# Maboroshi0327/MHAda-Style-Transfer

Hardware: AMD Instinct MI355X
Metric: stylized frames/sec (whole job) at 512x512 batch 8 fp32 [configs[1]] (higher is better)
Workload: dtype f32; 1 GPU; stylize 512x512 content+style, batch 8; resolution=512, batch_per_gpu=8, global_batch=8, compute_dtype=f32, parallelism=replicas x1

## Files before the change

include/mhada_hip.h:

```cpp
#ifndef MHADA_HIP_H
#define MHADA_HIP_H

#ifdef __cplusplus
extern "C" {
#endif

typedef void* mhada_stream_t;

enum { MHADA_OK = 0, MHADA_ERR_ARG = 1, MHADA_ERR_LAUNCH = 2 };
enum { MHADA_F32 = 0, MHADA_BF16 = 1 };
enum { MHADA_ACT_SOFTMAX = 0, MHADA_ACT_COSINE = 1 };
enum { MHADA_PAD_REFLECT = 0, MHADA_PAD_ZERO = 1 };
enum {
  MHADA_A_ROWS = 0,
  MHADA_A_PATCH8 = 1,
  MHADA_A_CONV3X3 = 2,
  MHADA_A_CONV3X3_UP2 = 3,
  MHADA_A_CONV3X3_ZERO = 4,
  MHADA_A_SPLIT3 = 5
};
enum { MHADA_BF16X3 = 2 };

int mhada_abi_version(void);
const char* mhada_last_error(void);

int mhada_set_tuning(const char* name, int value);
int mhada_get_tuning(const char* name, int* value);

int mhada_clock_probe(unsigned long long* stamps, int nblk, int iters, mhada_stream_t stream);

typedef struct mhada_gemm_args {
  int M, N, K;
  int nb1, nb2;
  int compute;
  int a_mode;
  const void* a; int a_dtype; long long lda, sa1, sa2;
  const float* a_mu; long long smu1, smu2;
  int img_c, img_h, img_w;
  const void* w; long long ldw, sw1, sw2;
  const float* bias; long long sb1, sb2;
  const void* r; int r_dtype; long long ldr, sr1, sr2;
  void* c; int c_dtype; long long ldc, sc1, sc2;
  int relu;
  int pad;
  void* c2; long long ldc2, sc21, sc22;
  void* vt; long long ldt, svt1, svt2;
  int c2_planes;
} mhada_gemm_args;

int mhada_gemm(const mhada_gemm_args* args, mhada_stream_t stream);

int mhada_layernorm(const float* x, void* y, int y_dtype, const float* gamma, const float* beta,
                    int rows, int cols, float eps, mhada_stream_t stream);

int mhada_vit_batch_attn(const void* qkv, void* out, int dtype, int L, int ntok, int heads,
                         int head_dim, mhada_stream_t stream);
int mhada_vit_batch_attn_split3(const float* qkv, void* planes, long long pstride, int L, int ntok, int heads,
                                int head_dim, mhada_stream_t stream);

int mhada_pos_embed(const float* pos, float* out, int C, int bh, int bw, int oh, int ow,
                    mhada_stream_t stream);

int mhada_instnorm_stats(const float* x, float* mu, float* rstd, double* work, int B, int N,
                         int C, int splits, float eps, mhada_stream_t stream);

int mhada_fold_block(const float* wf, const float* wg, const float* wh, const float* bg,
                     const float* bh, const float* rstd_c, const float* mu_s,
                     const float* rstd_s, void* wq, void* wkv, float* bkv, float* v_mu,
                     float kscale, int dtype, int B, int H, mhada_stream_t stream);

int mhada_transpose_v(const void* kv, void* vt, int dtype, int B, int H, int Ns, mhada_stream_t stream);

int mhada_cosine_prep(void* q, void* kv, int dtype, int B, int H, int Nc, int Ns,
                      mhada_stream_t stream);

int mhada_attn(const void* q, const void* kv, const void* vt, const float* fcs,
               const float* fcs_mu, const float* fcs_rstd, const float* v_mu, void* out,
               int dtype, int B, int H, int Nc, int Ns, int activation, mhada_stream_t stream);

int mhada_fold_block_hd(const float* wf, const float* wg, const float* wh, const float* bg,
                        const float* bh, const float* rstd_c, const float* mu_s,
                        const float* rstd_s, void* wq, void* wkv, float* bkv, float* v_mu,
                        float kscale, int dtype, int B, int H, int D, mhada_stream_t stream);

int mhada_cosine_prep_hd(void* q, void* kv, int dtype, int B, int H, int D, int Nc, int Ns,
                         mhada_stream_t stream);

int mhada_attn_hd(const void* q, const void* kv, const float* fcs, const float* fcs_mu,
                  const float* fcs_rstd, const float* v_mu, void* out, int dtype, int B, int H,
                  int D, int Nc, int Ns, int activation, mhada_stream_t stream);

int mhada_split3_kv(const float* kv, const float* vt, void* img, int B, int H, int Ns, mhada_stream_t stream);
int mhada_split3_rows(const float* x, void* planes, long long n, mhada_stream_t stream);
int mhada_split3_weight(const float* w, void* out, int N, int K0, int transposed, mhada_stream_t stream);

int mhada_layernorm_half2(const float* x, void* y, const float* gamma, const float* beta, int rows, int cols,
                          float eps, float scale, mhada_stream_t stream);
int mhada_half2_weight(const float* w, void* out, float* t, int N, int K0, mhada_stream_t stream);
int mhada_gemm_half2(const mhada_gemm_args* args, const float* col_scale, mhada_stream_t stream);
int mhada_kv_proj_split3(const float* fs, const float* mu_s, const float* wkv, const float* bkv, void* img,
                         int B, int H, int Ns, mhada_stream_t stream);
int mhada_attn_split3(const float* q, const void* img, const float* fcs, const float* fcs_mu,
                      const float* fcs_rstd, const float* v_mu, float* out, int B, int H, int Nc, int Ns,
                      mhada_stream_t stream);
int mhada_attn_split3_planes(const float* q, const void* img, const float* fcs, const float* fcs_mu,
                             const float* fcs_rstd, const float* v_mu, void* planes, int B, int H, int Nc, int Ns,
                             mhada_stream_t stream);

int mhada_cosine_moments(const void* kv, const void* vt, int dtype, int B, int H, int Ns, float* mom,
                         float* work, int splits, mhada_stream_t stream);
int mhada_cosine_attn(const void* q, const float* mom, const float* fcs, const float* fcs_mu,
                      const float* fcs_rstd, const float* v_mu, void* out, int dtype, int B, int H,
                      int Nc, mhada_stream_t stream);

int mhada_attn_train_fwd(const float* q, const float* k, const float* v, const float* x, float* out,
                         float* mo, float* lse, int BH, int Nc, int Ns, mhada_stream_t stream);
int mhada_attn_train_fwd_vt(const float* q, const float* k, const float* v, float* vt, const float* x,
                            float* out, float* mo, float* lse, int BH, int Nc, int Ns, mhada_stream_t stream);
int mhada_attn_train_fwd_split3(const float* q, const float* k, const float* v, void* img, const float* x,
                                float* out, float* mo, float* lse, int BH, int Nc, int Ns, mhada_stream_t stream);
int mhada_transpose64(const float* src, float* dst, int BH, int N, int ldt, mhada_stream_t stream);
int mhada_gemm_n64_split3(const float* a, const void* w_planes, float* c, int nz, int M, int K, int lda,
                          long long sa, int ldw, long long sw, long long wps, int ldc, long long sc,
                          mhada_stream_t stream);
int mhada_transpose64_split3(const float* k, void* planes, int BH, int N, int ldt, mhada_stream_t stream);
int mhada_attn_train_bwd(const float* q, const float* k, const float* v, const float* lse,
                         const float* dmo, const float* dd, float* dq, float* dk, float* dv,
                         int BH, int Nc, int Ns, mhada_stream_t stream);
int mhada_attn_train_dkv(const float* q, const float* k, const float* v, const float* lse, const float* dmo,
                         const float* dd, float* dk, float* dv, float* ds, int BH, int Nc, int Ns,
                         mhada_stream_t stream);

int mhada_attn_train_fwd_hd(const float* q, const float* k, const float* v, const float* x, float* out,
                            float* mo, float* lse, int BH, int D, int Nc, int Ns, mhada_stream_t stream);
int mhada_attn_train_bwd_hd(const float* q, const float* k, const float* v, const float* lse,
                            const float* dmo, const float* dd, float* dq, float* dk, float* dv,
                            int BH, int D, int Nc, int Ns, mhada_stream_t stream);

int mhada_attn_train_dq(const float* q, const float* k, const float* v, const float* lse, const float* dmo,
                        const float* dd, float* dq, int BH, int Nc, int Ns, mhada_stream_t stream);
int mhada_attn_train_dq_hd(const float* q, const float* k, const float* v, const float* lse, const float* dmo,
                           const float* dd, float* dq, int BH, int D, int Nc, int Ns, mhada_stream_t stream);

long long mhada_attn_train_bf16_workspace(int BH, int Nc, int Ns, int backward);
int mhada_attn_train_fwd_bf16(const float* q, const float* k, const float* v, const float* x, float* out,
                              float* mo, float* lse, void* ws, long long ws_size, int BH, int Nc, int Ns,
                              mhada_stream_t stream);
int mhada_attn_train_bwd_bf16(const float* q, const float* k, const float* v, const float* lse,
                              const float* dmo, const float* mo, float* dq, float* dk, float* dv,
                              void* ws, long long ws_size, int BH, int Nc, int Ns, int phases,
                              mhada_stream_t stream);

int mhada_conv3x3_out3(const void* x, int dtype, const float* w, const float* b, float* y,
                       int B, int H, int W, int Cin, int clamp255, mhada_stream_t stream);

int mhada_upsample2x(const void* x, void* y, int dtype, int B, int H, int W, int C,
                     mhada_stream_t stream);


int mhada_warp(const float* x, const float* flow, float* y, int B, int C, int H, int W,
               int padding, mhada_stream_t stream);

int mhada_warp_bwd(const float* gy, const float* flow, float* gx, int B, int C, int H, int W,
                   int padding, mhada_stream_t stream);

int mhada_flow_warp_mask(const float* flo01, const float* flo10, float* mask, int H, int W,
                         float threshold, int padding, mhada_stream_t stream);

int mhada_warp_l1(const float* cs1, const float* cs2, const float* flow, const float* mask,
                  double* work, float* out, int B, int C, int H, int W, mhada_stream_t stream);


typedef struct mhada_gemm_tn_args {
  int M, N, K;
  const float* a; long long lda;
  const float* b; long long ldb;
  int b_mode;
  int img_c, img_h, img_w, pad;
  float* c; long long ldc;
  float* colsum;
  int nb;
  long long sza, szb;
} mhada_gemm_tn_args;
int mhada_gemm_tn_splits(int M, int N, int K);
int mhada_gemm_tn(const mhada_gemm_tn_args* args, float* work, long long work_floats, mhada_stream_t stream);

int mhada_vit_batch_attn_bwd(const float* qkv, const float* dout, float* dqkv, int L, int ntok, int heads,
                             int head_dim, mhada_stream_t stream);
int mhada_vit_batch_attn_bwd_split3(const float* qkv, const float* dout, float* dqkv, void* planes,
                                    long long pstride, int L, int ntok, int heads, int head_dim,
                                    mhada_stream_t stream);

int mhada_colsum(const float* x, float* out, long long rows, int C, float* work, long long work_floats,
                 mhada_stream_t stream);

int mhada_layernorm_fwd(const float* x, float* y, float* stats, const float* gamma, const float* beta,
                        int rows, int cols, float eps, mhada_stream_t stream);
int mhada_layernorm_fwd_split3(const float* x, float* y, void* planes, float* stats, const float* gamma,
                               const float* beta, int rows, int cols, float eps, mhada_stream_t stream);

int mhada_layernorm_bwd(const float* x, const float* dy, const float* stats, const float* gamma, float* dx,
                        float* dgamma, float* dbeta, float* work, long long work_floats, int rows, int cols,
                        mhada_stream_t stream);

int mhada_instnorm_bwd(const float* dy, const float* y, const float* rstd, float* dx, double* work,
                       int B, int N, int C, int splits, mhada_stream_t stream);

int mhada_attn_train_bwd_prep(const float* dout, const float* x, const float* mo, float* dx, float* dmo,
                              float* dd, long long rows, mhada_stream_t stream);
int mhada_attn_train_bwd_prep_hd(const float* dout, const float* x, const float* mo, float* dx, float* dmo,
                                 float* dd, long long rows, int D, mhada_stream_t stream);

int mhada_pos_embed_bwd(const float* g, float* gpos, int C, int bh, int bw, int oh, int ow,
                        mhada_stream_t stream);
long long mhada_feat_stats_work(int B, long long P, int C);
int mhada_feat_stats(const float* x, const float* t, float* mu, float* sd, float* mse, double* work,
                     long long work_doubles, int B, long long P, int C, mhada_stream_t stream);
int mhada_feat_loss_bwd(const float* x, const float* t, const float* mu, const float* alpha, const float* beta,
                        const float* kp, float ks, float* g, int B, long long P, int C, int relu, mhada_stream_t stream);
int mhada_relu_bwd(const float* dy, const float* y, float* dx, long long n, mhada_stream_t stream);
int mhada_reflect_fold(const float* dxp, float* dx, int B, int H, int W, int C, const float* relu_mask,
                       mhada_stream_t stream);
int mhada_maxpool2(const float* x, float* y, int B, int H, int W, int C, mhada_stream_t stream);
int mhada_maxpool2_bwd(const float* x, const float* dy, float* dx, int B, int H, int W, int C, int relu_mask,
                       mhada_stream_t stream);
int mhada_upsample2x_bwd(const float* dy, const float* relu_x, float* dx, int B, int H, int W, int C,
                         mhada_stream_t stream);
int mhada_vgg_input(const float* img, float* out, int B, int H, int W, int Cp, mhada_stream_t stream);
int mhada_vgg_input_bwd(const float* dout, float* dimg, int B, int H, int W, int Cp, mhada_stream_t stream);

int mhada_loss_attn(const float* q, const float* k, const float* v, const float* x, const float* x_mu,
                    const float* x_rs, float* out, int B, int Nq, int Ns, int Dqk, int Dv, int activation,
                    mhada_stream_t stream);
int mhada_rows_normalize(const float* x, const float* mu, const float* rs, float* out, int unit,
                         int B, int N, int C, mhada_stream_t stream);

int mhada_frame_ingest(const void* frames, int B, int H, int W, long long row_bytes, int bgr, float* out,
                       int Ho, int Wo, mhada_stream_t stream);

int mhada_wino_weights(const float* w, float* u, int Cout, int Cin, mhada_stream_t stream);
int mhada_conv3x3_wgrad_wino_splits(int B, int H, int W, int Cin, int Cout);
int mhada_conv3x3_wgrad_wino(const float* x, const float* g, float* dw, float* db, float* work, long long work_floats,
                             int B, int H, int W, int Cin, int Cout, long long ldg, int pad_mode,
                             mhada_stream_t stream);
int mhada_conv3x3_wino(const float* x, const float* u, const float* bias, float* y, int B, int H, int W,
                       int Cin, int Cout, long long ldc, int pad_mode, int pad, int relu,
                       const float* relu_mask, mhada_stream_t stream);
int mhada_wino_weights_split3(const float* w, void* up, int Cout, int Cin, mhada_stream_t stream);
int mhada_conv3x3_wino_split3(const float* x, const float* u, const void* up, const float* bias, float* y, int B,
                              int H, int W, int Cin, int Cout, long long ldc, int pad_mode, int pad, int relu,
                              const float* relu_mask, mhada_stream_t stream);

// ... 16 lines not shown
```

mhada-style-transfer_amd/csrc/common.h:

```cpp
#pragma once
#include <hip/hip_runtime.h>
#include <stdint.h>
#include <string>

#include "../../include/mhada_hip.h"

typedef __bf16 bf16;
typedef __bf16 bf16x8 __attribute__((ext_vector_type(8)));
typedef __bf16 bf16x4 __attribute__((ext_vector_type(4)));
typedef float f32x16 __attribute__((ext_vector_type(16)));
typedef float f32x4 __attribute__((ext_vector_type(4)));
typedef float f32x2 __attribute__((ext_vector_type(2)));

#define MHADA_DEV __device__ __forceinline__

namespace mhada {

void set_error(const std::string& msg);
int fail(const std::string& msg);
int check_launch(const char* what);

struct Tuning {
  int attn_fixed_shift = 1;
  int attn_waves = 0;
  int attn_tk = 128;
  int attn_prio = 1;
  int vit_attn_vec = 1;
  int out3_mfma = 1;
  int out3_tile = 1;
  int gemm_pp = 1;
  int gemm_persist = 1;
  int gemm_pp128 = 1;
  int gemm_ldsepi = 1;
  int gemm_n64 = 128;
  int conv_c64 = 1;
  int conv_dir = 1;
  int gemm_rinit = 1;
  int tn_skinny_lds = 1;
  int wino4 = 1;
  int wino_split3 = 1;
  int gemm_s3_order = 1;
  int train_dkv_dma = 1;
  int upsample_quad = 1;
  int xknob = 0;
};
const Tuning& tuning();

int conv3x3_c64(const void* x, const void* w, const float* bias, void* y, int B, int H, int W, bool up, int relu,
                hipStream_t s);
int conv3x3_dir(const void* x, const void* w, const float* bias, void* y, int B, int H, int W, int cin, int cout,
                int relu, hipStream_t s);

int vit_batch_attn_hd(const void* qkv, void* out, int dtype, int L, int ntok, int heads, int head_dim, hipStream_t s);

template <typename T> MHADA_DEV float to_f32(T x);
template <> MHADA_DEV float to_f32<float>(float x) { return x; }
template <> MHADA_DEV float to_f32<bf16>(bf16 x) { return (float)x; }

template <typename T> MHADA_DEV T from_f32(float x);
template <> MHADA_DEV float from_f32<float>(float x) { return x; }
template <> MHADA_DEV bf16 from_f32<bf16>(float x) { return (bf16)x; }

template <typename T> struct Vec16;
template <> struct Vec16<float> { typedef f32x4 type; static constexpr int N = 4; };
template <> struct Vec16<bf16> { typedef bf16x8 type; static constexpr int N = 8; };

MHADA_DEV float bilerp(float ly0, float ly1, float lx0, float lx1, float x00, float x01, float x10, float x11) {
  return fmaf(ly1, fmaf(lx0, x10, lx1 * x11), ly0 * fmaf(lx0, x00, lx1 * x01));
}

MHADA_DEV float wave_sum(float v) {
#pragma unroll
  for (int o = 32; o > 0; o >>= 1) v += __shfl_xor(v, o, 64);
  return v;
}
MHADA_DEV float wave_max(float v) {
#pragma unroll
  for (int o = 32; o > 0; o >>= 1) v = fmaxf(v, __shfl_xor(v, o, 64));
  return v;
}

MHADA_DEV int xcd_remap(int bid, int nblk) {
  const int q = nblk / 8, r = nblk % 8;
  const int xcd = bid % 8, k = bid / 8;
  return (xcd < r ? xcd * (q + 1) : r * (q + 1) + (xcd - r) * q) + k;
}

}
```

mhada-style-transfer_amd/csrc/gemm_half2.hip:

```cpp
#include "gemm_impl.h"

using namespace mhada;

extern "C" int mhada_gemm_half2(const mhada_gemm_args* a, const float* col_scale, mhada_stream_t stream_) {
  if (!a) return fail("mhada_gemm_half2: null args");
  hipStream_t stream = (hipStream_t)stream_;
  if (a->M < 0 || a->N <= 0 || a->K <= 0) return fail("mhada_gemm_half2: bad sizes");
  if (a->nb1 != 1 || a->nb2 != 1) return fail("mhada_gemm_half2: one problem only (nb1 = nb2 = 1)");
  if (a->K % 64) return fail("mhada_gemm_half2: K0 must be a multiple of 64");
  if (a->a_mode != MHADA_A_ROWS || a->a_mu || a->vt) return fail("mhada_gemm_half2: ROWS mode, no centring / vt");
  if (a->c_dtype != MHADA_F32 && a->c_dtype != MHADA_BF16) return fail("mhada_gemm_half2: bad c_dtype");
  if (a->r && a->r_dtype != a->c_dtype) return fail("mhada_gemm_half2: residual dtype must equal output dtype");
  if (a->relu < 0 || a->relu > 1) return fail("mhada_gemm_half2: relu must be 0 or 1");
  if (!a->a || !a->w || !col_scale || (!a->c && !a->c2_planes)) return fail("mhada_gemm_half2: null operand");
  if (a->M == 0) return MHADA_OK;
  if (!aligned16(a->a) || a->lda % 8 || a->lda < a->K)
    return fail("mhada_gemm_half2: A must be 16-byte aligned with lda a multiple of 8 and >= K0");
  if (!aligned16(a->w) || a->ldw % 8 || a->ldw < 2 * (long long)a->K)
    return fail("mhada_gemm_half2: W must be 16-byte aligned with ldw a multiple of 8 and >= 2 K0");
  if (!aligned16(col_scale)) return fail("mhada_gemm_half2: col_scale must be 16-byte aligned");
  if (((uintptr_t)a->c & 7) || a->ldc % 4) return fail("mhada_gemm_half2: C must be 8-byte aligned with ldc % 4 == 0");
  if (a->r && (((uintptr_t)a->r & 7) || a->ldr % 4))
    return fail("mhada_gemm_half2: R must be 8-byte aligned with ldr % 4 == 0");
  if (a->bias && !aligned16(a->bias)) return fail("mhada_gemm_half2: bias must be 16-byte aligned");
  if (a->c2 && (a->c_dtype != MHADA_F32 || ((uintptr_t)a->c2 & 7) || a->ldc2 % 4))
    return fail("mhada_gemm_half2: c2 needs fp32 C, 8-byte alignment and ldc2 % 4 == 0");
  if (a->c2_planes && (!a->c2 || a->N % 4 || !tuning().gemm_ldsepi))
    return fail("mhada_gemm_half2: c2_planes needs a c2 buffer, N % 4 == 0 and the LDS epilogue");
  if ((((long long)a->M + 255) / 256) * (((long long)a->N + 255) / 256) >= (1LL << 31))
    return fail("mhada_gemm_half2: more than 2^31 tiles");
  if ((long long)(a->M - 1) * a->lda + a->K >= (1LL << 31) || (long long)(a->N - 1) * a->ldw + 2LL * a->K >= (1LL << 31))
    return fail("mhada_gemm_half2: operand spans need 32-bit element offsets");
  GemmP p{};
  p.M = a->M; p.N = a->N; p.K = a->K; p.nb2 = 1;
  p.a = a->a; p.lda = a->lda;
  p.spl = (long long)a->M * a->lda;
  p.w = a->w; p.ldw = a->ldw;
  p.bias = a->bias;
  p.r = a->r; p.ldr = a->ldr;
  p.c = a->c; p.ldc = a->ldc;
  p.relu = a->relu;
  p.c2 = a->c2; p.ldc2 = a->ldc2;
  p.c2planes = a->c2_planes ? 1 : 0;
  if (a->c_dtype == MHADA_F32) return launch_gemm_h2<float>(p, col_scale, stream);
  return launch_gemm_h2<bf16>(p, col_scale, stream);
}
```

mhada-style-transfer_amd/csrc/gemm_impl.h:

```cpp
#pragma once
#include "common.h"

#include <algorithm>
#include <mutex>
#include <stdlib.h>

namespace mhada {

struct GemmP {
  int M, N, K, nb2;
  const void* a; long long lda, sa1, sa2;
  const float* a_mu; long long smu1, smu2;
  int img_c, img_h, img_w, out_h, out_w;
  int pad;
  const void* w; long long ldw, sw1, sw2;
  const float* bias; long long sb1, sb2;
  const void* r; long long ldr, sr1, sr2;
  void* c; long long ldc, sc1, sc2;
  int relu, tiles_n, ntiles;
  int lds_epi;
  int rinit;
  void* c2; long long ldc2, sc21, sc22;
  void* vt; long long ldt, svt1, svt2;
  long long spl;
// ... 87 lines not shown
  bool valid;
};

template <typename TA, typename TC, int AMODE, int A_CH>
MHADA_DEV void issue_a(AStage<TA, TC, AMODE, A_CH>& st, const GemmP& p, const TA* abase,
                       const RowInfo (&ri)[A_CH], int k0, int kc) {
  constexpr int E = Cfg<TC>::E;
  const int k = k0 + kc * E;
  const bool kvalid = k < p.K;
  if constexpr (AMODE == MHADA_A_ROWS || AMODE == kRowsCentred) {
#pragma unroll
    for (int i = 0; i < A_CH; ++i) {
      const long long m = (long long)ri[i].b;
      st.raw[i][0] = (ri[i].valid && kvalid) ? load_raw<TA, TC>(abase + m * p.lda + k) : zero_raw<TA, TC>();
      st.wt[i][0] = 1.f;
    }
    if constexpr (AMODE == kRowsCentred) {
#pragma unroll
      for (int e = 0; e < E; ++e) st.mu[e] = kvalid ? p.a_mu[k + e] : 0.f;
    }
  } else if constexpr (AMODE == MHADA_A_PATCH8) {
    const int cch = k >> 6, py = (k >> 3) & 7, px = k & 7;
    const long long plane = (long long)p.img_h * p.img_w;
#pragma unroll
    for (int i = 0; i < A_CH; ++i) {
      const TA* src = abase + cch * plane + (long long)(ri[i].y * 8 + py) * p.img_w + ri[i].x * 8 + px;
      st.raw[i][0] = (ri[i].valid && kvalid) ? load_raw<TA, TC>(src) : zero_raw<TA, TC>();
      st.wt[i][0] = 1.f;
    }
  } else {
    const int cin_n = p.img_c;
    const int tap = k / cin_n, cin = k - tap * cin_n;
    const int dy = tap / 3 - 1, dx = tap % 3 - 1;
#pragma unroll
    for (int i = 0; i < A_CH; ++i) {
      int Y, X;
      const bool inside = conv_src<AMODE>(p, ri[i].y, ri[i].x, dy, dx, Y, X);
      const bool ok = ri[i].valid && kvalid && inside;
      if constexpr (AMODE == MHADA_A_CONV3X3 || AMODE == MHADA_A_CONV3X3_ZERO) {
        const TA* src = abase + (((long long)ri[i].b * p.img_h + Y) * p.img_w + X) * cin_n + cin;
        st.raw[i][0] = ok ? load_raw<TA, TC>(src) : zero_raw<TA, TC>();
        st.wt[i][0] = 1.f;
      } else {
        const float sy = fmaxf(((float)Y + 0.5f) * 0.5f - 0.5f, 0.f);
        const float sx = fmaxf(((float)X + 0.5f) * 0.5f - 0.5f, 0.f);
        const int y0 = (int)sy, x0 = (int)sx;
        const int y1 = y0 + (y0 < p.img_h - 1 ? 1 : 0), x1 = x0 + (x0 < p.img_w - 1 ? 1 : 0);
        const float ly1 = sy - (float)y0, lx1 = sx - (float)x0;
        const float ly0 = 1.f - ly1, lx0 = 1.f - lx1;
        const long long rb = (long long)ri[i].b * p.img_h;
        const TA* s00 = abase + ((rb + y0) * p.img_w + x0) * cin_n + cin;
        const TA* s01 = abase + ((rb + y0) * p.img_w + x1) * cin_n + cin;
        const TA* s10 = abase + ((rb + y1) * p.img_w + x0) * cin_n + cin;
        const TA* s11 = abase + ((rb + y1) * p.img_w + x1) * cin_n + cin;
        st.raw[i][0] = ok ? load_raw<TA, TC>(s00) : zero_raw<TA, TC>();
        st.raw[i][1] = ok ? load_raw<TA, TC>(s01) : zero_raw<TA, TC>();
        st.raw[i][2] = ok ? load_raw<TA, TC>(s10) : zero_raw<TA, TC>();
        st.raw[i][3] = ok ? load_raw<TA, TC>(s11) : zero_raw<TA, TC>();
        st.wt[i][0] = ly0; st.wt[i][1] = ly1; st.wt[i][2] = lx0; st.wt[i][3] = lx1;
      }
    }
  }
}

template <int RS, typename TA, typename TC, int AMODE, int A_CH>
MHADA_DEV void commit_a(const AStage<TA, TC, AMODE, A_CH>& st, TC* sA, int tid) {
  constexpr int E = Cfg<TC>::E, LS = Cfg<TC>::LS;
  const int kc = tid & 7;
#pragma unroll
  for (int i = 0; i < A_CH; ++i) {
    const int row = (tid >> 3) + RS * i;
    float f[E];
    if constexpr (AMODE == MHADA_A_CONV3X3_UP2) {
      const float ly0 = st.wt[i][0], ly1 = st.wt[i][1], lx0 = st.wt[i][2], lx1 = st.wt[i][3];
#pragma unroll
      for (int e = 0; e < E; ++e)
        f[e] = bilerp(ly0, ly1, lx0, lx1, raw_get(st.raw[i][0], e), raw_get(st.raw[i][1], e),
                      raw_get(st.raw[i][2], e), raw_get(st.raw[i][3], e));
    } else if constexpr (AMODE == kRowsCentred || sizeof(TA) != sizeof(TC)) {
#pragma unroll
      for (int e = 0; e < E; ++e) f[e] = raw_get(st.raw[i][0], e) - (AMODE == kRowsCentred ? st.mu[e] : 0.f);
    } else {
      *reinterpret_cast<typename Vec16<TC>::type*>(sA + row * LS + kc * E) = st.raw[i][0].v;
      continue;
    }
    store_chunk<TC>(sA + row * LS + kc * E, f);
  }
}

template <typename TO, int TM, int TN>
MHADA_DEV void store_tile(const GemmP& p, const f32x16 (&acc)[TM][TN], int z1, int z2, int mrow, int ncol, int h) {
  TO* cbase = reinterpret_cast<TO*>(p.c) + z1 * p.sc1 + z2 * p.sc2;
  const TO* rbase = p.r ? reinterpret_cast<const TO*>(p.r) + z1 * p.sr1 + z2 * p.sr2 : nullptr;
  const float* bbase = p.bias ? p.bias + z1 * p.sb1 + z2 * p.sb2 : nullptr;
#pragma unroll
  for (int mi = 0; mi < TM; ++mi) {
    const int m = mrow + mi * 32;
    if (m >= p.M) continue;
    TO* crow = cbase + (long long)m * p.ldc;
    const TO* rrow = rbase ? rbase + (long long)m * p.ldr : nullptr;
#pragma unroll
    for (int ni = 0; ni < TN; ++ni) {
#pragma unroll
      for (int g = 0; g < 4; ++g) {
        const int n = ncol + ni * 32 + 8 * g + 4 * h;
        float v[4];
#pragma unroll
        for (int e = 0; e < 4; ++e) v[e] = acc[mi][ni][4 * g + e];
        if (n + 3 < p.N) {
          if (bbase) {
            const f32x4 bb = *reinterpret_cast<const f32x4*>(bbase + n);
#pragma unroll
            for (int e = 0; e < 4; ++e) v[e] += bb[e];
          }
          if (p.relu == 1) {
#pragma unroll
            for (int e = 0; e < 4; ++e) v[e] = fmaxf(v[e], 0.f);
          }
          if constexpr (sizeof(TO) == 4) {
            if (rrow) {
              const f32x4 rr = *reinterpret_cast<const f32x4*>(rrow + n);
#pragma unroll
              for (int e = 0; e < 4; ++e) v[e] = p.relu == 2 ? (rr[e] > 0.f ? v[e] : 0.f) : v[e] + rr[e];
            }
            *reinterpret_cast<f32x4*>(crow + n) = f32x4{v[0], v[1], v[2], v[3]};
            if (p.c2)
              *reinterpret_cast<bf16x4*>(reinterpret_cast<bf16*>(p.c2) + z1 * p.sc21 + z2 * p.sc22 +
                                         (long long)m * p.ldc2 + n) = bf16x4{(bf16)v[0], (bf16)v[1], (bf16)v[2], (bf16)v[3]};
          } else {
            if (rrow) {
              const bf16x4 rr = *reinterpret_cast<const bf16x4*>(rrow + n);
#pragma unroll
              for (int e = 0; e < 4; ++e) v[e] += (float)rr[e];
            }
            *reinterpret_cast<bf16x4*>(crow + n) = bf16x4{(bf16)v[0], (bf16)v[1], (bf16)v[2], (bf16)v[3]};
          }
        } else {
#pragma unroll
          for (int e = 0; e < 4; ++e) {
            if (n + e < p.N) {
              float x = v[e] + (bbase ? bbase[n + e] : 0.f);
              if (p.relu == 1) x = fmaxf(x, 0.f);
              if (rrow) x = p.relu == 2 ? (to_f32<TO>(rrow[n + e]) > 0.f ? x : 0.f) : x + to_f32<TO>(rrow[n + e]);
              crow[n + e] = from_f32<TO>(x);
            }
          }
        }
      }
    }
  }
}


template <typename TO, int TM, int TN, bool PLANES = false>
MHADA_DEV void store_tile_lds(const GemmP& p, const f32x16 (&acc)[TM][TN], int z1, int z2, int mrow0, int ncol0,
                              int lane, float* scr) {
  TO* cbase = reinterpret_cast<TO*>(p.c) + z1 * p.sc1 + z2 * p.sc2;
  const TO* rbase = p.r ? reinterpret_cast<const TO*>(p.r) + z1 * p.sr1 + z2 * p.sr2 : nullptr;
  const float* bbase = p.bias ? p.bias + z1 * p.sb1 + z2 * p.sb2 : nullptr;
  const int h = lane >> 5, r32 = lane & 31;
  const int rr = lane >> 3, cq = lane & 7;
#pragma unroll
  for (int ni = 0; ni < TN; ++ni) {
    const int n = ncol0 + ni * 32 + 4 * cq;
    f32x4 bb = {0.f, 0.f, 0.f, 0.f};
    if (bbase) {
      if (n + 3 < p.N) {
        bb = *reinterpret_cast<const f32x4*>(bbase + n);
      } else {
#pragma unroll
        for (int e = 0; e < 4; ++e) bb[e] = n + e < p.N ? bbase[n + e] : 0.f;
      }
    }
#pragma unroll
    for (int mi = 0; mi < TM; ++mi) {
#pragma unroll
      for (int g = 0; g < 4; ++g) {
        const int c = 2 * g + h;
        *reinterpret_cast<f32x4*>(scr + r32 * 32 + 4 * (c ^ (r32 & 7))) =
            f32x4{acc[mi][ni][4 * g], acc[mi][ni][4 * g + 1], acc[mi][ni][4 * g + 2], acc[mi][ni][4 * g + 3]};
      }
      asm volatile("s_waitcnt lgkmcnt(0)" ::: "memory");
      f32x4 v[4];
#pragma unroll
      for (int i = 0; i < 4; ++i) {
        const int r = 8 * i + rr;
        v[i] = *reinterpret_cast<const f32x4*>(scr + r * 32 + 4 * (cq ^ (r & 7)));
      }
      asm volatile("s_waitcnt lgkmcnt(0)" ::: "memory");
#pragma unroll
      for (int i = 0; i < 4; ++i) {
        const int m = mrow0 + mi * 32 + 8 * i + rr;
        if (m >= p.M) continue;
        float x[4];
#pragma unroll
        for (int e = 0; e < 4; ++e) {
          x[e] = v[i][e] + bb[e];
          if (p.relu == 1) x[e] = fmaxf(x[e], 0.f);
        }
        TO* crow = cbase + (long long)m * p.ldc;
        const TO* rrow = rbase ? rbase + (long long)m * p.ldr : nullptr;
        if (n + 3 < p.N) {
          if constexpr (sizeof(TO) == 4) {
            if (rrow) {
              const f32x4 q = *reinterpret_cast<const f32x4*>(rrow + n);
#pragma unroll
              for (int e = 0; e < 4; ++e) x[e] = p.relu == 2 ? (q[e] > 0.f ? x[e] : 0.f) : x[e] + q[e];
            }
            if (!PLANES || p.c) *reinterpret_cast<f32x4*>(crow + n) = f32x4{x[0], x[1], x[2], x[3]};
            if (p.c2) {
              bf16* c2row = reinterpret_cast<bf16*>(p.c2) + z1 * p.sc21 + z2 * p.sc22 + (long long)m * p.ldc2 + n;
              const bf16x4 h0 = {(bf16)x[0], (bf16)x[1], (bf16)x[2], (bf16)x[3]};
              *reinterpret_cast<bf16x4*>(c2row) = h0;
              if (PLANES && p.c2planes) {
                const long long pl = (long long)p.M * p.ldc2;
                float r1[4];
                bf16x4 h1, h2;
#pragma unroll
                for (int e = 0; e < 4; ++e) {
                  r1[e] = x[e] - (float)h0[e];
                  h1[e] = (bf16)r1[e];
                  h2[e] = (bf16)(r1[e] - (float)h1[e]);
                }
                *reinterpret_cast<bf16x4*>(c2row + pl) = h1;
                *reinterpret_cast<bf16x4*>(c2row + 2 * pl) = h2;
              }
            }
          } else {
            if (rrow) {
              const bf16x4 q = *reinterpret_cast<const bf16x4*>(rrow + n);
#pragma unroll
              for (int e = 0; e < 4; ++e) x[e] += (float)q[e];
            }
            *reinterpret_cast<bf16x4*>(crow + n) = bf16x4{(bf16)x[0], (bf16)x[1], (bf16)x[2], (bf16)x[3]};
          }
        } else {
#pragma unroll
          for (int e = 0; e < 4; ++e) {
            if (n + e < p.N) {
              float y = x[e];
              if (rrow) y = p.relu == 2 ? (to_f32<TO>(rrow[n + e]) > 0.f ? y : 0.f) : y + to_f32<TO>(rrow[n + e]);
              crow[n + e] = from_f32<TO>(y);
            }
          }
        }
      }
    }
  }
}

template <typename TO, int TM>
MHADA_DEV void store_vt_tile(const GemmP& p, const f32x16 (&acc)[TM][2], int z1, int z2, int mrow0, int ncol0,
                             int lane, float* scr) {
  TO* vbase = reinterpret_cast<TO*>(p.vt) + z1 * p.svt1 + z2 * p.svt2;
  const float* bbase = p.bias ? p.bias + z1 * p.sb1 + z2 * p.sb2 : nullptr;
  const int h = lane >> 5, r32 = lane & 31;
#pragma unroll
  for (int mi = 0; mi < TM; ++mi) {
    const int m0 = mrow0 + 32 * mi;
    if (m0 >= p.ldt) break;
    const bool mv = m0 + r32 < p.M;
#pragma unroll
    for (int ni = 0; ni < 2; ++ni) {
      if constexpr (sizeof(TO) == 2) {
        bf16* sb = reinterpret_cast<bf16*>(scr);
        const int pos = (r32 & ~12) | ((r32 & 4) << 1) | ((r32 & 8) >> 1);
#pragma unroll
        for (int g = 0; g < 4; ++g)
#pragma unroll
          for (int e = 0; e < 4; ++e) {
            const int ol = 8 * g + 4 * h + e;
            float x = acc[mi][ni][4 * g + e] + (bbase ? bbase[ncol0 + 32 * ni + ol] : 0.f);
            sb[ol * 32 + pos] = mv ? (bf16)x : (bf16)0.0f;
          }
        asm volatile("s_waitcnt lgkmcnt(0)" ::: "memory");
        bf16x8 v[2];
#pragma unroll
        for (int j = 0; j < 2; ++j) {
          const int c = lane + 64 * j;
          v[j] = *reinterpret_cast<const bf16x8*>(sb + (c >> 2) * 32 + 8 * (c & 3));
        }
        asm volatile("s_waitcnt lgkmcnt(0)" ::: "memory");
#pragma unroll
        for (int j = 0; j < 2; ++j) {
          const int c = lane + 64 * j, ol = c >> 2, part = c & 3;
          TO* dst = vbase + (long long)(32 * ni + ol) * p.ldt + m0 + 8 * part;
          *reinterpret_cast<bf16x8*>(dst) = v[j];
          bf16x8 sq;
#pragma unroll
          for (int e = 0; e < 8; ++e) {
            const float f = (float)v[j][e];
            sq[e] = (bf16)(f * f);
          }
          *reinterpret_cast<bf16x8*>(dst + 64 * p.ldt) = sq;
        }
      } else {
#pragma unroll
        for (int g = 0; g < 4; ++g)
#pragma unroll
          for (int e = 0; e < 4; ++e) {
            const int ol = 8 * g + 4 * h + e;
            const float x = acc[mi][ni][4 * g + e] + (bbase ? bbase[ncol0 + 32 * ni + ol] : 0.f);
            scr[ol * 32 + r32] = mv ? x : 0.f;
          }
        asm volatile("s_waitcnt lgkmcnt(0)" ::: "memory");
        f32x4 v[4];
#pragma unroll
        for (int j = 0; j < 4; ++j) {
          const int c = lane + 64 * j;
          v[j] = *reinterpret_cast<const f32x4*>(scr + (c >> 3) * 32 + 4 * (c & 7));
        }
        asm volatile("s_waitcnt lgkmcnt(0)" ::: "memory");
#pragma unroll
        for (int j = 0; j < 4; ++j) {
          const int c = lane + 64 * j, ol = c >> 3, part = c & 7;
          float* dst = reinterpret_cast<float*>(vbase) + (long long)(32 * ni + ol) * p.ldt + m0 + 4 * part;
          *reinterpret_cast<f32x4*>(dst) = v[j];
          *reinterpret_cast<f32x4*>(dst + 64 * p.ldt) = v[j] * v[j];
        }
      }
    }
  }
}

template <int TM>
MHADA_DEV void store_tile_lds_bf16(const GemmP& p, const f32x16 (&acc)[TM][2], int z1, int z2, int mrow0, int ncol0,
                                   int lane, float* scr_f) {
  bf16* cbase = reinterpret_cast<bf16*>(p.c) + z1 * p.sc1 + z2 * p.sc2;
  const float* bbase = p.bias ? p.bias + z1 * p.sb1 + z2 * p.sb2 : nullptr;
  char* scr = reinterpret_cast<char*>(scr_f);
  const int h = lane >> 5, r32 = lane & 31;
  const int rr = lane >> 3, cq = lane & 7;
  f32x4 bb[2][4];
#pragma unroll
  for (int ni = 0; ni < 2; ++ni)
#pragma unroll
    for (int g = 0; g < 4; ++g) {
      const int n = ncol0 + ni * 32 + 8 * g + 4 * h;
      bb[ni][g] = f32x4{0.f, 0.f, 0.f, 0.f};
      if (bbase) {
        if (n + 3 < p.N) {
          bb[ni][g] = *reinterpret_cast<const f32x4*>(bbase + n);
        } else {
#pragma unroll
          for (int e = 0; e < 4; ++e) bb[ni][g][e] = n + e < p.N ? bbase[n + e] : 0.f;
        }
      }
    }
  const int n = ncol0 + 8 * cq;
#pragma unroll
  for (int mi = 0; mi < TM; ++mi) {
#pragma unroll
    for (int ni = 0; ni < 2; ++ni)
#pragma unroll
      for (int g = 0; g < 4; ++g) {
        bf16x4 o;
#pragma unroll
        for (int e = 0; e < 4; ++e) {
          float x = acc[mi][ni][4 * g + e] + bb[ni][g][e];
          if (p.relu == 1) x = fmaxf(x, 0.f);
          o[e] = (bf16)x;
        }
        const int c = 4 * ni + g;
// ... 642 lines not shown
#pragma unroll
      for (int i = 0; i < 2; ++i) glds16(src + s.aoff[hh][i], dst + hh * HALF + PE * i);
  };
  auto stage_w = [&](const St& s, int hh, int blk, int kk, int slot) {
    const bf16* src = wb + (6 * kk + blk) * BK;
    bf16* dst = smW + slot * SLOT + hh * HALF + wave * 2 * PE;
#pragma unroll
    for (int i = 0; i < 2; ++i) glds16(src + s.woff[hh][i], dst + PE * i);
  };

  const int swz = (r32 >> 1) & 7;
  int koff[4];
#pragma unroll
  for (int ks = 0; ks < 4; ++ks) koff[ks] = 8 * ((2 * ks + h) ^ swz);
  const bf16* sA = smA + grp * HALF + r32 * BK;
  const bf16* sW = smW + (wc >> 1) * HALF + ((wc & 1) * 64 + r32) * BK;
  bf16x8 af[4][2], wf[2][2];
  auto read_a = [&](int kp, int slot) {
#pragma unroll
    for (int mt = 0; mt < 4; ++mt)
#pragma unroll
      for (int s2 = 0; s2 < 2; ++s2)
        af[mt][s2] = *reinterpret_cast<const bf16x8*>(sA + slot * SLOT + mt * 32 * BK + koff[2 * kp + s2]);
  };
  auto read_w = [&](int nt, int kp, int slot) {
#pragma unroll
    for (int s2 = 0; s2 < 2; ++s2)
      wf[nt][s2] = *reinterpret_cast<const bf16x8*>(sW + slot * SLOT + nt * 32 * BK + koff[2 * kp + s2]);
  };
  f32x16 acc[4][2];
  auto zero_acc = [&](const St& s) {
    if constexpr (sizeof(TO) == 4) {
      if (p.rinit) {
        const float* rb = reinterpret_cast<const float*>(p.r);
        const float* bb = p.bias;
#pragma unroll
        for (int nt = 0; nt < 2; ++nt)
#pragma unroll
          for (int g = 0; g < 4; ++g) {
            const int n = s.n0 + wc * 64 + nt * 32 + 8 * g + 4 * h;
            const bool nok = n + 3 < p.N;
            const f32x4 b4 = (bb && nok) ? *reinterpret_cast<const f32x4*>(bb + n) : f32x4{0.f, 0.f, 0.f, 0.f};
#pragma unroll
            for (int mt = 0; mt < 4; ++mt) {
              const int m = s.m0 + grp * 128 + mt * 32 + r32;
              f32x4 r4 = {0.f, 0.f, 0.f, 0.f};
              if (nok && m < p.M) r4 = *reinterpret_cast<const f32x4*>(rb + (long long)m * p.ldr + n);
#pragma unroll
              for (int e = 0; e < 4; ++e) acc[mt][nt][4 * g + e] = r4[e] + b4[e];
            }
          }
        return;
      }
    }
#pragma unroll
    for (int a = 0; a < 4; ++a)
#pragma unroll
      for (int b = 0; b < 2; ++b)
#pragma unroll
        for (int e = 0; e < 16; ++e) acc[a][b][e] = 0.f;
  };
  GemmP pe = p;
  if (p.rinit) {
    pe.r = nullptr;
    pe.bias = nullptr;
  }
  auto compute = [&](int nt) {
    __builtin_amdgcn_s_setprio(1);
#pragma unroll
    for (int s2 = 0; s2 < 2; ++s2)
#pragma unroll
      for (int mt = 0; mt < 4; ++mt)
        acc[mt][nt] = __builtin_amdgcn_mfma_f32_32x32x16_bf16(wf[nt][s2], af[mt][s2], acc[mt][nt], 0, 0, 0);
    __builtin_amdgcn_s_setprio(0);
  };
  constexpr int EPI_MIN = sizeof(TO) == 4 ? 32 : 16;
  auto wait_vm = [&](int keep) __attribute__((always_inline)) {
    if (keep == 0) asm volatile("s_waitcnt vmcnt(0)" ::: "memory");
    else if (keep == 4) asm volatile("s_waitcnt vmcnt(4)" ::: "memory");
    else if (keep == 8) asm volatile("s_waitcnt vmcnt(8)" ::: "memory");
    else asm volatile("s_waitcnt vmcnt(%0)" :: "n"(8 + EPI_MIN) : "memory");
  };
  auto ktile = [&](int as, int ws, bool sw, const St& wt, int wblk, int wkk, int wsl, bool sa, const St& at, int apl,
                   int akk, int asl, int keep) __attribute__((always_inline)) {
    read_a(0, as); read_w(0, 0, ws);
    if (sw) stage_w(wt, 0, wblk, wkk, wsl);
    PP_LGKM0(); PP_BARRIER(); compute(0); PP_BARRIER();
    read_w(1, 0, ws);
    if (sw) stage_w(wt, 1, wblk, wkk, wsl);
    PP_LGKM0(); PP_BARRIER(); compute(1); PP_BARRIER();
    read_a(1, as); read_w(0, 1, ws);
    PP_LGKM0(); PP_BARRIER(); compute(0); PP_BARRIER();
    read_w(1, 1, ws);
    if (sa) stage_a(at, apl, akk, asl);
    wait_vm(keep);
    PP_LGKM0(); PP_BARRIER(); compute(1); PP_BARRIER();
  };
  int ap = 0;
  auto chunk = [&](const St& sc, int kk, const St& sn, int kn, bool nx, bool wx) __attribute__((always_inline)) {
    const int a0 = ap, a1 = ap ^ 1;
    ktile(a0, 0, true, sc, 0, kk, 1, true, sc, 0, kk, a0, wx ? 8 + EPI_MIN : 8);
    ktile(a1, 0, false, sc, 0, 0, 0, false, sc, 0, 0, 0, 4);
    ktile(a1, 1, true, sc, 2, kk, 0, nx, sn, 2, kn, a1, nx ? 8 : 4);
    ktile(a0, 1, false, sc, 0, 0, 0, false, sc, 0, 0, 0, nx ? 4 : 0);
    ktile(a0, 0, true, sc, 1, kk, 1, false, sc, 0, 0, 0, 0);
    ktile(a0, 1, nx, sn, 1, kn, 0, nx, sn, 1, kn, a0, nx ? 4 : 0);
    ap ^= 1;
  };

  const int KC = p.K / (6 * BK);
  int w = blockIdx.x;
  St cur, nxt;
  setup(w, cur);
  bool has_nxt = w + G < total;
  if (has_nxt) setup(w + G, nxt);
  zero_acc(cur);
  stage_a(cur, 2, 0, 0);
  stage_w(cur, 0, 1, 0, 0); stage_w(cur, 1, 1, 0, 0);
  stage_a(cur, 1, 0, 1);
  asm volatile("s_waitcnt vmcnt(4)" ::: "memory");
  PP_BARRIER();
  if (grp == 1) PP_BARRIER();

  bool lazy = false;
  while (true) {
    for (int kk = 0; kk + 1 < KC; ++kk) chunk(cur, kk, cur, kk + 1, true, kk == 0 && lazy);
    chunk(cur, KC - 1, nxt, 0, has_nxt, KC == 1 && lazy);
    if (grp == 0) PP_BARRIER();
    lazy = has_nxt && !p.rinit && cur.m0 + 256 <= p.M && cur.n0 + 256 <= p.N;
    __builtin_amdgcn_sched_barrier(0);
    if (p.lds_epi) {
      float* scr = reinterpret_cast<float*>(smem + 4 * SLOT) + wave * 1024;
      bool wide = false;
      if constexpr (sizeof(TO) == 2) {
        wide = !pe.r;
        if (wide) store_tile_lds_bf16<4>(pe, acc, 0, 0, cur.m0 + grp * 128, cur.n0 + wc * 64, lane, scr);
      }
      if (!wide) store_tile_lds<TO, 4, 2, true>(pe, acc, 0, 0, cur.m0 + grp * 128, cur.n0 + wc * 64, lane, scr);
    } else {
      store_tile<TO, 4, 2>(pe, acc, 0, 0, cur.m0 + grp * 128 + r32, cur.n0 + wc * 64, h);
    }
    if (!has_nxt) break;
    if (grp == 1) PP_BARRIER();
    zero_acc(nxt);
    cur = nxt;
    w += G;
    has_nxt = w + G < total;
    if (has_nxt) setup(w + G, nxt);
  }
}

typedef _Float16 f16x8 __attribute__((ext_vector_type(8)));

template <typename TO>
__global__ void __launch_bounds__(512) gemm_h2_kernel(const GemmP p, int total, const float* __restrict__ cs) {
  constexpr int BK = 64, PE = 512, HALF = 128 * BK, SLOT = 2 * HALF;
  constexpr int SCR = 8 * 4096 / 2;
  __shared__ __attribute__((aligned(16))) _Float16 smem[4 * SLOT + SCR];
  _Float16* const smA = smem;
  _Float16* const smW = smem + 2 * SLOT;
  const int tid = threadIdx.x, lane = tid & 63;
  const int wave = __builtin_amdgcn_readfirstlane(tid >> 6);
  const int grp = wave >> 2, wc = wave & 3;
  const int h = lane >> 5, r32 = lane & 31;
  const int G = gridDim.x;

  int cofs[2];
#pragma unroll
  for (int i = 0; i < 2; ++i) cofs[i] = 8 * ((lane & 7) ^ (4 * i + (lane >> 4)));
  struct St {
    unsigned aoff[2][2], woff[2][2];
    int m0, n0;
  };
  const _Float16* const ab = reinterpret_cast<const _Float16*>(p.a);
  const _Float16* const wb = reinterpret_cast<const _Float16*>(p.w);
  auto setup = [&](int w, St& s) {
    const int t = xcd_remap(w, total);
    const int tm = t / p.tiles_n, tn = t - tm * p.tiles_n;
    s.m0 = tm * 256;
    s.n0 = tn * 256;
#pragma unroll
    for (int hh = 0; hh < 2; ++hh)
#pragma unroll
      for (int i = 0; i < 2; ++i) {
        const int rr = 16 * wave + 8 * i + (lane >> 3);
        const int m = min(s.m0 + 128 * hh + rr, p.M - 1);
        const int n = min(s.n0 + 128 * hh + rr, p.N - 1);
        s.woff[hh][i] = (unsigned)((long long)n * p.ldw + cofs[i]);
        s.aoff[hh][i] = (unsigned)((long long)m * p.lda + cofs[i]);
      }
  };
  auto stage_a = [&](const St& s, int pl, int kk, int slot) {
    const _Float16* src = ab + pl * p.spl + kk * BK;
    _Float16* dst = smA + slot * SLOT + wave * 2 * PE;
#pragma unroll
    for (int hh = 0; hh < 2; ++hh)
#pragma unroll
      for (int i = 0; i < 2; ++i) glds16(src + s.aoff[hh][i], dst + hh * HALF + PE * i);
  };
  auto stage_w = [&](const St& s, int hh, int blk, int kk, int slot) {
    const _Float16* src = wb + (2 * kk + blk) * BK;
    _Float16* dst = smW + slot * SLOT + hh * HALF + wave * 2 * PE;
#pragma unroll
    for (int i = 0; i < 2; ++i) glds16(src + s.woff[hh][i], dst + PE * i);
  };

  const int swz = (r32 >> 1) & 7;
  int koff[4];
#pragma unroll
  for (int ks = 0; ks < 4; ++ks) koff[ks] = 8 * ((2 * ks + h) ^ swz);
  const _Float16* sA = smA + grp * HALF + r32 * BK;
  const _Float16* sW = smW + (wc >> 1) * HALF + ((wc & 1) * 64 + r32) * BK;
  f16x8 af[4][2], wf[2][2];
  auto read_a = [&](int kp, int slot) {
#pragma unroll
    for (int mt = 0; mt < 4; ++mt)
#pragma unroll
      for (int s2 = 0; s2 < 2; ++s2)
        af[mt][s2] = *reinterpret_cast<const f16x8*>(sA + slot * SLOT + mt * 32 * BK + koff[2 * kp + s2]);
  };
  auto read_w = [&](int nt, int kp, int slot) {
#pragma unroll
    for (int s2 = 0; s2 < 2; ++s2)
      wf[nt][s2] = *reinterpret_cast<const f16x8*>(sW + slot * SLOT + nt * 32 * BK + koff[2 * kp + s2]);
  };
  f32x16 acc[4][2];
  auto zero_acc = [&]() {
#pragma unroll
    for (int a = 0; a < 4; ++a)
#pragma unroll
      for (int b = 0; b < 2; ++b)
#pragma unroll
        for (int e = 0; e < 16; ++e) acc[a][b][e] = 0.f;
  };
  auto scale_acc = [&](const St& s) {
#pragma unroll
    for (int nt = 0; nt < 2; ++nt)
#pragma unroll
      for (int g = 0; g < 4; ++g) {
        const int n = s.n0 + wc * 64 + nt * 32 + 8 * g + 4 * h;
        f32x4 c4 = {0.f, 0.f, 0.f, 0.f};
        if (n + 3 < p.N) {
          c4 = *reinterpret_cast<const f32x4*>(cs + n);
        } else {
#pragma unroll
          for (int e = 0; e < 4; ++e)
            if (n + e < p.N) c4[e] = cs[n + e];
        }
#pragma unroll
        for (int mt = 0; mt < 4; ++mt)
#pragma unroll
          for (int e = 0; e < 4; ++e) acc[mt][nt][4 * g + e] *= c4[e];
      }
  };
  auto compute = [&](int nt) {
    __builtin_amdgcn_s_setprio(1);
#pragma unroll
    for (int s2 = 0; s2 < 2; ++s2)
#pragma unroll
      for (int mt = 0; mt < 4; ++mt)
        acc[mt][nt] = __builtin_amdgcn_mfma_f32_32x32x16_f16(wf[nt][s2], af[mt][s2], acc[mt][nt], 0, 0, 0);
    __builtin_amdgcn_s_setprio(0);
  };
  constexpr int EPI_MIN = sizeof(TO) == 4 ? 32 : 16;
  auto wait_vm = [&](int keep) __attribute__((always_inline)) {
    if (keep == 0) asm volatile("s_waitcnt vmcnt(0)" ::: "memory");
    else if (keep == 4) asm volatile("s_waitcnt vmcnt(4)" ::: "memory");
    else if (keep == 8) asm volatile("s_waitcnt vmcnt(8)" ::: "memory");
    else asm volatile("s_waitcnt vmcnt(%0)" :: "n"(8 + EPI_MIN) : "memory");
  };
  auto ktile = [&](int as, int ws, bool sw, const St& wt, int wblk, int wkk, int wsl, bool sa, const St& at, int apl,
                   int akk, int asl, int keep) __attribute__((always_inline)) {
    read_a(0, as); read_w(0, 0, ws);
    if (sw) stage_w(wt, 0, wblk, wkk, wsl);
    PP_LGKM0(); PP_BARRIER(); compute(0); PP_BARRIER();
    read_w(1, 0, ws);
    if (sw) stage_w(wt, 1, wblk, wkk, wsl);
    PP_LGKM0(); PP_BARRIER(); compute(1); PP_BARRIER();
    read_a(1, as); read_w(0, 1, ws);
    PP_LGKM0(); PP_BARRIER(); compute(0); PP_BARRIER();
    read_w(1, 1, ws);
    if (sa) stage_a(at, apl, akk, asl);
    wait_vm(keep);
    PP_LGKM0(); PP_BARRIER(); compute(1); PP_BARRIER();
  };
  auto chunk = [&](const St& sc, int kk, const St& sn, int kn, bool nx, bool wx) __attribute__((always_inline)) {
    ktile(0, 0, true, sc, 1, kk, 1, nx, sn, 1, kn, 0, nx ? (wx ? 8 + EPI_MIN : 8) : 4);
    ktile(1, 0, false, sc, 0, 0, 0, false, sc, 0, 0, 0, nx ? 4 : 0);
    ktile(1, 1, nx, sn, 0, kn, 0, nx, sn, 0, kn, 1, nx ? 4 : 0);
  };

  const int KC = p.K / BK;
  int w = blockIdx.x;
  St cur, nxt;
  setup(w, cur);
  bool has_nxt = w + G < total;
  if (has_nxt) setup(w + G, nxt);
  zero_acc();
  stage_a(cur, 1, 0, 0);
  stage_w(cur, 0, 0, 0, 0); stage_w(cur, 1, 0, 0, 0);
  stage_a(cur, 0, 0, 1);
  asm volatile("s_waitcnt vmcnt(4)" ::: "memory");
  PP_BARRIER();
  if (grp == 1) PP_BARRIER();

  bool lazy = false;
  while (true) {
    for (int kk = 0; kk + 1 < KC; ++kk) chunk(cur, kk, cur, kk + 1, true, kk == 0 && lazy);
    chunk(cur, KC - 1, nxt, 0, has_nxt, KC == 1 && lazy);
    if (grp == 0) PP_BARRIER();
    lazy = has_nxt && cur.m0 + 256 <= p.M && cur.n0 + 256 <= p.N;
    __builtin_amdgcn_sched_barrier(0);
    scale_acc(cur);
    if (p.lds_epi) {
      float* scr = reinterpret_cast<float*>(smem + 4 * SLOT) + wave * 1024;
      bool wide = false;
      if constexpr (sizeof(TO) == 2) {
        wide = !p.r;
        if (wide) store_tile_lds_bf16<4>(p, acc, 0, 0, cur.m0 + grp * 128, cur.n0 + wc * 64, lane, scr);
      }
      if (!wide) store_tile_lds<TO, 4, 2, true>(p, acc, 0, 0, cur.m0 + grp * 128, cur.n0 + wc * 64, lane, scr);
    } else {
      store_tile<TO, 4, 2>(p, acc, 0, 0, cur.m0 + grp * 128 + r32, cur.n0 + wc * 64, h);
    }
    if (!has_nxt) break;
    if (grp == 1) PP_BARRIER();
    zero_acc();
    cur = nxt;
    w += G;
    has_nxt = w + G < total;
    if (has_nxt) setup(w + G, nxt);
  }
}

template <int BM, int NS, int BK>
__global__ void __launch_bounds__(BM * 2) gemm_n64_kernel(const GemmP p) {
  constexpr int NWV = BM / 32, CH = BK / 4, RPI = 64 / CH;
  constexpr int AH = BM * BK, WH = 64 * BK, STAGE = AH + WH;
  constexpr int API = 32 / RPI, WPI = 64 / RPI / NWV;
  static_assert(WPI >= 1 && (CH == 8 || CH == 16), "tile config");
  __shared__ __attribute__((aligned(16))) float smem[NS * STAGE];
  const int tid = threadIdx.x, lane = tid & 63;
  const int wave = __builtin_amdgcn_readfirstlane(tid >> 6);
  int z, tile;
  if (p.lds_epi == 4) {
    const int L = blockIdx.y * gridDim.x + blockIdx.x, nt = gridDim.x;
    z = L % 8 + 8 * (L / (8 * nt));
    tile = (L / 8) % nt;
  } else {
    z = blockIdx.y;
    tile = xcd_remap(blockIdx.x, p.ntiles);
  }
  const int z1 = z / p.nb2, z2 = z - z1 * p.nb2;
  const int m0 = tile * BM;
  const float* ab = reinterpret_cast<const float*>(p.a) + z1 * p.sa1 + z2 * p.sa2;
  const float* wb = reinterpret_cast<const float*>(p.w) + z1 * p.sw1 + z2 * p.sw2;
  auto sw = [](int r) { return CH == 8 ? (r >> 1) & 7 : r & 15; };
  const float* asrc[API];
  const float* wsrc[WPI];
#pragma unroll
  for (int i = 0; i < API; ++i) {
    const int r = 32 * wave + RPI * i + lane / CH;
    const int m = min(m0 + r, p.M - 1);
    asrc[i] = ab + (long long)m * p.lda + 4 * ((lane % CH) ^ sw(r));
  }
#pragma unroll
  for (int i = 0; i < WPI; ++i) {
    const int r = RPI * (WPI * wave + i) + lane / CH;
    const int n = min(r, p.N - 1);
    wsrc[i] = wb + (long long)n * p.ldw + 4 * ((lane % CH) ^ sw(r));
  }
  auto stage = [&](int kt, int slot) {
    float* dst = smem + slot * STAGE;
    const int k0 = kt * BK;
#pragma unroll
    for (int i = 0; i < API; ++i) glds16(asrc[i] + k0, dst + (32 * wave + RPI * i) * BK);
#pragma unroll
    for (int i = 0; i < WPI; ++i) glds16(wsrc[i] + k0, dst + AH + RPI * (WPI * wave + i) * BK);
  };
  const int h = lane >> 5, r32 = lane & 31;
  int koff[CH / 2];
#pragma unroll
  for (int q = 0; q < CH / 2; ++q) koff[q] = 4 * (((CH / 2) * h + q) ^ sw(r32));
  f32x16 acc[1][2];
#pragma unroll
  for (int n = 0; n < 2; ++n)
#pragma unroll
    for (int e = 0; e < 16; ++e) acc[0][n][e] = 0.f;
  const int KT = p.K / BK;
#pragma unroll
  for (int i = 0; i < NS - 1; ++i)
    if (i < KT) stage(i, i);
  for (int kt = 0; kt < KT; ++kt) {
    const int ahead = min(KT - 1 - kt, NS - 2);
    if (ahead >= 2) asm volatile("s_waitcnt vmcnt(%0)" :: "n"(2 * (API + WPI)) : "memory");
    else if (ahead == 1) asm volatile("s_waitcnt vmcnt(%0)" :: "n"(API + WPI) : "memory");
    else asm volatile("s_waitcnt vmcnt(0)" ::: "memory");
    PP_BARRIER();
    if (kt + NS - 1 < KT) stage(kt + NS - 1, (kt + NS - 1) % NS);
    const float* sa = smem + (kt % NS) * STAGE + (32 * wave + r32) * BK;
    const float* swp = smem + (kt % NS) * STAGE + AH + r32 * BK;
    f32x4 af[CH / 2], wf[2][CH / 2];
#pragma unroll
    for (int q = 0; q < CH / 2; ++q) af[q] = *reinterpret_cast<const f32x4*>(sa + koff[q]);
#pragma unroll
    for (int n = 0; n < 2; ++n)
#pragma unroll
      for (int q = 0; q < CH / 2; ++q) wf[n][q] = *reinterpret_cast<const f32x4*>(swp + n * 32 * BK + koff[q]);
#pragma unroll
    for (int s = 0; s < BK / 2; ++s)
#pragma unroll
      for (int n = 0; n < 2; ++n)
        acc[0][n] = __builtin_amdgcn_mfma_f32_32x32x2f32(wf[n][s >> 2][s & 3], af[s >> 2][s & 3], acc[0][n], 0, 0, 0);
  }
  store_tile<float, 1, 2>(p, acc, z1, z2, m0 + 32 * wave + r32, 0, h);
}

static bool aligned16(const void* ptr) { return ((uintptr_t)ptr & 15) == 0; }

static int num_cus() {
  static int n = 0;
  if (!n) {
    int dev = 0;
    (void)hipGetDevice(&dev);
    if (hipDeviceGetAttribute(&n, hipDeviceAttributeMultiprocessorCount, dev) != hipSuccess || n <= 0) n = 256;
  }
  return n;
}

static bool persist_enabled() { return tuning().gemm_persist != 0; }

template <typename TC, typename TO, int AMODE, int BN = 256>
static int launch_gemm_pp(const GemmP& p0, int nz, hipStream_t stream) {
  GemmP p = p0;
  p.tiles_n = (p.N + BN - 1) / BN;
  p.ntiles = ((p.M + 255) / 256) * p.tiles_n;
  p.lds_epi = tuning().gemm_ldsepi ? 1 : 0;
  p.rinit = (sizeof(TO) == 4 && p.r && !p.relu && tuning().gemm_rinit && ((uintptr_t)p.r & 15) == 0 &&
             p.ldr % 4 == 0 && p.sr1 % 4 == 0 && p.sr2 % 4 == 0 && p.N % 4 == 0) ? 1 : 0;
  const long long total = (long long)p.ntiles * nz;
  if constexpr (AMODE == kRowsSplit3 && sizeof(TC) == 2 && BN == 256) {
    if (tuning().gemm_s3_order && nz == 1 && total < (1LL << 31)) {
      const int grid = (int)std::min<long long>(total, num_cus());
      hipLaunchKernelGGL((gemm_s3_kernel<TO>), dim3(grid), dim3(512), 0, stream, p, (int)total);
      return check_launch("mhada_gemm");
    }
  }
  if (sizeof(TC) == 4 || BN != 256 || AMODE == kRowsSplit3 || (p.K >= 128 && persist_enabled() && total < (1LL << 31))) {
    const int grid = (int)std::min<long long>(total, num_cus());
    hipLaunchKernelGGL((gemm_ppp_kernel<TC, TO, AMODE, BN>), dim3(grid), dim3(512), 0, stream, p, (int)total);
    return check_launch("mhada_gemm");
  }
  if constexpr (sizeof(TC) == 2 && BN == 256 && AMODE != kRowsSplit3) {
    hipLaunchKernelGGL((gemm_pp_kernel<TO, AMODE>), dim3(p.ntiles, nz), dim3(512), 0, stream, p);
    return check_launch("mhada_gemm");
  }
  return fail("mhada_gemm: no ping-pong form");
}

template <typename TO>
static int launch_gemm_h2(const GemmP& p0, const float* cs, hipStream_t stream) {
  GemmP p = p0;
  p.tiles_n = (int)(((long long)p.N + 255) / 256);
  const long long total = (((long long)p.M + 255) / 256) * p.tiles_n;
  if (total >= (1LL << 31)) return fail("mhada_gemm_half2: more than 2^31 tiles");
  p.ntiles = (int)total;
  p.lds_epi = tuning().gemm_ldsepi ? 1 : 0;
  p.rinit = 0;
  const int grid = (int)std::min<long long>(total, num_cus());
  hipLaunchKernelGGL((gemm_h2_kernel<TO>), dim3(grid), dim3(512), 0, stream, p, (int)total, cs);
  return check_launch("mhada_gemm_half2");
}

static bool pp_enabled() { return tuning().gemm_pp != 0; }

template <typename TC, typename TA, typename TO, int AMODE, int BM, int BN, int WM, int WN>
static int launch_gemm(const GemmP& p0, int nz, hipStream_t stream) {
  GemmP p = p0;
  p.tiles_n = (p.N + BN - 1) / BN;
  p.lds_epi = (tuning().gemm_ldsepi &&
               (size_t)2 * (BM + BN) * Cfg<TC>::LS * sizeof(TC) >= (size_t)WM * WN * 4096) ? 1 : 0;
  const int tiles_m = (p.M + BM - 1) / BM;
  p.ntiles = tiles_m * p.tiles_n;
  const size_t lds2 = (size_t)2 * (BM + BN) * Cfg<TC>::LS * sizeof(TC);
  const size_t lds = p.K > Cfg<TC>::BK ? lds2
                                       : std::max(lds2 / 2, (size_t)(p.lds_epi || p.vt ? WM * WN * 4096 : 0));
  static std::once_flag attr_once;
  std::call_once(attr_once, [&] {
    (void)hipFuncSetAttribute((const void*)gemm_kernel<TC, TA, TO, AMODE, BM, BN, WM, WN>,
                              hipFuncAttributeMaxDynamicSharedMemorySize, (int)lds2);
  });
  hipLaunchKernelGGL((gemm_kernel<TC, TA, TO, AMODE, BM, BN, WM, WN>), dim3(p.ntiles, nz), dim3(64 * WM * WN),
                     lds, stream, p);
  return check_launch("mhada_gemm");
}

static bool pp_offsets_fit(const GemmP& p, int amode) {
  const long long lim = 1LL << 31;
  const long long wspan = (long long)(p.N - 1) * p.ldw + p.K;
  long long aspan;
  if (amode == MHADA_A_ROWS) aspan = (long long)(p.M - 1) * p.lda + p.K;
  else aspan = (long long)p.M / ((long long)p.out_h * p.out_w) * p.img_h * p.img_w * p.img_c;
  return wspan < lim && aspan < lim;
}

template <typename TC, typename TA, typename TO, int AMODE>
static int dispatch_tile(const GemmP& p, int nz, hipStream_t s) {
  if constexpr (AMODE == MHADA_A_ROWS || AMODE == kRowsCentred) {
    if (p.vt) {
      if constexpr (sizeof(TC) == 2) return launch_gemm<TC, TA, TO, AMODE, 256, 128, 4, 2>(p, nz, s);
      else return launch_gemm<TC, TA, TO, AMODE, 128, 128, 2, 2>(p, nz, s);
    }
  }
  if (p.N <= 64) {
    if constexpr (sizeof(TC) == 4 && sizeof(TA) == 4 && sizeof(TO) == 4 && AMODE == MHADA_A_ROWS) {
      if (p.K % 32 == 0 && p.lda % 4 == 0 && p.ldw % 4 == 0 && p.sa1 % 4 == 0 && p.sa2 % 4 == 0 &&
          p.sw1 % 4 == 0 && p.sw2 % 4 == 0 && aligned16(p.a) && aligned16(p.w)) {
        GemmP q = p;
        q.tiles_n = 1;
        q.lds_epi = nz % 8 == 0 ? 4 : 0;
        if (p.K >= 1024 && p.K % 64 == 0) {
          q.ntiles = (p.M + 255) / 256;
          hipLaunchKernelGGL((gemm_n64_kernel<256, 2, 64>), dim3(q.ntiles, nz), dim3(512), 0, s, q);
        } else {
          q.ntiles = (p.M + 127) / 128;
          hipLaunchKernelGGL((gemm_n64_kernel<128, 2, 32>), dim3(q.ntiles, nz), dim3(256), 0, s, q);
        }
        return check_launch("mhada_gemm");
      }
    }
    if (tuning().gemm_n64 == 256) return launch_gemm<TC, TA, TO, AMODE, 256, 64, 8, 1>(p, nz, s);
    return launch_gemm<TC, TA, TO, AMODE, 128, 64, 4, 1>(p, nz, s);
  }
  if constexpr (sizeof(TC) == 4) {
    if constexpr (sizeof(TA) == 4 && (AMODE == MHADA_A_ROWS || AMODE == MHADA_A_CONV3X3 || AMODE == MHADA_A_CONV3X3_ZERO)) {
      const long long t256 = (long long)((p.M + 255) / 256) * ((p.N + 255) / 256) * nz;
      if (p.N > 128 && p.K % 32 == 0 && p.K >= 64 && 8 * t256 >= 7LL * num_cus() && pp_enabled() && persist_enabled() &&
          pp_offsets_fit(p, AMODE)) {
        return launch_gemm_pp<float, TO, AMODE>(p, nz, s);
      }
    }
    return launch_gemm<TC, TA, TO, AMODE, 128, 128, 2, 2>(p, nz, s);
  } else {
    if constexpr (AMODE == MHADA_A_CONV3X3_UP2) {
      return launch_gemm<TC, TA, TO, AMODE, 128, 128, 2, 2>(p, nz, s);
    } else {
      if constexpr (sizeof(TA) == 2 && (AMODE == MHADA_A_ROWS || AMODE == MHADA_A_CONV3X3)) {
        if (p.N > 128 && p.K % 64 == 0 && pp_enabled() && pp_offsets_fit(p, AMODE))
          return launch_gemm_pp<bf16, TO, AMODE>(p, nz, s);
        if (p.N > 64 && p.N <= 128 && p.K % 64 == 0 && p.K >= 128 && tuning().gemm_pp128 && pp_enabled() &&
            pp_offsets_fit(p, AMODE))
          return launch_gemm_pp<bf16, TO, AMODE, 128>(p, nz, s);
      }
      if (p.N <= 128) return launch_gemm<TC, TA, TO, AMODE, 256, 128, 4, 2>(p, nz, s);
      return launch_gemm<TC, TA, TO, AMODE, 256, 256, 2, 4>(p, nz, s);
    }
  }
}

template <typename TC, typename TA, typename TO>
static int dispatch_mode(int mode, const GemmP& p, int nz, hipStream_t s) {
  switch (mode) {
    case MHADA_A_ROWS:
      if (p.a_mu) return dispatch_tile<TC, TA, TO, kRowsCentred>(p, nz, s);
      return dispatch_tile<TC, TA, TO, MHADA_A_ROWS>(p, nz, s);
    case MHADA_A_CONV3X3: return dispatch_tile<TC, TA, TO, MHADA_A_CONV3X3>(p, nz, s);
    case MHADA_A_CONV3X3_UP2: return dispatch_tile<TC, TA, TO, MHADA_A_CONV3X3_UP2>(p, nz, s);
    case MHADA_A_CONV3X3_ZERO: return dispatch_tile<TC, TA, TO, MHADA_A_CONV3X3_ZERO>(p, nz, s);
    case MHADA_A_PATCH8:
      if constexpr (sizeof(TA) == 4) return dispatch_tile<TC, TA, TO, MHADA_A_PATCH8>(p, nz, s);
      return fail("mhada_gemm: PATCH8 needs an fp32 image");
    case MHADA_A_SPLIT3:
      if constexpr (sizeof(TC) == 2 && sizeof(TA) == 2) {
        if (nz != 1 || p.N <= 128 || p.K % (6 * 64) || p.K < 6 * 64 || !pp_offsets_fit(p, MHADA_A_ROWS))
          return fail("mhada_gemm: SPLIT3 needs one problem, N > 128, K0 = K / 6 a multiple of 64 and 32-bit offsets");
        return launch_gemm_pp<bf16, TO, kRowsSplit3>(p, nz, s);
      }
      return fail("mhada_gemm: SPLIT3 needs bf16 planes and bf16 compute");
  }
  return fail("mhada_gemm: bad a_mode");
}



int gemm_dispatch_f32(int mode, const GemmP& p, int nz, hipStream_t s);
int gemm_dispatch_bf16_a32_o32(int mode, const GemmP& p, int nz, hipStream_t s);
int gemm_dispatch_bf16_a32_o16(int mode, const GemmP& p, int nz, hipStream_t s);
int gemm_dispatch_bf16_a16_o32(int mode, const GemmP& p, int nz, hipStream_t s);
int gemm_dispatch_bf16_a16_o16(int mode, const GemmP& p, int nz, hipStream_t s);

}
```

mhada-style-transfer_amd/csrc/small_ops.hip:

```cpp
#include "common.h"

#include <stdlib.h>

namespace mhada {

typedef _Float16 f16;
MHADA_DEV f16 half2_plane(float v) {
  const f16 q = (f16)v;
  return fabsf((float)q) < 6.103515625e-05f ? (f16)0.0f : q;
}

template <typename TO, int VPL, int FORM = 0>
__global__ void __launch_bounds__(256) layernorm_kernel(const float* __restrict__ x, TO* __restrict__ y,
                                                        const float* __restrict__ g,
                                                        const float* __restrict__ b, int rows, float eps,
                                                        float scale) {
  constexpr int COLS = VPL * 64;
  const int lane = threadIdx.x & 63;
  const int row = blockIdx.x * 4 + (threadIdx.x >> 6);
  if (row >= rows) return;
  const float* xr = x + (long long)row * COLS;
  float v[VPL];
#pragma unroll
  for (int i = 0; i < VPL / 4; ++i) {
    const f32x4 t = *reinterpret_cast<const f32x4*>(xr + (i * 64 + lane) * 4);
    v[4 * i] = t[0]; v[4 * i + 1] = t[1]; v[4 * i + 2] = t[2]; v[4 * i + 3] = t[3];
  }
  if constexpr (FORM == 2) {
#pragma clang fp contract(off)
    float s = 0.f;
#pragma unroll
    for (int i = 0; i < VPL; ++i) s += v[i];
    const float mean = wave_sum(s) * (1.0f / COLS);
    float ss = 0.f;
#pragma unroll
    for (int i = 0; i < VPL; ++i) {
      v[i] = v[i] - mean;
      ss += v[i] * v[i];
    }
    const float rstd = rsqrtf(fmaf(wave_sum(ss), 1.0f / COLS, eps));
    TO* yr = y + (long long)row * COLS;
    const long long plane = (long long)rows * COLS;
#pragma unroll
    for (int i = 0; i < VPL / 4; ++i) {
#pragma unroll
      for (int e = 0; e < 4; ++e) {
        const int c = (i * 64 + lane) * 4 + e;
        const float sv = fmaf(v[4 * i + e] * rstd, g[c], b[c]) * scale;
        const f16 hi = half2_plane(sv);
        yr[c] = hi;
        yr[plane + c] = half2_plane(sv - (float)hi);
      }
    }
    return;
  }
  float s = 0.f;
#pragma unroll
  for (int i = 0; i < VPL; ++i) s += v[i];
  const float mean = wave_sum(s) * (1.0f / COLS);
  float ss = 0.f;
#pragma unroll
  for (int i = 0; i < VPL; ++i) {
    const float d = v[i] - mean;
    ss += d * d;
  }
  const float rstd = rsqrtf(wave_sum(ss) * (1.0f / COLS) + eps);
  TO* yr = y + (long long)row * COLS;
  const long long plane = (long long)rows * COLS;
#pragma unroll
  for (int i = 0; i < VPL / 4; ++i) {
#pragma unroll
    for (int e = 0; e < 4; ++e) {
      const int c = (i * 64 + lane) * 4 + e;
      const float val = (v[4 * i + e] - mean) * rstd * g[c] + b[c];
      if constexpr (FORM == 1) {
        const bf16 p0 = (bf16)val;
        const float r1 = val - (float)p0;
        const bf16 p1 = (bf16)r1;
        yr[c] = p0;
        yr[plane + c] = p1;
        yr[2 * plane + c] = (bf16)(r1 - (float)p1);
      } else {
        yr[c] = from_f32<TO>(val);
      }
    }
  }
}

template <typename T>
__global__ void __launch_bounds__(256) vit_batch_attn_kernel(const T* __restrict__ qkv, T* __restrict__ out,
                                                             int L, int ntok, int heads) {
  constexpr int D = 64;
  const int lane = threadIdx.x & 63, wv = threadIdx.x >> 6;
  const long long pair = (long long)blockIdx.x * 4 + wv;
  const int C = heads * D;
  if (pair >= (long long)ntok * heads) return;
  const int n = (int)(pair / heads), hh = (int)(pair - (long long)n * heads);
  const float scale = 0.125f;
  const long long row_stride = (long long)ntok * 3 * C;
  const T* base = qkv + (long long)n * 3 * C + hh * D + lane;
  for (int i = 0; i < L; ++i) {
    const float qi = to_f32<T>(base[i * row_stride]) * scale;
    float m = -INFINITY, l = 0.f, o = 0.f;
    for (int j = 0; j < L; ++j) {
      const float sj = wave_sum(qi * to_f32<T>(base[j * row_stride + C]));
      const float mn = fmaxf(m, sj);
      const float a = __expf(m - mn), p = __expf(sj - mn);
      l = l * a + p;
      o = o * a + p * to_f32<T>(base[j * row_stride + 2 * C]);
      m = mn;
    }
    out[((long long)i * ntok + n) * C + hh * D + lane] = from_f32<T>(o / l);
  }
}

template <typename T, int LMAX>
__global__ void __launch_bounds__(256) vit_batch_attn_vec_kernel(const T* __restrict__ qkv, T* __restrict__ out,
                                                                 int L, int ntok, int heads) {
  constexpr int D = 64, E = 8;
  const int g8 = threadIdx.x & 7;
  const long long pair = (long long)blockIdx.x * 32 + (threadIdx.x >> 3);
  const bool valid = pair < (long long)ntok * heads;
  const long long pp = valid ? pair : 0;
  const int C = heads * D;
  const int n = (int)(pp / heads), hh = (int)(pp - (long long)n * heads);
  const long long row_stride = (long long)ntok * 3 * C;
  const T* base = qkv + (long long)n * 3 * C + hh * D + g8 * E;
  auto load8 = [&](const T* p, float (&f)[E]) {
    if constexpr (sizeof(T) == 2) {
      const bf16x8 v = *reinterpret_cast<const bf16x8*>(p);
#pragma unroll
      for (int e = 0; e < E; ++e) f[e] = (float)v[e];
    } else {
      const f32x4 a = *reinterpret_cast<const f32x4*>(p), b = *reinterpret_cast<const f32x4*>(p + 4);
#pragma unroll
      for (int e = 0; e < 4; ++e) {
        f[e] = a[e];
        f[4 + e] = b[e];
      }
    }
  };
  float q[LMAX][E], k[LMAX][E], v[LMAX][E];
#pragma unroll
  for (int i = 0; i < LMAX; ++i) {
    if (i < L) {
      load8(base + i * row_stride, q[i]);
      load8(base + i * row_stride + C, k[i]);
      load8(base + i * row_stride + 2 * C, v[i]);
    }
  }
#pragma unroll
  for (int i = 0; i < LMAX; ++i) {
    if (i >= L) break;
    float sc[LMAX];
    float m = -INFINITY;
#pragma unroll
    for (int j = 0; j < LMAX; ++j) {
      if (j < L) {
        float d = 0.f;
#pragma unroll
        for (int e = 0; e < E; ++e) d = fmaf(q[i][e], k[j][e], d);
#pragma unroll
        for (int o = 1; o < 8; o <<= 1) d += __shfl_xor(d, o, 64);
        sc[j] = d * 0.125f;
        m = fmaxf(m, sc[j]);
      }
    }
    float l = 0.f, o8[E];
#pragma unroll
    for (int e = 0; e < E; ++e) o8[e] = 0.f;
#pragma unroll
    for (int j = 0; j < LMAX; ++j) {
      if (j < L) {
        const float p = __expf(sc[j] - m);
        l += p;
#pragma unroll
        for (int e = 0; e < E; ++e) o8[e] = fmaf(p, v[j][e], o8[e]);
      }
    }
    const float inv = 1.f / l;
    if (valid) {
      T* dst = out + ((long long)i * ntok + n) * C + hh * D + g8 * E;
      if constexpr (sizeof(T) == 2) {
        bf16x8 r;
#pragma unroll
        for (int e = 0; e < E; ++e) r[e] = (bf16)(o8[e] * inv);
        *reinterpret_cast<bf16x8*>(dst) = r;
      } else {
        *reinterpret_cast<f32x4*>(dst) = f32x4{o8[0] * inv, o8[1] * inv, o8[2] * inv, o8[3] * inv};
        *reinterpret_cast<f32x4*>(dst + 4) = f32x4{o8[4] * inv, o8[5] * inv, o8[6] * inv, o8[7] * inv};
      }
    }
  }
}

__global__ void __launch_bounds__(256) vit_batch_copy_v_kernel(const uint4* __restrict__ qkv, uint4* __restrict__ out,
                                                               int ntok, int row16) {
  const long long idx = (long long)blockIdx.x * 256 + threadIdx.x;
  if (idx >= (long long)ntok * row16) return;
  const long long n = idx / row16;
  const int c = (int)(idx - n * row16);
  out[n * row16 + c] = qkv[n * 3 * row16 + 2 * row16 + c];
}

template <typename T, bool PLANES>
MHADA_DEV void vit_batch_attn_small_body(const T* __restrict__ qkv, void* __restrict__ out_, long long pstride,
                                         int L, int ntok, int heads) {
  constexpr int D = 64;
  __shared__ float sq[4][8][D + 1];
  __shared__ float sk[4][8][D + 1];
  __shared__ float sp[4][8][8];
  const int lane = threadIdx.x & 63, wv = threadIdx.x >> 6;
  const long long pair = (long long)blockIdx.x * 4 + wv;
  const bool valid = pair < (long long)ntok * heads;
  const int C = heads * D;
  const long long pp = valid ? pair : 0;
  const int n = (int)(pp / heads), hh = (int)(pp - (long long)n * heads);
  const long long row_stride = (long long)ntok * 3 * C;
  const T* base = qkv + (long long)n * 3 * C + hh * D + lane;
  float vr[8];
#pragma unroll
  for (int i = 0; i < 8; ++i) {
    if (i < L) {
      sq[wv][i][lane] = to_f32<T>(base[i * row_stride]) * 0.125f;
      sk[wv][i][lane] = to_f32<T>(base[i * row_stride + C]);
      vr[i] = to_f32<T>(base[i * row_stride + 2 * C]);
    } else {
      vr[i] = 0.f;
    }
  }
  __syncthreads();
  const int i = lane >> 3, j = lane & 7;
  float s = -INFINITY;
  if (i < L && j < L) {
    s = 0.f;
#pragma unroll 16
    for (int d = 0; d < D; ++d) s = fmaf(sq[wv][i][d], sk[wv][j][d], s);
  }
  float m = s;
#pragma unroll
  for (int o = 1; o < 8; o <<= 1) m = fmaxf(m, __shfl_xor(m, o, 64));
  const float e = (i < L && j < L) ? __expf(s - m) : 0.f;
  float sum = e;
#pragma unroll
  for (int o = 1; o < 8; o <<= 1) sum += __shfl_xor(sum, o, 64);
  sp[wv][i][j] = e / sum;
  __syncthreads();
  if (!valid) return;
  for (int r = 0; r < L; ++r) {
    float o = 0.f;
#pragma unroll
    for (int c = 0; c < 8; ++c) o = fmaf(sp[wv][r][c], vr[c], o);
    const long long at = ((long long)r * ntok + n) * C + hh * D + lane;
    if constexpr (PLANES) {
      bf16* pl = reinterpret_cast<bf16*>(out_) + at;
      const bf16 a = (bf16)o;
      const float r1 = o - (float)a;
      const bf16 b = (bf16)r1;
      pl[0] = a;
      pl[pstride] = b;
      pl[2 * pstride] = (bf16)(r1 - (float)b);
    } else {
      reinterpret_cast<T*>(out_)[at] = from_f32<T>(o);
    }
  }
}

template <typename T>
__global__ void __launch_bounds__(256) vit_batch_attn_small_kernel(const T* __restrict__ qkv, T* __restrict__ out,
                                                                   int L, int ntok, int heads) {
  vit_batch_attn_small_body<T, false>(qkv, out, 0, L, ntok, heads);
}

__global__ void __launch_bounds__(256) vit_batch_attn_small_s3_kernel(const float* __restrict__ qkv,
                                                                      bf16* __restrict__ planes, long long pstride,
                                                                      int L, int ntok, int heads) {
  vit_batch_attn_small_body<float, true>(qkv, planes, pstride, L, ntok, heads);
}

__global__ void __launch_bounds__(256) vit_batch_copy_v_s3_kernel(const float* __restrict__ qkv,
                                                                  bf16* __restrict__ planes, long long pstride,
                                                                  int ntok, int row4) {
  const long long idx = (long long)blockIdx.x * 256 + threadIdx.x;
  if (idx >= (long long)ntok * row4) return;
  const long long n = idx / row4;
  const int c = (int)(idx - n * row4);
  const f32x4 v = *reinterpret_cast<const f32x4*>(qkv + 4 * (n * 3 * row4 + 2 * row4 + c));
  bf16x4 a, b, d;
#pragma unroll
  for (int e = 0; e < 4; ++e) {
    a[e] = (bf16)v[e];
    const float r = v[e] - (float)a[e];
    b[e] = (bf16)r;
    d[e] = (bf16)(r - (float)b[e]);
  }
  bf16* pl = planes + 4 * idx;
  *reinterpret_cast<bf16x4*>(pl) = a;
  *reinterpret_cast<bf16x4*>(pl + pstride) = b;
  *reinterpret_cast<bf16x4*>(pl + 2 * pstride) = d;
}

__global__ void pos_embed_kernel(const float* __restrict__ pos, float* __restrict__ out, int C, int bh,
                                 int bw, int oh, int ow) {
  const long long idx = (long long)blockIdx.x * blockDim.x + threadIdx.x;
  if (idx >= (long long)oh * ow * C) return;
  const int c = (int)(idx % C);
  const int tkn = (int)(idx / C);
  const int oy = tkn / ow, ox = tkn - (tkn / ow) * ow;
  const float* pc = pos + (long long)c * bh * bw;
  if (oh == bh && ow == bw) {
    out[idx] = pc[oy * bw + ox];
    return;
  }
  const float shy = (float)bh / (float)oh, shx = (float)bw / (float)ow;
  const float sy = fmaxf(shy * ((float)oy + 0.5f) - 0.5f, 0.f);
  const float sx = fmaxf(shx * ((float)ox + 0.5f) - 0.5f, 0.f);
  const int y0 = min((int)sy, bh - 1), x0 = min((int)sx, bw - 1);
  const int y1 = y0 + (y0 < bh - 1 ? 1 : 0), x1 = x0 + (x0 < bw - 1 ? 1 : 0);
  const float ly1 = sy - (float)y0, lx1 = sx - (float)x0;
  const float ly0 = 1.f - ly1, lx0 = 1.f - lx1;
  out[idx] = ly0 * (lx0 * pc[y0 * bw + x0] + lx1 * pc[y0 * bw + x1]) +
             ly1 * (lx0 * pc[y1 * bw + x0] + lx1 * pc[y1 * bw + x1]);
}

__global__ void __launch_bounds__(256) in_partial_kernel(const float* __restrict__ x, double* __restrict__ work,
                                                         int B, int N, int C, int splits) {
  __shared__ double red[2][16][65];
  const int quad = threadIdx.x & 15, ph = threadIdx.x >> 4;
  const int c0 = blockIdx.x * 64 + 4 * quad;
  const int b = blockIdx.y, s = blockIdx.z;
  const int per = (N + splits - 1) / splits;
  const int r0 = s * per, r1 = min(N, r0 + per);
  double s1[4] = {0.0, 0.0, 0.0, 0.0}, s2[4] = {0.0, 0.0, 0.0, 0.0};
  if (c0 < C) {
    const float* xb = x + (long long)b * N * C + c0;
#pragma unroll 4
    for (int r = r0 + ph; r < r1; r += 16) {
      const f32x4 v = *reinterpret_cast<const f32x4*>(xb + (long long)r * C);
#pragma unroll
      for (int e = 0; e < 4; ++e) {
        const double d = (double)v[e];
        s1[e] += d;
        s2[e] += d * d;
      }
    }
  }
#pragma unroll
  for (int e = 0; e < 4; ++e) {
    red[0][ph][4 * quad + e] = s1[e];
    red[1][ph][4 * quad + e] = s2[e];
  }
  __syncthreads();
  if (threadIdx.x < 128) {
    const int t = threadIdx.x & 63, which = threadIdx.x >> 6;
    const int c = blockIdx.x * 64 + t;
    double a = 0.0;
#pragma unroll
    for (int k = 0; k < 16; ++k) a += red[which][k][t];
    if (c < C) work[(((long long)s * B + b) * C + c) * 2 + which] = a;
  }
}

__global__ void __launch_bounds__(256) in_finalize_kernel(const double* __restrict__ work, float* __restrict__ mu,
                                                          float* __restrict__ rstd, int B, int N, int C, int splits,
                                                          float eps) {
  __shared__ double red[2][16][17];
  const int o = threadIdx.x & 15, ph = threadIdx.x >> 4;
  const int idx = blockIdx.x * 16 + o;
  double a = 0.0, q = 0.0;
  if (idx < B * C) {
    for (int s = ph; s < splits; s += 16) {
      a += work[((long long)s * B * C + idx) * 2];
      q += work[((long long)s * B * C + idx) * 2 + 1];
    }
  }
  red[0][ph][o] = a;
  red[1][ph][o] = q;
  __syncthreads();
  if (ph == 0 && idx < B * C) {
    double sa = 0.0, sq = 0.0;
#pragma unroll
    for (int k = 0; k < 16; ++k) {
      sa += red[0][k][o];
      sq += red[1][k][o];
    }
    const double mean = sa / N;
    double var = sq / N - mean * mean;
    if (var < 0.0) var = 0.0;
    mu[idx] = (float)mean;
    rstd[idx] = (float)(1.0 / sqrt(var + (double)eps));
  }
}

template <typename T>
__global__ void __launch_bounds__(256) fold_kernel(const float* __restrict__ wf, const float* __restrict__ wg,
                                                   const float* __restrict__ wh, const float* __restrict__ bg,
                                                   const float* __restrict__ bh, const float* __restrict__ rstd_c,
                                                   const float* __restrict__ mu_s, const float* __restrict__ rstd_s,
                                                   T* __restrict__ wq, T* __restrict__ wkv, float* __restrict__ bkv,
                                                   float* __restrict__ v_mu, float kscale, int H) {
  constexpr int D = 64;
  const int b = blockIdx.x / H, hh = blockIdx.x - (blockIdx.x / H) * H;
  const int C = H * D;
  const float* rc = rstd_c + (long long)b * C + hh * D;
  const float* rs = rstd_s + (long long)b * C + hh * D;
  const float* ms = mu_s + (long long)b * C + hh * D;
  const float* Wf = wf + (long long)hh * D * D;
  const float* Wg = wg + (long long)hh * D * D;
  const float* Wh = wh + (long long)hh * D * D;
  T* oq = wq + (long long)blockIdx.x * D * D;
  T* okv = wkv + (long long)blockIdx.x * 2 * D * D;
  for (int i = threadIdx.x; i < D * D; i += 256) {
    const int c = i & (D - 1);
    oq[i] = from_f32<T>(Wf[i] * rc[c]);
    okv[i] = from_f32<T>(Wg[i] * rs[c] * kscale);
    okv[D * D + i] = from_f32<T>(Wh[i]);
  }
  if (threadIdx.x < D) {
    const int o = threadIdx.x;
    float acc = bh[hh * D + o];
    for (int c = 0; c < D; ++c) acc += Wh[o * D + c] * ms[c];
    v_mu[(long long)b * C + hh * D + o] = acc;
    if (b == 0) {
      bkv[hh * 2 * D + o] = bg[hh * D + o] * kscale;
      bkv[hh * 2 * D + D + o] = 0.f;
    }
  }
}

template <typename T>
// ... 384 lines not shown
    (void)frexpf(m, &e);
    tn = ldexpf(1.f, min(15 - e, 127));
  }
  if (threadIdx.x == 0) t[n] = tn;
  f16* o = out + (long long)n * 2 * K0;
  for (int k = threadIdx.x; k < K0; k += 256) {
    const float v = wr[k] * tn;
    const f16 hi = half2_plane(v);
    o[128 * (k >> 6) + (k & 63)] = hi;
    o[128 * (k >> 6) + 64 + (k & 63)] = half2_plane(v - (float)hi);
  }
}

}

using namespace mhada;

extern "C" int mhada_half2_weight(const float* w, void* out, float* t, int N, int K0, mhada_stream_t s_) {
  if (!w || !out || !t || N <= 0 || K0 <= 0 || K0 % 64) return fail("mhada_half2_weight: bad args (K0 % 64 == 0)");
  hipLaunchKernelGGL(half2_weight_kernel, dim3((unsigned)N), dim3(256), 0, (hipStream_t)s_, w, (f16*)out, t, K0);
  return check_launch("mhada_half2_weight");
}

extern "C" int mhada_layernorm_half2(const float* x, void* y, const float* gamma, const float* beta, int rows,
                                     int cols, float eps, float scale, mhada_stream_t s_) {
  hipStream_t s = (hipStream_t)s_;
  if (!x || !y || !gamma || !beta || rows < 0 || !(scale > 0.f) || !(scale < INFINITY))
    return fail("mhada_layernorm_half2: bad args");
  if (rows == 0) return MHADA_OK;
  if (!aligned16(x)) return fail("mhada_layernorm_half2: x must be 16-byte aligned");
  const dim3 grid((rows + 3) / 4), blk(256);
#define LN_CASE(VPL)                                                                                       \
  case VPL * 64:                                                                                           \
    hipLaunchKernelGGL((layernorm_kernel<f16, VPL, 2>), grid, blk, 0, s, x, (f16*)y, gamma, beta, rows, eps, \
                       scale);                                                                             \
    break;
  switch (cols) {
    LN_CASE(4)
    LN_CASE(8)
    LN_CASE(16)
    LN_CASE(32)
    default:
      return fail("mhada_layernorm_half2: cols must be 256, 512, 1024 or 2048");
  }
#undef LN_CASE
  return check_launch("mhada_layernorm_half2");
}

extern "C" int mhada_split3_weight(const float* w, void* out, int N, int K0, int transposed, mhada_stream_t s_) {
  if (!w || !out || N <= 0 || K0 <= 0 || K0 % 64) return fail("mhada_split3_weight: bad args (K0 % 64 == 0)");
  const long long n = (long long)N * K0;
  hipLaunchKernelGGL(split3_weight_kernel, dim3((unsigned)((n + 255) / 256)), dim3(256), 0, (hipStream_t)s_, w,
                     (bf16*)out, N, K0, transposed);
  return check_launch("mhada_split3_weight");
}

extern "C" int mhada_layernorm(const float* x, void* y, int y_dtype, const float* gamma, const float* beta,
                               int rows, int cols, float eps, mhada_stream_t s_) {
  hipStream_t s = (hipStream_t)s_;
  if (!x || !y || !gamma || !beta || rows < 0 || y_dtype < MHADA_F32 || y_dtype > MHADA_BF16X3)
    return fail("mhada_layernorm: bad args");
  if (rows == 0) return MHADA_OK;
  if (!aligned16(x)) return fail("mhada_layernorm: x must be 16-byte aligned");
  const dim3 grid((rows + 3) / 4), blk(256);
#define LN_CASE(VPL)                                                                                   \
  case VPL * 64:                                                                                       \
    if (y_dtype == MHADA_F32)                                                                          \
      hipLaunchKernelGGL((layernorm_kernel<float, VPL>), grid, blk, 0, s, x, (float*)y, gamma, beta, rows, eps, 1.f); \
    else if (y_dtype == MHADA_BF16X3)                                                                  \
      hipLaunchKernelGGL((layernorm_kernel<bf16, VPL, 1>), grid, blk, 0, s, x, (bf16*)y, gamma, beta, rows, eps, 1.f); \
    else                                                                                               \
      hipLaunchKernelGGL((layernorm_kernel<bf16, VPL>), grid, blk, 0, s, x, (bf16*)y, gamma, beta, rows, eps, 1.f); \
    break;
  switch (cols) {
    LN_CASE(4)
    LN_CASE(8)
    LN_CASE(16)
    LN_CASE(32)
    default:
      return fail("mhada_layernorm: cols must be 256, 512, 1024 or 2048");
  }
#undef LN_CASE
  return check_launch("mhada_layernorm");
}

extern "C" int mhada_vit_batch_attn(const void* qkv, void* out, int dtype, int L, int ntok, int heads,
                                    int head_dim, mhada_stream_t s_) {
  hipStream_t s = (hipStream_t)s_;
  if (!qkv || !out || L <= 0 || ntok < 0 || heads <= 0) return fail("mhada_vit_batch_attn: bad args");
  if (head_dim != 64 && head_dim != 32 && head_dim != 128)
    return fail("mhada_vit_batch_attn: head_dim must be 32, 64 or 128");
  if (ntok == 0) return MHADA_OK;
  const long long pairs = (long long)ntok * heads;
  const size_t lds = 0;
  const dim3 grid((unsigned)((pairs + 3) / 4));
  if (L == 1 && aligned16(qkv) && aligned16(out)) {
    const int row16 = heads * head_dim * (dtype == MHADA_F32 ? 4 : 2) / 16;
    const long long n16 = (long long)ntok * row16;
    hipLaunchKernelGGL(vit_batch_copy_v_kernel, dim3((unsigned)((n16 + 255) / 256)), dim3(256), 0, s,
                       (const uint4*)qkv, (uint4*)out, ntok, row16);
    return check_launch("mhada_vit_batch_attn");
  }
  if (head_dim != 64) return vit_batch_attn_hd(qkv, out, dtype, L, ntok, heads, head_dim, s);
  if (L <= 8) {
    if (dtype != MHADA_F32 && tuning().vit_attn_vec && aligned16(qkv) && aligned16(out)) {
      const dim3 g32((unsigned)((pairs + 31) / 32));
      if (L <= 4)
        hipLaunchKernelGGL((vit_batch_attn_vec_kernel<bf16, 4>), g32, dim3(256), 0, s, (const bf16*)qkv, (bf16*)out, L,
                           ntok, heads);
      else
        hipLaunchKernelGGL((vit_batch_attn_vec_kernel<bf16, 8>), g32, dim3(256), 0, s, (const bf16*)qkv, (bf16*)out, L,
                           ntok, heads);
      return check_launch("mhada_vit_batch_attn");
    }
    if (dtype == MHADA_F32)
      hipLaunchKernelGGL((vit_batch_attn_small_kernel<float>), grid, dim3(256), 0, s, (const float*)qkv, (float*)out,
                         L, ntok, heads);
    else
      hipLaunchKernelGGL((vit_batch_attn_small_kernel<bf16>), grid, dim3(256), 0, s, (const bf16*)qkv, (bf16*)out,
                         L, ntok, heads);
  } else if (dtype == MHADA_F32) {
    hipLaunchKernelGGL((vit_batch_attn_kernel<float>), grid, dim3(256), lds, s, (const float*)qkv, (float*)out, L,
                       ntok, heads);
  } else {
    hipLaunchKernelGGL((vit_batch_attn_kernel<bf16>), grid, dim3(256), lds, s, (const bf16*)qkv, (bf16*)out, L,
                       ntok, heads);
  }
  return check_launch("mhada_vit_batch_attn");
}

extern "C" int mhada_vit_batch_attn_split3(const float* qkv, void* planes, long long pstride, int L, int ntok,
                                           int heads, int head_dim, mhada_stream_t s_) {
  hipStream_t s = (hipStream_t)s_;
  if (!qkv || !planes || L <= 0 || ntok < 0 || heads <= 0) return fail("mhada_vit_batch_attn_split3: bad args");
  if (head_dim != 64) return fail("mhada_vit_batch_attn_split3: head_dim must be 64");
  if (L > 8) return fail("mhada_vit_batch_attn_split3: L must be <= 8");
  if (pstride < (long long)L * ntok * heads * 64)
    return fail("mhada_vit_batch_attn_split3: plane stride smaller than this call's output");
  if (ntok == 0) return MHADA_OK;
  bf16* pl = reinterpret_cast<bf16*>(planes);
  if (L == 1 && aligned16(qkv) && aligned16(planes) && pstride % 4 == 0) {
    const int row4 = heads * 16;
    const long long n4 = (long long)ntok * row4;
    hipLaunchKernelGGL(vit_batch_copy_v_s3_kernel, dim3((unsigned)((n4 + 255) / 256)), dim3(256), 0, s, qkv, pl, pstride,
                       ntok, row4);
  } else {
    const long long pairs = (long long)ntok * heads;
    hipLaunchKernelGGL(vit_batch_attn_small_s3_kernel, dim3((unsigned)((pairs + 3) / 4)), dim3(256), 0, s, qkv, pl,
                       pstride, L, ntok, heads);
  }
  return check_launch("mhada_vit_batch_attn_split3");
}

extern "C" int mhada_pos_embed(const float* pos, float* out, int C, int bh, int bw, int oh, int ow,
                               mhada_stream_t s_) {
  if (!pos || !out || C <= 0 || bh <= 0 || bw <= 0 || oh <= 0 || ow <= 0) return fail("mhada_pos_embed: bad args");
  const long long n = (long long)oh * ow * C;
  hipLaunchKernelGGL(pos_embed_kernel, dim3((unsigned)((n + 255) / 256)), dim3(256), 0, (hipStream_t)s_, pos, out,
                     C, bh, bw, oh, ow);
  return check_launch("mhada_pos_embed");
}

extern "C" int mhada_instnorm_stats(const float* x, float* mu, float* rstd, double* work, int B, int N, int C,
                                    int splits, float eps, mhada_stream_t s_) {
  hipStream_t s = (hipStream_t)s_;
  if (!x || !mu || !rstd || !work || B <= 0 || N <= 0 || C <= 0 || splits <= 0)
    return fail("mhada_instnorm_stats: bad args");
  if (splits > 65535) return fail("mhada_instnorm_stats: too many splits");
  if (C % 4 || ((uintptr_t)x & 15)) return fail("mhada_instnorm_stats: needs C % 4 == 0 and a 16-byte aligned x");
  hipLaunchKernelGGL(in_partial_kernel, dim3((C + 63) / 64, B, splits), dim3(256), 0, s, x, work, B, N, C, splits);
  int rc = check_launch("mhada_instnorm_stats/partial");
  if (rc) return rc;
  hipLaunchKernelGGL(in_finalize_kernel, dim3((B * C + 15) / 16), dim3(256), 0, s, work, mu, rstd, B, N, C, splits,
                     eps);
  return check_launch("mhada_instnorm_stats/finalize");
}

extern "C" int mhada_fold_block(const float* wf, const float* wg, const float* wh, const float* bg, const float* bh,
                                const float* rstd_c, const float* mu_s, const float* rstd_s, void* wq, void* wkv,
                                float* bkv, float* v_mu, float kscale, int dtype, int B, int H, mhada_stream_t s_) {
  hipStream_t s = (hipStream_t)s_;
  if (!wf || !wg || !wh || !bg || !bh || !rstd_c || !mu_s || !rstd_s || !wq || !wkv || !bkv || !v_mu || B <= 0 ||
      H <= 0)
    return fail("mhada_fold_block: bad args");
  if (dtype == MHADA_F32)
    hipLaunchKernelGGL((fold_kernel<float>), dim3(B * H), dim3(256), 0, s, wf, wg, wh, bg, bh, rstd_c, mu_s, rstd_s,
                       (float*)wq, (float*)wkv, bkv, v_mu, kscale, H);
  else
    hipLaunchKernelGGL((fold_kernel<bf16>), dim3(B * H), dim3(256), 0, s, wf, wg, wh, bg, bh, rstd_c, mu_s, rstd_s,
                       (bf16*)wq, (bf16*)wkv, bkv, v_mu, kscale, H);
  return check_launch("mhada_fold_block");
}

extern "C" int mhada_transpose_v(const void* kv, void* vt, int dtype, int B, int H, int Ns, mhada_stream_t s_) {
  if (!kv || !vt || B <= 0 || H <= 0 || Ns <= 0) return fail("mhada_transpose_v: bad args");
  if (dtype != MHADA_F32 && dtype != MHADA_BF16) return fail("mhada_transpose_v: bad dtype");
  const int ldt = (Ns + 63) / 64 * 64;
  const dim3 grid(ldt / 64, B * H);
  if (dtype == MHADA_F32)
    hipLaunchKernelGGL((transpose_v_kernel<float>), grid, dim3(256), 0, (hipStream_t)s_, (const float*)kv, (float*)vt,
                       Ns, ldt);
  else
    hipLaunchKernelGGL((transpose_v_kernel<bf16>), grid, dim3(256), 0, (hipStream_t)s_, (const bf16*)kv, (bf16*)vt,
                       Ns, ldt);
  return check_launch("mhada_transpose_v");
}

extern "C" int mhada_cosine_prep(void* q, void* kv, int dtype, int B, int H, int Nc, int Ns, mhada_stream_t s_) {
  hipStream_t s = (hipStream_t)s_;
  if (B <= 0 || H <= 0 || Nc < 0 || Ns < 0 || (Nc == 0 && Ns == 0) || (Nc > 0 && !q) || (Ns > 0 && !kv))
    return fail("mhada_cosine_prep: bad args");
  if (dtype != MHADA_F32 && dtype != MHADA_BF16) return fail("mhada_cosine_prep: bad dtype");
  const long long rq = (long long)B * H * Nc, rk = (long long)B * H * Ns;
  if (rq > 0) {
    if (dtype == MHADA_F32)
      hipLaunchKernelGGL((rownorm_kernel<float>), dim3((unsigned)((rq + 3) / 4)), dim3(256), 0, s, (float*)q, rq, 64);
    else
      hipLaunchKernelGGL((rownorm_kernel<bf16>), dim3((unsigned)((rq + 3) / 4)), dim3(256), 0, s, (bf16*)q, rq, 64);
  }
  if (rk > 0) {
    if (dtype == MHADA_F32)
      hipLaunchKernelGGL((rownorm_kernel<float>), dim3((unsigned)((rk + 3) / 4)), dim3(256), 0, s, (float*)kv, rk, 128);
    else
      hipLaunchKernelGGL((rownorm_kernel<bf16>), dim3((unsigned)((rk + 3) / 4)), dim3(256), 0, s, (bf16*)kv, rk, 128);
  }
  return check_launch("mhada_cosine_prep");
}

extern "C" int mhada_conv3x3_out3(const void* x, int dtype, const float* w, const float* b, float* y, int B, int H,
                                  int W, int Cin, int clamp255, mhada_stream_t s_) {
  if (!x || !w || !b || !y || B <= 0 || H < 2 || W < 2) return fail("mhada_conv3x3_out3: bad args");
  if (!aligned16(x)) return fail("mhada_conv3x3_out3: x must be 16-byte aligned");
  const long long pix = (long long)B * H * W;
  const dim3 grid((unsigned)((pix + 255) / 256));
  hipStream_t s = (hipStream_t)s_;
  if (dtype == MHADA_BF16 && tuning().out3_mfma && (Cin == 32 || Cin == 64)) {
    const int tiles_x = (W + 63) / 64, strips_y = (H + 4 * kOut3RowsM - 1) / (4 * kOut3RowsM);
    const long long nb = (long long)B * strips_y * tiles_x;
    if (nb >= (1LL << 31)) return fail("mhada_conv3x3_out3: grid too large");
    const dim3 g((unsigned)nb);
    if (Cin == 64)
      hipLaunchKernelGGL((conv_out3_mfma_kernel<64, 32>), g, dim3(256), 0, s, (const bf16*)x, w, b, y, H, W, tiles_x, strips_y, clamp255);
    else
      hipLaunchKernelGGL((conv_out3_mfma_kernel<32, 32>), g, dim3(256), 0, s, (const bf16*)x, w, b, y, H, W, tiles_x, strips_y, clamp255);
    return check_launch("mhada_conv3x3_out3");
  }
  if (dtype == MHADA_F32 && tuning().out3_tile && (Cin == 32 || Cin == 64)) {
    const int tiles_x = (W + 63) / 64, strips_y = (H + 4 * kOut3Rows - 1) / (4 * kOut3Rows);
    const long long nb = (long long)B * strips_y * tiles_x;
    if (nb >= (1LL << 31)) return fail("mhada_conv3x3_out3: grid too large");
    const dim3 g((unsigned)nb);
    if (Cin == 64)
      hipLaunchKernelGGL((conv_out3_f32_kernel<64, 16>), g, dim3(256), 0, s, (const float*)x, w, b, y, H, W, tiles_x,
                         strips_y, clamp255);
    else
      hipLaunchKernelGGL((conv_out3_f32_kernel<32, 16>), g, dim3(256), 0, s, (const float*)x, w, b, y, H, W, tiles_x,
                         strips_y, clamp255);
    return check_launch("mhada_conv3x3_out3");
  }
#define OUT3_CASE(CI)                                                                                          \
  case CI:                                                                                                     \
    if (dtype == MHADA_F32)                                                                                    \
      hipLaunchKernelGGL((conv_out3_kernel<float, CI>), grid, dim3(256), 0, s, (const float*)x, w, b, y, B, H, W, \
                         clamp255);                                                                            \
    else                                                                                                       \
      hipLaunchKernelGGL((conv_out3_kernel<bf16, CI>), grid, dim3(256), 0, s, (const bf16*)x, w, b, y, B, H, W,   \
                         clamp255);                                                                            \
    break;
  switch (Cin) {
    OUT3_CASE(64)
    OUT3_CASE(32)
    OUT3_CASE(128)
    default:
      return fail("mhada_conv3x3_out3: Cin must be 32, 64 or 128");
  }
#undef OUT3_CASE
  return check_launch("mhada_conv3x3_out3");
}

template <typename T>
__global__ void __launch_bounds__(256) upsample2x_quad_kernel(const T* __restrict__ x, T* __restrict__ y, int B, int H,
                                                              int W, int C) {
  typedef typename Vec16<T>::type V;
  constexpr int N = Vec16<T>::N, NV = 8 / N;
  const int G = C / 8;
  const long long idx = (long long)blockIdx.x * 256 + threadIdx.x;
  const long long total = (long long)B * H * W * G;
  if (idx >= total) return;
  const int g = (int)(idx % G);
  long long pix = idx / G;
  const int j = (int)(pix % W);
  pix /= W;
  const int i = (int)(pix % H);
  const int b = (int)(pix / H);
  const T* base = x + (long long)b * H * W * C + g * 8;
  const int Wo = 2 * W, Ho = 2 * H;
  T* obase = y + (long long)b * Ho * Wo * C + g * 8;
  if (i >= 1 && i <= H - 2 && j >= 1 && j <= W - 2) {
#pragma unroll
    for (int v = 0; v < NV; ++v) {
      V w[3][3];
#pragma unroll
      for (int r = 0; r < 3; ++r)
#pragma unroll
        for (int c = 0; c < 3; ++c)
          w[r][c] = reinterpret_cast<const V*>(base + ((long long)(i - 1 + r) * W + (j - 1 + c)) * C)[v];
// ... 91 lines not shown
```

mhada-style-transfer_amd/mhada_hip/_lib.py:

```python
from __future__ import annotations

import ctypes
import os
import threading

LIB_PATH = os.path.join(os.path.dirname(os.path.abspath(__file__)), "libmhada_hip.so")

F32, BF16 = 0, 1
ACT_SOFTMAX, ACT_COSINE = 0, 1
A_ROWS, A_PATCH8, A_CONV3X3, A_CONV3X3_UP2, A_CONV3X3_ZERO, A_SPLIT3 = 0, 1, 2, 3, 4, 5
BF16X3 = 2
PAD_REFLECT, PAD_ZERO = 0, 1

_c_ll = ctypes.c_longlong
_vp = ctypes.c_void_p


class GemmArgs(ctypes.Structure):
    _fields_ = [
        ("M", ctypes.c_int), ("N", ctypes.c_int), ("K", ctypes.c_int),
        ("nb1", ctypes.c_int), ("nb2", ctypes.c_int),
        ("compute", ctypes.c_int), ("a_mode", ctypes.c_int),
        ("a", _vp), ("a_dtype", ctypes.c_int), ("lda", _c_ll), ("sa1", _c_ll), ("sa2", _c_ll),
        ("a_mu", _vp), ("smu1", _c_ll), ("smu2", _c_ll),
        ("img_c", ctypes.c_int), ("img_h", ctypes.c_int), ("img_w", ctypes.c_int),
        ("w", _vp), ("ldw", _c_ll), ("sw1", _c_ll), ("sw2", _c_ll),
        ("bias", _vp), ("sb1", _c_ll), ("sb2", _c_ll),
        ("r", _vp), ("r_dtype", ctypes.c_int), ("ldr", _c_ll), ("sr1", _c_ll), ("sr2", _c_ll),
        ("c", _vp), ("c_dtype", ctypes.c_int), ("ldc", _c_ll), ("sc1", _c_ll), ("sc2", _c_ll),
        ("relu", ctypes.c_int), ("pad", ctypes.c_int),
        ("c2", _vp), ("ldc2", _c_ll), ("sc21", _c_ll), ("sc22", _c_ll),
        ("vt", _vp), ("ldt", _c_ll), ("svt1", _c_ll), ("svt2", _c_ll),
        ("c2_planes", ctypes.c_int),
    ]


class GemmTnArgs(ctypes.Structure):
    _fields_ = [
        ("M", ctypes.c_int), ("N", ctypes.c_int), ("K", ctypes.c_int),
        ("a", _vp), ("lda", _c_ll), ("b", _vp), ("ldb", _c_ll), ("b_mode", ctypes.c_int),
        ("img_c", ctypes.c_int), ("img_h", ctypes.c_int), ("img_w", ctypes.c_int), ("pad", ctypes.c_int),
        ("c", _vp), ("ldc", _c_ll), ("colsum", _vp),
        ("nb", ctypes.c_int), ("sza", _c_ll), ("szb", _c_ll),
    ]


_I, _F = ctypes.c_int, ctypes.c_float
SIGNATURES = {
    "mhada_abi_version": (_I, []),
    "mhada_last_error": (ctypes.c_char_p, []),
    "mhada_set_tuning": (_I, [ctypes.c_char_p, _I]),
    "mhada_get_tuning": (_I, [ctypes.c_char_p, ctypes.POINTER(_I)]),
    "mhada_clock_probe": (_I, [_vp, _I, _I, _vp]),
    "mhada_gemm": (_I, [ctypes.POINTER(GemmArgs), _vp]),
    "mhada_layernorm": (_I, [_vp, _vp, _I, _vp, _vp, _I, _I, _F, _vp]),
    "mhada_vit_batch_attn": (_I, [_vp, _vp, _I, _I, _I, _I, _I, _vp]),
    "mhada_vit_batch_attn_split3": (_I, [_vp, _vp, _c_ll, _I, _I, _I, _I, _vp]),
    "mhada_pos_embed": (_I, [_vp, _vp, _I, _I, _I, _I, _I, _vp]),
    "mhada_instnorm_stats": (_I, [_vp, _vp, _vp, _vp, _I, _I, _I, _I, _F, _vp]),
    "mhada_fold_block": (_I, [_vp] * 12 + [_F, _I, _I, _I, _vp]),
    "mhada_transpose_v": (_I, [_vp, _vp, _I, _I, _I, _I, _vp]),
    "mhada_cosine_prep": (_I, [_vp, _vp, _I, _I, _I, _I, _I, _vp]),
    "mhada_cosine_moments": (_I, [_vp, _vp, _I, _I, _I, _I, _vp, _vp, _I, _vp]),
    "mhada_cosine_attn": (_I, [_vp, _vp, _vp, _vp, _vp, _vp, _vp, _I, _I, _I, _I, _vp]),
    "mhada_attn": (_I, [_vp] * 8 + [_I, _I, _I, _I, _I, _I, _vp]),
    "mhada_fold_block_hd": (_I, [_vp] * 12 + [_F, _I, _I, _I, _I, _vp]),
    "mhada_cosine_prep_hd": (_I, [_vp, _vp, _I, _I, _I, _I, _I, _I, _vp]),
    "mhada_attn_hd": (_I, [_vp] * 7 + [_I, _I, _I, _I, _I, _I, _I, _vp]),
    "mhada_split3_kv": (_I, [_vp, _vp, _vp, _I, _I, _I, _vp]),
    "mhada_kv_proj_split3": (_I, [_vp] * 5 + [_I, _I, _I, _vp]),
    "mhada_split3_rows": (_I, [_vp, _vp, _c_ll, _vp]),
    "mhada_split3_weight": (_I, [_vp, _vp, _I, _I, _I, _vp]),
    "mhada_layernorm_half2": (_I, [_vp, _vp, _vp, _vp, _I, _I, _F, _F, _vp]),
    "mhada_half2_weight": (_I, [_vp, _vp, _vp, _I, _I, _vp]),
    "mhada_gemm_half2": (_I, [ctypes.POINTER(GemmArgs), _vp, _vp]),
    "mhada_attn_split3": (_I, [_vp] * 7 + [_I, _I, _I, _I, _vp]),
    "mhada_attn_split3_planes": (_I, [_vp] * 7 + [_I, _I, _I, _I, _vp]),
    "mhada_attn_train_fwd": (_I, [_vp] * 7 + [_I, _I, _I, _vp]),
    "mhada_attn_train_fwd_vt": (_I, [_vp] * 8 + [_I, _I, _I, _vp]),
    "mhada_attn_train_fwd_split3": (_I, [_vp] * 8 + [_I, _I, _I, _vp]),
    "mhada_transpose64": (_I, [_vp, _vp, _I, _I, _I, _vp]),
    "mhada_gemm_n64_split3": (_I, [_vp, _vp, _vp, _I, _I, _I, _I, _c_ll, _I, _c_ll, _c_ll, _I, _c_ll, _vp]),
    "mhada_transpose64_split3": (_I, [_vp, _vp, _I, _I, _I, _vp]),
    "mhada_attn_train_bwd": (_I, [_vp] * 9 + [_I, _I, _I, _vp]),
    "mhada_attn_train_dkv": (_I, [_vp] * 9 + [_I, _I, _I, _vp]),
    "mhada_attn_train_fwd_hd": (_I, [_vp] * 7 + [_I, _I, _I, _I, _vp]),
    "mhada_attn_train_bwd_hd": (_I, [_vp] * 9 + [_I, _I, _I, _I, _vp]),
    "mhada_attn_train_dq": (_I, [_vp] * 7 + [_I, _I, _I, _vp]),
    "mhada_attn_train_dq_hd": (_I, [_vp] * 7 + [_I, _I, _I, _I, _vp]),
    "mhada_patch_embed_dgrad": (_I, [_vp, _vp, _vp, _I, _I, _I, _I, _I, _vp]),
    "mhada_attn_train_bf16_workspace": (_c_ll, [_I, _I, _I, _I]),
    "mhada_attn_train_fwd_bf16": (_I, [_vp] * 8 + [_c_ll, _I, _I, _I, _vp]),
    "mhada_attn_train_bwd_bf16": (_I, [_vp] * 10 + [_c_ll, _I, _I, _I, _I, _vp]),
    "mhada_conv3x3_out3": (_I, [_vp, _I, _vp, _vp, _vp, _I, _I, _I, _I, _I, _vp]),
    "mhada_upsample2x": (_I, [_vp, _vp, _I, _I, _I, _I, _I, _vp]),
    "mhada_warp": (_I, [_vp, _vp, _vp, _I, _I, _I, _I, _I, _vp]),
    "mhada_warp_bwd": (_I, [_vp, _vp, _vp, _I, _I, _I, _I, _I, _vp]),
    "mhada_flow_warp_mask": (_I, [_vp, _vp, _vp, _I, _I, _F, _I, _vp]),
    "mhada_warp_l1": (_I, [_vp, _vp, _vp, _vp, _vp, _vp, _I, _I, _I, _I, _vp]),
    "mhada_frame_ingest": (_I, [_vp, _I, _I, _I, _c_ll, _I, _vp, _I, _I, _vp]),
    "mhada_gemm_tn_splits": (_I, [_I, _I, _I]),
    "mhada_loss_attn": (_I, [_vp] * 7 + [_I, _I, _I, _I, _I, _I, _vp]),
    "mhada_rows_normalize": (_I, [_vp] * 4 + [_I, _I, _I, _I, _vp]),
    "mhada_gemm_tn": (_I, [ctypes.POINTER(GemmTnArgs), _vp, _c_ll, _vp]),
    "mhada_colsum": (_I, [_vp, _vp, _c_ll, _I, _vp, _c_ll, _vp]),
    "mhada_layernorm_fwd": (_I, [_vp, _vp, _vp, _vp, _vp, _I, _I, _F, _vp]),
    "mhada_layernorm_fwd_split3": (_I, [_vp, _vp, _vp, _vp, _vp, _vp, _I, _I, _F, _vp]),
    "mhada_layernorm_bwd": (_I, [_vp, _vp, _vp, _vp, _vp, _vp, _vp, _vp, _c_ll, _I, _I, _vp]),
    "mhada_pos_embed_bwd": (_I, [_vp, _vp, _I, _I, _I, _I, _I, _vp]),
    "mhada_instnorm_bwd": (_I, [_vp, _vp, _vp, _vp, _vp, _I, _I, _I, _I, _vp]),
    "mhada_attn_train_bwd_prep": (_I, [_vp, _vp, _vp, _vp, _vp, _vp, _c_ll, _vp]),
    "mhada_attn_train_bwd_prep_hd": (_I, [_vp, _vp, _vp, _vp, _vp, _vp, _c_ll, _I, _vp]),
    "mhada_vit_batch_attn_bwd": (_I, [_vp, _vp, _vp, _I, _I, _I, _I, _vp]),
    "mhada_vit_batch_attn_bwd_split3": (_I, [_vp, _vp, _vp, _vp, _c_ll, _I, _I, _I, _I, _vp]),
    "mhada_relu_bwd": (_I, [_vp, _vp, _vp, _c_ll, _vp]),
    "mhada_feat_stats_work": (_c_ll, [_I, _c_ll, _I]),
    "mhada_feat_stats": (_I, [_vp, _vp, _vp, _vp, _vp, _vp, _c_ll, _I, _c_ll, _I, _vp]),
    "mhada_feat_loss_bwd": (_I, [_vp, _vp, _vp, _vp, _vp, _vp, _F, _vp, _I, _c_ll, _I, _I, _vp]),
    "mhada_reflect_fold": (_I, [_vp, _vp, _I, _I, _I, _I, _vp, _vp]),
    "mhada_maxpool2": (_I, [_vp, _vp, _I, _I, _I, _I, _vp]),
    "mhada_maxpool2_bwd": (_I, [_vp, _vp, _vp, _I, _I, _I, _I, _I, _vp]),
    "mhada_upsample2x_bwd": (_I, [_vp, _vp, _vp, _I, _I, _I, _I, _vp]),
    "mhada_vgg_input": (_I, [_vp, _vp, _I, _I, _I, _I, _vp]),
    "mhada_vgg_input_bwd": (_I, [_vp, _vp, _I, _I, _I, _I, _vp]),
    "mhada_wino_weights": (_I, [_vp, _vp, _I, _I, _vp]),
    "mhada_conv3x3_wgrad_wino_splits": (_I, [_I, _I, _I, _I, _I]),
    "mhada_conv3x3_wgrad_wino": (_I, [_vp, _vp, _vp, _vp, _vp, _c_ll, _I, _I, _I, _I, _I, _c_ll, _I, _vp]),
    "mhada_conv3x3_wino": (_I, [_vp] * 4 + [_I] * 5 + [_c_ll, _I, _I, _I, _vp, _vp]),
    "mhada_conv3x3_wino_split3": (_I, [_vp] * 5 + [_I] * 5 + [_c_ll, _I, _I, _I, _vp, _vp]),
    "mhada_wino_weights_split3": (_I, [_vp, _vp, _I, _I, _vp]),
    "mhada_vgg_stem_dgrad": (_I, [_vp] * 4 + [_I] * 3 + [_vp]),
    "mhada_out3_dgrad": (_I, [_vp] * 5 + [_I] * 3 + [_vp]),
    "mhada_out3_wgrad_work": (_c_ll, [_I, _I, _I]),
    "mhada_out3_wgrad": (_I, [_vp] * 6 + [_c_ll, _I, _I, _I, _vp]),
}

_lib = None
_lock = threading.Lock()


def load(path: str | None = None) -> ctypes.CDLL:
    global _lib
    if _lib is not None and path is None:
        return _lib
    with _lock:
        if _lib is not None and path is None:
            return _lib
        p = path or LIB_PATH
        if not os.path.exists(p):
            raise RuntimeError(
                f"MHAda HIP library not found at {p}; build it with "
                "`python -c 'import __graft_entry__ as g; g.build()'` (make -C mhada-style-transfer_amd/csrc)")
        lib = ctypes.CDLL(p)
        for name, (res, args) in SIGNATURES.items():
            fn = getattr(lib, name)
            fn.restype = res
            fn.argtypes = args
        if path is None:
            _lib = lib
        return lib


ABI_VERSION = 18


def get_tuning(name: str) -> int:
    v = ctypes.c_int()
    check(load().mhada_get_tuning(name.encode(), ctypes.byref(v)), "mhada_get_tuning")
    return v.value


def set_tuning(name: str, value: int) -> None:
    check(load().mhada_set_tuning(name.encode(), int(value)), "mhada_set_tuning")


class tuning:

    def __init__(self, **knobs: int):
        self.knobs = knobs
        self.saved = {}

    def __enter__(self):
        for k, v in self.knobs.items():
            self.saved[k] = get_tuning(k)
            set_tuning(k, v)
        return self

    def __exit__(self, *exc):
        for k, v in self.saved.items():
            set_tuning(k, v)
        return False


def check(rc: int, what: str) -> None:
    if rc != 0:
        msg = load().mhada_last_error()
        msg = msg.decode() if msg else "unknown error"
        if rc == 1:
            raise ValueError(f"{what}: {msg}")
        raise RuntimeError(f"{what}: {msg}")
```

mhada-style-transfer_amd/mhada_hip/engine.py:

```python
from __future__ import annotations

from typing import Dict, List, Optional, Sequence, Tuple

import weakref

import torch

from . import ops
from ._lib import ACT_COSINE, ACT_SOFTMAX

HEAD_DIM = 64
DECODER_LAYERS: Tuple[Tuple[str, bool], ...] = (
    ("conv1.0", False), ("conv1.1", True), ("conv1.2", False), ("conv1.3", False),
    ("conv1.4", False), ("conv2.0", True), ("conv2.1", False), ("conv3.0", True),
)
LAST_LAYER = "conv3.1"
FUSE_UPSAMPLE = {torch.float32: False, torch.bfloat16: False}


def _fuse_upsample(dt: torch.dtype, w: torch.Tensor) -> bool:
    return FUSE_UPSAMPLE[dt] or (dt == torch.bfloat16 and w.shape[0] == 64 and w.shape[1] == 9 * 64)


_event_log = None


def record_kernel_events(log) -> None:
    global _event_log
    _event_log = log


class _timed:
    def __init__(self, name):
        self.name = name

    def __enter__(self):
        if _event_log is not None:
            self.s = torch.cuda.Event(enable_timing=True)
            self.s.record()
        return self

    def __exit__(self, *exc):
        if _event_log is not None:
            e = torch.cuda.Event(enable_timing=True)
            e.record()
            _event_log.setdefault(self.name, []).append((self.s, e))
        return False


def resolve_compute_dtype(module: torch.nn.Module) -> torch.dtype:
    explicit = getattr(module, "compute_dtype", None)
    if explicit is not None:
        if explicit not in (torch.float32, torch.bfloat16):
            raise ValueError(f"compute_dtype must be torch.float32 or torch.bfloat16, got {explicit}")
        return explicit
    if torch.is_autocast_enabled("cuda"):
        if torch.get_autocast_dtype("cuda") in (torch.bfloat16, torch.float16):
            return torch.bfloat16
    return torch.float32


def _signature(module: torch.nn.Module):
    return tuple((p.data_ptr(), p._version) for p in module.parameters())


def cached_prep(module: torch.nn.Module, dtype: torch.dtype, build):
    cache: Dict = module.__dict__.setdefault("_mhada_prep", {})
    key = (dtype, _signature(module))
    hit = cache.get(dtype)
    if hit is not None and hit[0] == key:
        return hit[1]
    with torch.no_grad():
        prep = build(dtype)
    cache[dtype] = (key, prep)
    return prep


def require_device(t: torch.Tensor, what: str) -> None:
    if not t.is_cuda:
        raise RuntimeError(f"{what}: the MI355X-native network runs on ROCm device tensors only; "
                           "move the module and inputs with .to('cuda')")


def to_tokens(x: torch.Tensor) -> torch.Tensor:
    t = x.permute(0, 2, 3, 1)
    if t.dtype != torch.float32:
        t = t.float()
    return t.contiguous()


def tokens_to_nchw(t: torch.Tensor, h: int, w: int) -> torch.Tensor:
    B, _, C = t.shape
    return t.view(B, h, w, C).permute(0, 3, 1, 2)


def vit_prep(vit, dtype):
    def build(dt):
        pe = vit.patch_embedding.conv_proj
        layers = []
        for blk in vit.encoder:
            att = blk.attention
            layers.append(dict(
                ln1_g=blk.ln1.weight.float().contiguous(), ln1_b=blk.ln1.bias.float().contiguous(),
                ln2_g=blk.ln2.weight.float().contiguous(), ln2_b=blk.ln2.bias.float().contiguous(),
                w_qkv=att.in_proj_weight.to(dt).contiguous(), b_qkv=att.in_proj_bias.float().contiguous(),
                w_o=att.out_proj.weight.to(dt).contiguous(), b_o=att.out_proj.bias.float().contiguous(),
                w1=blk.mlp[0].weight.to(dt).contiguous(), b1=blk.mlp[0].bias.float().contiguous(),
                w2=blk.mlp[2].weight.to(dt).contiguous(), b2=blk.mlp[2].bias.float().contiguous(),
                heads=att.num_heads, eps=blk.ln1.eps))
        return dict(patch_w=pe.weight.reshape(pe.weight.shape[0], -1).to(dt).contiguous(),
                    patch_b=pe.bias.float().contiguous(), layers=layers, pos={})
    return cached_prep(vit, dtype, build)


_NUM_CUS: Dict = {}


def _split3_fills(M: int, N: int, dev: torch.device) -> bool:
    if not ops.F32_SPLIT:
        return False
    idx = dev.index if dev.index is not None else torch.cuda.current_device()
    if idx not in _NUM_CUS:
        _NUM_CUS[idx] = torch.cuda.get_device_properties(idx).multi_processor_count
    return 8 * ((M + 255) // 256) * ((N + 255) // 256) >= 7 * _NUM_CUS[idx]


def _w6(L: dict, key: str) -> torch.Tensor:
    k6 = key + "_split3"
    if k6 not in L:
        with torch.no_grad():
            L[k6] = ops.split3_weight(L[key])
    return L[k6]


def _h2(L: dict, ln: str, key: str) -> Optional[dict]:
    if not ops.F32_HALF2:
        return None
    k2 = key + "_half2"
    if k2 not in L:
        with torch.no_grad():
            L[k2] = ops.half2_prepare(L[ln + "_g"], L[ln + "_b"], L[key])
    return L[k2]


def vit_forward(vit, x: torch.Tensor) -> List[torch.Tensor]:
    require_device(x, "VisionTransformer")
    dt = resolve_compute_dtype(vit)
    prep = vit_prep(vit, dt)
    if x.dim() != 4 or x.shape[1] != 3:
        raise ValueError(f"expected an image batch (B, 3, H, W), got {tuple(x.shape)}")
    img = x.float().contiguous()
    B, _, H, W = img.shape
    p = vit.patch_size
    h, w = H // p, W // p
    N = h * w
    C = prep["patch_w"].shape[0]
    pos = None
    if vit.pos_embedding is not None:
        pos = prep["pos"].get((h, w))
        if pos is None:
            pos = ops.pos_embed(vit.pos_embedding.pos_embed.detach().float().contiguous(), h, w)
            prep["pos"][(h, w)] = pos
    tok = ops.patch_embed(img, prep["patch_w"], prep["patch_b"], pos, p)
    xs = tok.view(B * N, C)
    outs = []
    for L in prep["layers"]:
        split = dt == torch.float32 and _split3_fills(B * N, 3 * C, xs.device)
        split_mlp = dt == torch.float32 and _split3_fills(B * N, C, xs.device)
        h2q = _h2(L, "ln1", "w_qkv") if split else None
        h2m = _h2(L, "ln2", "w1") if split_mlp else None
        if h2q is not None:
            qkv = ops.linear_half2(ops.layernorm_half2(xs, L["ln1_g"], L["ln1_b"], L["eps"], h2q["s_a"]),
                                   h2q["w2"], h2q["cs"], L["b_qkv"], dt)
        elif split:
            qkv = ops.linear_split3(ops.layernorm_split3(xs, L["ln1_g"], L["ln1_b"], L["eps"]), _w6(L, "w_qkv"),
                                    L["b_qkv"], dt)
        else:
            hb = ops.layernorm(xs, L["ln1_g"], L["ln1_b"], dt, L["eps"])
            qkv = ops.linear(hb, L["w_qkv"], L["b_qkv"], dt)
        if split_mlp and ops.F32_SPLIT_OUTPROJ and C == L["heads"] * HEAD_DIM and B <= ops.VIT_ATTN_SPLIT3_MAX_L:
            att3 = ops.vit_batch_attn_split3(qkv.view(B, N, 3 * C), B, N, L["heads"])
            xs = ops.linear_split3(att3, _w6(L, "w_o"), L["b_o"], torch.float32, residual=xs)
        else:
            att = ops.vit_batch_attn(qkv.view(B, N, 3 * C), B, N, L["heads"])
            xs = ops.linear(att.view(B * N, C), L["w_o"], L["b_o"], torch.float32, residual=xs)
        if split_mlp:
            if h2m is not None:
                m1 = ops.linear_half2(ops.layernorm_half2(xs, L["ln2_g"], L["ln2_b"], L["eps"], h2m["s_a"]),
                                      h2m["w2"], h2m["cs"], L["b1"], dt, relu=True, out_planes=True)
            else:
                m1 = ops.linear_split3(ops.layernorm_split3(xs, L["ln2_g"], L["ln2_b"], L["eps"]), _w6(L, "w1"),
                                       L["b1"], dt, relu=True, out_planes=True)
            xs = ops.linear_split3(m1, _w6(L, "w2"), L["b2"], torch.float32, residual=xs)
        else:
            h2 = ops.layernorm(xs, L["ln2_g"], L["ln2_b"], dt, L["eps"])
            m1 = ops.linear(h2, L["w1"], L["b1"], dt, relu=True)
            xs = ops.linear(m1, L["w2"], L["b2"], torch.float32, residual=xs)
        outs.append(tokens_to_nchw(xs.view(B, N, C), h, w))
    return outs


def block_prep(blk, dtype):
    def build(dt):
        H = blk.num_heads
        d = blk.head_dim

        def stack(lst):
            return torch.stack([m.weight.reshape(d, d) for m in lst]).float().contiguous()

        def stackb(lst):
            return torch.stack([m.bias for m in lst]).float().contiguous()
        C = H * d
        return dict(wf=stack(blk.f_list), wg=stack(blk.g_list), wh=stack(blk.h_list),
                    bf=stackb(blk.f_list), bg=stackb(blk.g_list), bh=stackb(blk.h_list),
                    w_out=blk.out_conv.weight.reshape(C, C).to(dt).contiguous(),
                    b_out=blk.out_conv.bias.float().contiguous())
    return cached_prep(blk, dtype, build)


class _Feat:

    def __init__(self, t: torch.Tensor, h: int, w: int):
        self.t, self.h, self.w = t, h, w
        self._stats = None
        self.t16 = None

    @classmethod
    def from_nchw(cls, x: torch.Tensor):
        _, _, h, w = x.shape
        t = to_tokens(x)
        return cls(t.view(t.shape[0], h * w, t.shape[3]), h, w)

    def stats(self):
        if self._stats is None:
            self._stats = ops.instnorm_stats(self.t)
        return self._stats


def block_forward(blk, fc: _Feat, fs: Optional[_Feat], fcs: _Feat, dt: torch.dtype,
                  side: Optional[dict] = None, want_bf16: bool = False) -> _Feat:
    if blk.head_dim in ops.HD_WIDTHS:
        return _block_forward_hd(blk, fc, fs, fcs, dt, side, want_bf16)
    if blk.head_dim != HEAD_DIM:
        raise ValueError("the HIP MHAda kernels implement head_dim (qkv_dim/num_heads) in {32, 64, 128}, "
                         f"got {blk.head_dim}")
    prep = block_prep(blk, dt)
    H = blk.num_heads
    C = H * HEAD_DIM
    B, Nc, Cc = fc.t.shape
    cached = bool(side)
    mom = img = kv = vt = None
    act = ACT_COSINE if blk.activation_name == "cosine" else ACT_SOFTMAX
    split_attn = act == ACT_SOFTMAX and dt == torch.float32 and ops.F32_SPLIT_ATTN
    if cached:
        mu_s, rstd_s, mom, Ns = side["mu_s"], side["rstd_s"], side.get("mom"), side["Ns"]
        kv, vt, img = side.get("kv"), side.get("vt"), side.get("img")
        if side["B"] != B:
            raise ValueError(f"cached style batch {side['B']} != content batch {B}")
    else:
        if fs.t.shape[2] != C:
            raise ValueError(f"channel mismatch: block expects {C}")
        mu_s, rstd_s = fs.stats()
    if Cc != C or fcs.t.shape[2] != C:
        raise ValueError(f"channel mismatch: block expects {C}")
    mu_c, rstd_c = fc.stats()
    mu_o, rstd_o = fcs.stats()
    wq, wkv, bkv, v_mu = ops.fold_block(prep["wf"], prep["wg"], prep["wh"], prep["bg"], prep["bh"],
                                        rstd_c, mu_s, rstd_s, dt, ops.LOG2E if act == ACT_SOFTMAX else 1.0)
    dev = fc.t.device
    q = torch.empty(B, H, Nc, HEAD_DIM, device=dev, dtype=dt)
    ops.gemm(a=fc.t, w=wq, c=q, M=Nc, N=HEAD_DIM, K=HEAD_DIM, compute=dt, lda=C, sa=(Nc * C, HEAD_DIM),
             nb=(B, H), a_mu=mu_c, smu=(C, HEAD_DIM), ldw=HEAD_DIM, sw=(H * HEAD_DIM * HEAD_DIM, HEAD_DIM * HEAD_DIM),
             bias=prep["bf"], sb=(0, HEAD_DIM), ldc=HEAD_DIM, sc=(H * Nc * HEAD_DIM, Nc * HEAD_DIM))
    if not cached and split_attn:
        Ns = fs.t.shape[1]
        img = ops.kv_proj_split3(fs.t, mu_s, wkv, bkv)
        if side is not None:
            side.update(mu_s=mu_s, rstd_s=rstd_s, img=img, Ns=Ns, B=B)
    elif not cached:
        Ns = fs.t.shape[1]
        kv = torch.empty(B, H, Ns, 2 * HEAD_DIM, device=dev, dtype=dt)
        ldt = (Ns + 63) // 64 * 64
        vt = torch.empty(B, H, 2 * HEAD_DIM, ldt, device=dev, dtype=dt)
        ops.gemm(a=fs.t, w=wkv, c=kv, M=Ns, N=2 * HEAD_DIM, K=HEAD_DIM, compute=dt, lda=C, sa=(Ns * C, HEAD_DIM),
                 nb=(B, H), a_mu=mu_s, smu=(C, HEAD_DIM), ldw=HEAD_DIM,
                 sw=(H * 2 * HEAD_DIM * HEAD_DIM, 2 * HEAD_DIM * HEAD_DIM), bias=bkv, sb=(0, 2 * HEAD_DIM),
                 ldc=2 * HEAD_DIM, sc=(H * Ns * 2 * HEAD_DIM, Ns * 2 * HEAD_DIM),
                 vt=vt, ldt=ldt, svt=(H * 2 * HEAD_DIM * ldt, 2 * HEAD_DIM * ldt))
        if act == ACT_COSINE:
            ops.cosine_prep(None, kv)
            mom = ops.cosine_moments(kv, vt)
        if side is not None:
            side.update(mu_s=mu_s, rstd_s=rstd_s, kv=kv, vt=vt, mom=mom, Ns=Ns, B=B)
    if act == ACT_COSINE:
        ops.cosine_prep(q, None)
        with _timed("mhada_attn"):
            att = ops.cosine_attn(q, mom, fcs.t, mu_o, rstd_o, v_mu)
    elif split_attn and ops.F32_SPLIT_OUTPROJ and _split3_fills(B * Nc, C, dev):
        with _timed("mhada_attn"):
            att3 = ops.attn_split3_planes(q, img, Ns, fcs.t, mu_o, rstd_o, v_mu)
        if "w_out_split3" not in prep:
            with torch.no_grad():
                prep["w_out_split3"] = ops.split3_weight(prep["w_out"])
        out = ops.linear_split3(att3, prep["w_out_split3"], prep["b_out"], torch.float32)
        return _Feat(out.view(B, Nc, C), fc.h, fc.w)
    elif split_attn:
        with _timed("mhada_attn"):
            att = ops.attn_split3(q, img, Ns, fcs.t, mu_o, rstd_o, v_mu)
    else:
        with _timed("mhada_attn"):
            att = ops.mhada_attn(q, kv, vt, fcs.t, mu_o, rstd_o, v_mu, act)
    out = torch.empty(B * Nc, C, device=dev, dtype=torch.float32)
    t16 = torch.empty(B * Nc, C, device=dev, dtype=torch.bfloat16) if want_bf16 else None
    ops.gemm(a=att.view(B * Nc, C), w=prep["w_out"], c=out, M=B * Nc, N=C, K=C, compute=dt, lda=C, ldw=C,
             bias=prep["b_out"], ldc=C, c2=t16, ldc2=C)
    f = _Feat(out.view(B, Nc, C), fc.h, fc.w)
    f.t16 = None if t16 is None else t16.view(B, Nc, C)
    return f


def _block_forward_hd(blk, fc: _Feat, fs: Optional[_Feat], fcs: _Feat, dt: torch.dtype,
                      side: Optional[dict], want_bf16: bool) -> _Feat:
    prep = block_prep(blk, dt)
    H, D = blk.num_heads, blk.head_dim
    C = H * D
    B, Nc, Cc = fc.t.shape
    cached = bool(side)
    kv = None
    act = ACT_COSINE if blk.activation_name == "cosine" else ACT_SOFTMAX
    if cached:
        mu_s, rstd_s, kv, Ns = side["mu_s"], side["rstd_s"], side["kv"], side["Ns"]
        if side["B"] != B:
            raise ValueError(f"cached style batch {side['B']} != content batch {B}")
    else:
        if fs.t.shape[2] != C:
            raise ValueError(f"channel mismatch: block expects {C}")
        mu_s, rstd_s = fs.stats()
    if Cc != C or fcs.t.shape[2] != C:
        raise ValueError(f"channel mismatch: block expects {C}")
    mu_c, rstd_c = fc.stats()
    mu_o, rstd_o = fcs.stats()
    wq, wkv, bkv, v_mu = ops.fold_block_hd(prep["wf"], prep["wg"], prep["wh"], prep["bg"], prep["bh"],
                                           rstd_c, mu_s, rstd_s, dt, ops.LOG2E if act == ACT_SOFTMAX else 1.0)
    dev = fc.t.device
    q = torch.empty(B, H, Nc, D, device=dev, dtype=dt)
    ops.gemm(a=fc.t, w=wq, c=q, M=Nc, N=D, K=D, compute=dt, lda=C, sa=(Nc * C, D), nb=(B, H), a_mu=mu_c,
# ... 84 lines not shown
```

mhada-style-transfer_amd/mhada_hip/ops.py:

```python
from __future__ import annotations

import contextlib
import ctypes
import math
from typing import Optional

import torch

from . import _lib
from ._lib import A_CONV3X3, A_CONV3X3_UP2, A_CONV3X3_ZERO, A_PATCH8, A_ROWS, A_SPLIT3, BF16, BF16X3, F32, GemmArgs, GemmTnArgs

_DT = {torch.float32: F32, torch.bfloat16: BF16}


def dt_code(dtype: torch.dtype) -> int:
    try:
        return _DT[dtype]
    except KeyError:
        raise ValueError(f"unsupported dtype {dtype}; the HIP path computes in float32 or bfloat16")


def _ptr(t: Optional[torch.Tensor]) -> Optional[int]:
    return None if t is None else t.data_ptr()


def _need_gpu(*ts: Optional[torch.Tensor]) -> None:
    dev = None
    for t in ts:
        if t is None:
            continue
        if not t.is_cuda:
            raise RuntimeError("mhada_hip ops need ROCm device tensors (the MI355X path has no CPU fallback)")
        if dev is None:
            dev = t.device
        elif t.device != dev:
            raise RuntimeError(f"mhada_hip ops need all operands on one device, got {dev} and {t.device}")


def _call(name: str, dev_tensor: torch.Tensor, *args) -> None:
    idx = dev_tensor.device.index
    guard = contextlib.nullcontext() if idx is None or idx == torch.cuda.current_device() \
        else torch.cuda.device(idx)
    with guard:
        rc = getattr(_lib.load(), name)(*args, torch.cuda.current_stream().cuda_stream)
    _lib.check(rc, name)


def gemm(*, a: torch.Tensor, w: torch.Tensor, c: torch.Tensor, M: int, N: int, K: int,
         compute: torch.dtype, a_mode: int = A_ROWS, lda: int = 0, sa=(0, 0), nb=(1, 1),
         a_mu: Optional[torch.Tensor] = None, smu=(0, 0), img=(0, 0, 0),
         ldw: int = 0, sw=(0, 0), bias: Optional[torch.Tensor] = None, sb=(0, 0),
         r: Optional[torch.Tensor] = None, ldr: int = 0, sr=(0, 0),
         ldc: int = 0, sc=(0, 0), relu: bool = False, pad: int = 0,
         c2: Optional[torch.Tensor] = None, ldc2: int = 0, sc2=(0, 0),
         vt: Optional[torch.Tensor] = None, ldt: int = 0, svt=(0, 0), c2_planes: bool = False,
         col_scale: Optional[torch.Tensor] = None) -> torch.Tensor:
    _need_gpu(a, w, c, a_mu, bias, r, c2, vt, col_scale)
    half2 = col_scale is not None
    if half2 and (a.dtype != torch.float16 or col_scale.dtype != torch.float32 or col_scale.numel() < N):
        raise ValueError("col_scale (fp32 [N]) goes with fp16 HALF2 operands")
    if c is None and not c2_planes:
        raise ValueError("gemm: C may be None only with c2_planes")
    if c2 is not None and (c2.dtype != torch.bfloat16 or (c is not None and c.dtype != torch.float32)):
        raise ValueError("c2 is the bf16 copy of an fp32 C")
    if c2_planes and (c2 is None or c2.shape[0] != 3 or not c2.is_contiguous()):
        raise ValueError("c2_planes needs c2 = contiguous bf16 [3][M][ldc2]")
    if vt is not None and vt.dtype != c.dtype:
        raise ValueError("vt has the dtype of C")
    if w.dtype != compute:
        raise ValueError("W must already be in the compute dtype")
    for t in (a_mu, bias):
        if t is not None and t.dtype != torch.float32:
            raise ValueError("a_mu / bias must be float32")
    if r is not None and r.dtype != (c.dtype if c is not None else torch.float32):
        raise ValueError("residual dtype must equal the output dtype (fp32 for a c2_planes-only output)")
    args = GemmArgs()
    args.M, args.N, args.K = M, N, K
    args.nb1, args.nb2 = nb
    args.compute = BF16 if half2 else dt_code(compute)
    args.a_mode = a_mode
    args.a, args.a_dtype, args.lda = a.data_ptr(), BF16 if half2 else dt_code(a.dtype), lda
    args.sa1, args.sa2 = sa
    args.a_mu = _ptr(a_mu)
    args.smu1, args.smu2 = smu
    args.img_c, args.img_h, args.img_w = img
    args.w, args.ldw = w.data_ptr(), ldw
    args.sw1, args.sw2 = sw
    args.bias = _ptr(bias)
    args.sb1, args.sb2 = sb
    args.r = _ptr(r)
    args.r_dtype = dt_code(r.dtype) if r is not None else 0
    args.ldr = ldr
    args.sr1, args.sr2 = sr
    args.c, args.c_dtype, args.ldc = _ptr(c), dt_code(c.dtype) if c is not None else F32, ldc
    args.sc1, args.sc2 = sc
    args.relu = int(relu)
    args.pad = int(pad)
    args.c2, args.ldc2 = _ptr(c2), ldc2
    args.sc21, args.sc22 = sc2
    args.vt, args.ldt = _ptr(vt), ldt
    args.svt1, args.svt2 = svt
    args.c2_planes = int(c2_planes)
    if half2:
        _call("mhada_gemm_half2", a, ctypes.byref(args), col_scale.data_ptr())
    else:
        _call("mhada_gemm", a, ctypes.byref(args))
    return c if c is not None else c2


def linear(x: torch.Tensor, w: torch.Tensor, bias: Optional[torch.Tensor], out_dtype: torch.dtype,
           residual: Optional[torch.Tensor] = None, relu: bool = False,
           relu_mask: Optional[torch.Tensor] = None) -> torch.Tensor:
    M, K = x.shape
    N = w.shape[0]
    c = torch.empty(M, N, device=x.device, dtype=out_dtype)
    if relu_mask is not None:
        if residual is not None or relu or out_dtype != torch.float32 or relu_mask.dtype != torch.float32 \
                or relu_mask.shape != (M, N) or not relu_mask.is_contiguous():
            raise ValueError("linear: relu_mask needs fp32 output, a contiguous fp32 [M][N] mask, no residual / relu")
        return gemm(a=x, w=w, c=c, M=M, N=N, K=K, compute=w.dtype, lda=x.stride(0), ldw=w.stride(0),
                    bias=bias, r=relu_mask, ldr=N, ldc=N, relu=2)
    return gemm(a=x, w=w, c=c, M=M, N=N, K=K, compute=w.dtype, lda=x.stride(0), ldw=w.stride(0),
                bias=bias, r=residual, ldr=N if residual is not None else 0, ldc=N, relu=relu)


def patch_embed(img: torch.Tensor, w: torch.Tensor, bias: torch.Tensor, pos: Optional[torch.Tensor],
                patch: int = 8) -> torch.Tensor:
    if patch != 8:
        raise ValueError("the HIP patch embedding implements patch_size=8 (the reference default)")
    B, Ci, H, W = img.shape
    h, wd = H // 8, W // 8
    N, C = h * wd, w.shape[0]
    out = torch.empty(B, N, C, device=img.device, dtype=torch.float32)
    return gemm(a=img, w=w, c=out, M=N, N=C, K=Ci * 64, compute=w.dtype, a_mode=A_PATCH8,
                sa=(Ci * H * W, 0), nb=(B, 1), img=(Ci, H, W), ldw=w.stride(0), bias=bias,
                r=pos, ldr=C, sr=(0, 0), ldc=C, sc=(N * C, 0))


def patch_embed_dgrad(dy: torch.Tensor, w: torch.Tensor, H: int, W: int,
                      out: Optional[torch.Tensor] = None) -> torch.Tensor:
    _need_gpu(dy, w, out)
    for t, what in ((dy, "dy"), (w, "w"), (out, "out")):
        if t is not None and (t.dtype != torch.float32 or not t.is_contiguous()):
            raise ValueError(f"patch_embed_dgrad: {what} must be contiguous float32")
    if dy.dim() != 3 or w.dim() not in (2, 4) or w.shape[0] != dy.shape[2] or (w.dim() == 4 and w.shape[2:] != (8, 8)) \
            or (w.dim() == 2 and w.shape[1] % 64):
        raise ValueError(f"patch_embed_dgrad: dy [B][N][C] and w (C, Ci, 8, 8) or [C][64 Ci], got "
                         f"{tuple(dy.shape)} and {tuple(w.shape)}")
    B, N, C = dy.shape
    Ci = w.shape[1] if w.dim() == 4 else w.shape[1] // 64
    if H < 8 or W < 8 or N != (H // 8) * (W // 8):
        raise ValueError(f"patch_embed_dgrad: {N} token rows do not match a {H} x {W} image")
    if out is None:
        out =(torch.zeros if H % 8 else torch.empty)(B, Ci, H, W, device=dy.device, dtype=torch.float32)
    elif out.shape != (B, Ci, H, W):
        raise ValueError(f"patch_embed_dgrad: out must be {(B, Ci, H, W)}, got {tuple(out.shape)}")
    _call("mhada_patch_embed_dgrad", dy, dy.data_ptr(), w.data_ptr(), out.data_ptr(), B, C, Ci, H, W)
    return out


WINO = True


def wino_eligible(x: torch.Tensor, w: torch.Tensor, upsample: bool) -> bool:
    return (WINO and w.dtype == torch.float32 and x.dtype == torch.float32 and not upsample
            and x.shape[-1] % 8 == 0 and w.shape[0] % 64 == 0 and x.shape[1] >= 2 and x.shape[2] >= 2
            and x.numel() < 2 ** 31 and x.numel() // x.shape[-1] * w.shape[0] < 2 ** 31)


WINO_WGRAD = True


def wgrad_wino_eligible(x: torch.Tensor, g: torch.Tensor, cout: int) -> bool:
    if not (WINO_WGRAD and x.is_cuda and x.dtype == torch.float32 and g.dtype == torch.float32):
        return False
    B, H, W, ci = x.shape
    return (ci % 64 == 0 and cout % 64 == 0 and H % 2 == 0 and W % 16 == 0 and g.shape[:3] == x.shape[:3]
            and g.shape[3] >= cout and g.shape[3] % 4 == 0 and x.is_contiguous() and g.is_contiguous()
            and B * H * W * max(ci, g.shape[3]) < 2 ** 31)


def conv3x3_wgrad_wino(x: torch.Tensor, g: torch.Tensor, cout: int, pad_mode: str = "reflect",
                       bias: bool = True):
    _need_gpu(x, g)
    B, H, W, ci = x.shape
    lib = _lib.load()
    S = lib.mhada_conv3x3_wgrad_wino_splits(B, H, W, ci, cout)
    if S <= 0:
        raise ValueError("conv3x3_wgrad_wino: ineligible shape")
    work = torch.empty(S * (16 * cout * ci + (cout if bias else 0)), device=x.device, dtype=torch.float32)
    dw = torch.empty(cout, 9 * ci, device=x.device, dtype=torch.float32)
    db = torch.empty(cout, device=x.device, dtype=torch.float32) if bias else None
    _call("mhada_conv3x3_wgrad_wino", x, x.data_ptr(), g.data_ptr(), dw.data_ptr(),
          db.data_ptr() if bias else None, work.data_ptr(), work.numel(), B, H, W, ci, cout, g.shape[3],
          _lib.PAD_REFLECT if pad_mode == "reflect" else _lib.PAD_ZERO)
    return dw, db


def wino_weights_split3(w: torch.Tensor) -> torch.Tensor:
    _need_gpu(w)
    Co, K = w.shape
    Ci = K // 9
    if w.dtype != torch.float32 or K != 9 * Ci or Ci % 16 or not w.is_contiguous():
        raise ValueError("wino_weights_split3 needs a contiguous fp32 [Cout][9*Cin] weight, Cin % 16 == 0")
    up = torch.empty(Ci // 16, 16, 3, Co, 16, device=w.device, dtype=torch.bfloat16)
    _call("mhada_wino_weights_split3", w, w.data_ptr(), up.data_ptr(), Co, Ci)
    return up


def wino_weights(w: torch.Tensor) -> torch.Tensor:
    _need_gpu(w)
    Co, K = w.shape
    Ci = K // 9
    if w.dtype != torch.float32 or K != 9 * Ci or not w.is_contiguous():
        raise ValueError("wino_weights needs a contiguous fp32 [Cout][9*Cin] weight")
    u = torch.empty(Ci // 8, 16, Co, 8, device=w.device, dtype=torch.float32)
    _call("mhada_wino_weights", w, w.data_ptr(), u.data_ptr(), Co, Ci)
    if Ci % 16 == 0:
        u.split3 = wino_weights_split3(w)
    return u


def conv3x3_wino(x: torch.Tensor, u: torch.Tensor, bias: Optional[torch.Tensor], relu: bool = True,
                 pad_mode: str = "reflect", pad: int = 1, out: Optional[torch.Tensor] = None,
                 relu_mask: Optional[torch.Tensor] = None) -> torch.Tensor:
    _need_gpu(x, u, bias, out, relu_mask)
    B, H, W, Ci = x.shape
    Co = u.shape[2]
    if x.dtype != torch.float32 or not x.is_contiguous() or u.shape[0] * 8 != Ci:
        raise ValueError("conv3x3_wino: contiguous fp32 NHWC input matching the filters")
    if pad_mode == "reflect":
        mode, Ho, Wo, pad = _lib.PAD_REFLECT, H, W, 1
    elif pad_mode == "zero":
        mode, Ho, Wo = _lib.PAD_ZERO, H + 2 * (pad - 1), W + 2 * (pad - 1)
    else:
        raise ValueError(f"pad_mode {pad_mode!r}")
    y = torch.empty(B, Ho, Wo, Co, device=x.device, dtype=torch.float32) if out is None else out
    if y.shape[:3] != (B, Ho, Wo) or y.dtype != torch.float32 or y.shape[-1] < Co or not y.is_contiguous():
        raise ValueError("conv3x3_wino: bad output buffer")
    if relu_mask is not None and (relu_mask.shape != y.shape or relu_mask.dtype != torch.float32
                                  or not relu_mask.is_contiguous()):
        raise ValueError("conv3x3_wino: relu_mask must be a contiguous fp32 tensor shaped like the output")
    up = getattr(u, "split3", None)
    if up is not None:
        _call("mhada_conv3x3_wino_split3", x, x.data_ptr(), u.data_ptr(), up.data_ptr(), _ptr(bias), y.data_ptr(),
              B, H, W, Ci, Co, y.shape[-1], mode, pad, int(relu), _ptr(relu_mask))
    else:
        _call("mhada_conv3x3_wino", x, x.data_ptr(), u.data_ptr(), _ptr(bias), y.data_ptr(), B, H, W, Ci, Co,
              y.shape[-1], mode, pad, int(relu), _ptr(relu_mask))
    return y


def conv3x3(x: torch.Tensor, w: torch.Tensor, bias: Optional[torch.Tensor], out_dtype: torch.dtype,
            upsample: bool, relu: bool = True, pad_mode: str = "reflect", pad: int = 1,
            out: Optional[torch.Tensor] = None, wino_u: Optional[torch.Tensor] = None,
            relu_mask: Optional[torch.Tensor] = None) -> torch.Tensor:
# ... 51 lines not shown

F32_SPLIT_OUTPROJ = True


def layernorm_split3(x: torch.Tensor, g: torch.Tensor, b: torch.Tensor, eps: float) -> torch.Tensor:
    _need_gpu(x, g, b)
    rows, cols = x.shape
    y = torch.empty(3, rows, cols, device=x.device, dtype=torch.bfloat16)
    _call("mhada_layernorm", x, x.data_ptr(), y.data_ptr(), BF16X3, g.data_ptr(), b.data_ptr(), rows, cols, eps)
    return y


def split3_weight(w: torch.Tensor) -> torch.Tensor:
    w = w.float()
    N, K0 = w.shape
    if K0 % 64:
        raise ValueError("split3_weight: K0 must be a multiple of 64")
    q0 = w.bfloat16()
    r = w - q0.float()
    q1 = r.bfloat16()
    q2 = (r - q1.float()).bfloat16()
    terms = torch.stack([t.view(N, K0 // 64, 64) for t in (q1, q0, q2, q0, q1, q0)], dim=2)
    return terms.reshape(N, 6 * K0).contiguous()


def split3_weight_dev(w: torch.Tensor, transposed: bool = False) -> torch.Tensor:
    _need_gpu(w)
    if w.dtype != torch.float32 or not w.is_contiguous() or w.dim() != 2:
        raise ValueError("split3_weight_dev needs a contiguous float32 matrix")
    N, K0 = (w.shape[1], w.shape[0]) if transposed else w.shape
    if K0 % 64:
        raise ValueError("split3_weight_dev: K0 must be a multiple of 64")
    out = torch.empty(N, 6 * K0, device=w.device, dtype=torch.bfloat16)
    _call("mhada_split3_weight", w, w.data_ptr(), out.data_ptr(), N, K0, int(transposed))
    return out


def split3_rows(x: torch.Tensor) -> torch.Tensor:
    _need_gpu(x)
    if x.dtype != torch.float32 or not x.is_contiguous() or x.dim() != 2:
        raise ValueError("split3_rows needs a contiguous float32 [M][K0] matrix")
    y = torch.empty(3, *x.shape, device=x.device, dtype=torch.bfloat16)
    _call("mhada_split3_rows", x, x.data_ptr(), y.data_ptr(), x.numel())
    return y


def linear_split3(planes: torch.Tensor, w6: torch.Tensor, bias: Optional[torch.Tensor], out_dtype: torch.dtype,
                  residual: Optional[torch.Tensor] = None, relu: bool = False,
                  out_planes: bool = False, relu_mask: Optional[torch.Tensor] = None, both: bool = False):
    if planes.dim() != 3 or planes.shape[0] != 3 or planes.dtype != torch.bfloat16 or not planes.is_contiguous():
        raise ValueError("linear_split3: planes must be contiguous bf16 [3][M][K0]")
    _, M, K0 = planes.shape
    N = w6.shape[0]
    if w6.dtype != torch.bfloat16 or w6.shape[1] != 6 * K0:
        raise ValueError("linear_split3: w6 must be split3_weight(w), bf16 [N][6*K0]")
    if out_planes:
        if out_dtype != torch.float32:
            raise ValueError("linear_split3: out_planes splits an fp32 result")
        c2 = torch.empty(3, M, N, device=planes.device, dtype=torch.bfloat16)
        return gemm(a=planes, w=w6, c=None, M=M, N=N, K=6 * K0, compute=torch.bfloat16, a_mode=A_SPLIT3, lda=K0,
                    ldw=6 * K0, bias=bias, r=residual, ldr=N if residual is not None else 0, ldc=N, relu=relu,
                    c2=c2, ldc2=N, c2_planes=True)
    c = torch.empty(M, N, device=planes.device, dtype=out_dtype)
    c2 = None
    if both:
        if out_dtype != torch.float32:
            raise ValueError("linear_split3: both splits an fp32 result")
        c2 = torch.empty(3, M, N, device=planes.device, dtype=torch.bfloat16)
    if relu_mask is not None:
        if residual is not None or relu or out_dtype != torch.float32 or relu_mask.dtype != torch.float32 \
                or relu_mask.shape != (M, N) or not relu_mask.is_contiguous():
            raise ValueError("linear_split3: relu_mask needs fp32 output, a contiguous fp32 [M][N] mask, no residual / relu")
        gemm(a=planes, w=w6, c=c, M=M, N=N, K=6 * K0, compute=torch.bfloat16, a_mode=A_SPLIT3, lda=K0,
             ldw=6 * K0, bias=bias, r=relu_mask, ldr=N, ldc=N, relu=2, c2=c2, ldc2=N if both else 0, c2_planes=both)
    else:
        gemm(a=planes, w=w6, c=c, M=M, N=N, K=6 * K0, compute=torch.bfloat16, a_mode=A_SPLIT3, lda=K0,
             ldw=6 * K0, bias=bias, r=residual, ldr=N if residual is not None else 0, ldc=N, relu=relu,
             c2=c2, ldc2=N if both else 0, c2_planes=both)
    return (c, c2) if both else c


F32_HALF2 = True

_H2_MIN = 2.0 ** -14
_H2_SCALE_WINDOW = (2.0 ** -40, 2.0 ** 40)


def _half2_planes(v: torch.Tensor):
    hi = v.half()
    hi = torch.where(hi.abs() < _H2_MIN, torch.zeros_like(hi), hi)
    lo = (v - hi.float()).half()
    lo = torch.where(lo.abs() < _H2_MIN, torch.zeros_like(lo), lo)
    return hi, lo


def half2_a_scale(gamma: torch.Tensor, beta: torch.Tensor) -> Optional[float]:
    Y = math.sqrt(gamma.numel()) * float(gamma.detach().abs().max()) + float(beta.detach().abs().max())
    if not math.isfinite(Y) or Y <= 0.0:
        return None
    q = 32768.0 / Y
    if not math.isfinite(q) or q <= 0.0:
        return None
    s_a = 2.0 ** (math.frexp(q)[1] - 1)
    return s_a if _H2_SCALE_WINDOW[0] <= s_a <= _H2_SCALE_WINDOW[1] else None


def half2_weight(w: torch.Tensor):
    w = w.float()
    N, K0 = w.shape
    if K0 % 64:
        raise ValueError("half2_weight: K0 must be a multiple of 64")
    m = w.abs().amax(dim=1)
    ok = torch.isfinite(m) & (m > 0)
    e = torch.frexp(torch.where(ok, m, torch.ones_like(m)))[1]
    t = ((127 + torch.clamp(15 - e, max=127)).to(torch.int32) << 23).view(torch.float32)
    t = torch.where(ok, t, torch.ones_like(m))
    hi, lo = _half2_planes(w * t[:, None])
    w2 = torch.stack([p.view(N, K0 // 64, 64) for p in (hi, lo)], dim=2)
    return w2.reshape(N, 2 * K0).contiguous(), t


def half2_weight_dev(w: torch.Tensor):
    _need_gpu(w)
    if w.dtype != torch.float32 or not w.is_contiguous() or w.dim() != 2 or w.shape[1] % 64:
        raise ValueError("half2_weight_dev needs a contiguous float32 [N][K0] matrix, K0 % 64 == 0")
    N, K0 = w.shape
    w2 = torch.empty(N, 2 * K0, device=w.device, dtype=torch.float16)
    t = torch.empty(N, device=w.device, dtype=torch.float32)
    _call("mhada_half2_weight", w, w.data_ptr(), w2.data_ptr(), t.data_ptr(), N, K0)
    return w2, t


def half2_prepare(gamma: torch.Tensor, beta: torch.Tensor, w: torch.Tensor) -> Optional[dict]:
    s_a = half2_a_scale(gamma, beta)
    if s_a is None or w.shape[1] % 64 or not bool(torch.isfinite(w).all()):
        return None
    w2, t = half2_weight_dev(w.float().contiguous()) if w.is_cuda else half2_weight(w)
    lo, hi = _H2_SCALE_WINDOW
    if float(t.min()) < lo or float(t.max()) > hi:
        return None
    return dict(s_a=s_a, w2=w2, cs=(1.0 / (s_a * t.double())).float().contiguous())


def layernorm_half2(x: torch.Tensor, g: torch.Tensor, b: torch.Tensor, eps: float, s_a: float) -> torch.Tensor:
    _need_gpu(x, g, b)
    rows, cols = x.shape
    y = torch.empty(2, rows, cols, device=x.device, dtype=torch.float16)
    _call("mhada_layernorm_half2", x, x.data_ptr(), y.data_ptr(), g.data_ptr(), b.data_ptr(), rows, cols, eps, s_a)
    return y


def linear_half2(planes: torch.Tensor, w2: torch.Tensor, cs: torch.Tensor, bias: Optional[torch.Tensor],
                 out_dtype: torch.dtype, residual: Optional[torch.Tensor] = None, relu: bool = False,
                 out_planes: bool = False):
    if planes.dim() != 3 or planes.shape[0] != 2 or planes.dtype != torch.float16 or not planes.is_contiguous():
        raise ValueError("linear_half2: planes must be contiguous fp16 [2][M][K0]")
    _, M, K0 = planes.shape
    N = w2.shape[0]
    if w2.dtype != torch.float16 or w2.shape[1] != 2 * K0 or not w2.is_contiguous():
        raise ValueError("linear_half2: w2 must be half2_weight(w), fp16 [N][2*K0]")
    kw = dict(a=planes, w=w2, M=M, N=N, K=K0, compute=torch.float16, lda=K0, ldw=2 * K0, bias=bias, r=residual,
              ldr=N if residual is not None else 0, ldc=N, relu=relu, col_scale=cs)
    if out_planes:
        if out_dtype != torch.float32:
            raise ValueError("linear_half2: out_planes splits an fp32 result")
        c2 = torch.empty(3, M, N, device=planes.device, dtype=torch.bfloat16)
        return gemm(c=None, c2=c2, ldc2=N, c2_planes=True, **kw)
    return gemm(c=torch.empty(M, N, device=planes.device, dtype=out_dtype), **kw)


def vit_batch_attn(qkv: torch.Tensor, L: int, ntok: int, heads: int, groups: int = 1) -> torch.Tensor:
    _need_gpu(qkv)
    C = qkv.shape[-1] // 3
    if L % groups:
        raise ValueError("vit_batch_attn: L must be a multiple of groups")
    out = torch.empty(L, ntok, C, device=qkv.device, dtype=qkv.dtype)
    Lg, es = L // groups, qkv.element_size()
    for g in range(groups):
        _call("mhada_vit_batch_attn", qkv, qkv.data_ptr() + g * Lg * ntok * 3 * C * es,
              out.data_ptr() + g * Lg * ntok * C * es, dt_code(qkv.dtype), Lg, ntok, heads, C // heads)
    return out


VIT_ATTN_SPLIT3_MAX_L = 8


def vit_batch_attn_split3(qkv: torch.Tensor, L: int, ntok: int, heads: int) -> torch.Tensor:
    _need_gpu(qkv)
    if qkv.dtype != torch.float32 or not qkv.is_contiguous():
        raise ValueError("vit_batch_attn_split3 needs contiguous float32 qkv")
    C = qkv.shape[-1] // 3
    planes = torch.empty(3, L * ntok, C, device=qkv.device, dtype=torch.bfloat16)
    _call("mhada_vit_batch_attn_split3", qkv, qkv.data_ptr(), planes.data_ptr(), L * ntok * C, L, ntok, heads,
          C // heads)
    return planes


def pos_embed(pos: torch.Tensor, oh: int, ow: int) -> torch.Tensor:
    _need_gpu(pos)
    _, C, bh, bw = pos.shape
    out = torch.empty(oh * ow, C, device=pos.device, dtype=torch.float32)
    _call("mhada_pos_embed", pos, pos.data_ptr(), out.data_ptr(), C, bh, bw, oh, ow)
    return out


def pos_embed_bwd(g: torch.Tensor, bh: int, bw: int) -> torch.Tensor:
    _need_gpu(g)
    oh, ow, C = g.shape
    if g.dtype != torch.float32 or not g.is_contiguous():
        raise ValueError("pos_embed_bwd needs a contiguous float32 [oh][ow][C] gradient")
    out = torch.empty(1, C, bh, bw, device=g.device, dtype=torch.float32)
    _call("mhada_pos_embed_bwd", g, g.data_ptr(), out.data_ptr(), C, bh, bw, oh, ow)
    return out


def instnorm_bwd(dy: torch.Tensor, y: torch.Tensor, rs: torch.Tensor) -> torch.Tensor:
    _need_gpu(dy, y, rs)
    for t in (dy, y, rs):
        if t.dtype != torch.float32 or not t.is_contiguous():
            raise ValueError("instnorm_bwd needs contiguous float32 operands")
    B, N, C = y.shape
    if dy.shape != y.shape or rs.shape != (B, C):
        raise ValueError("instnorm_bwd: shape mismatch")
    splits = max(1, min(N // 32, 2048 // max(1, B * ((C + 63) // 64))))
    work = torch.empty(splits * B * C * 2 + B * C, device=y.device, dtype=torch.float64)
    dx = torch.empty_like(y)
    _call("mhada_instnorm_bwd", y, dy.data_ptr(), y.data_ptr(), rs.data_ptr(), dx.data_ptr(), work.data_ptr(), B, N, C,
          splits)
    return dx


def attn_train_bwd_prep(dout: torch.Tensor, x: torch.Tensor, mo: torch.Tensor):
    _rows64(dout, x, mo)
    BH, Nc, _ = x.shape
    if dout.shape != x.shape or mo.shape != (BH, Nc, 128):
        raise ValueError("attn_train_bwd_prep: bad shapes")
    dx = torch.empty_like(x)
    dmo = torch.empty_like(mo)
    dd = torch.empty(BH, Nc, device=x.device, dtype=torch.float32)
    _call("mhada_attn_train_bwd_prep", x, dout.data_ptr(), x.data_ptr(), mo.data_ptr(), dx.data_ptr(), dmo.data_ptr(),
          dd.data_ptr(), BH * Nc)
    return dx, dmo, dd


def attn_train_bwd_prep_hd(dout: torch.Tensor, x: torch.Tensor, mo: torch.Tensor):
    _rows64(dout, x, mo)
    D = _train_hd_width("attn_train_bwd_prep_hd", x)
    BH, Nc, _ = x.shape
    if dout.shape != x.shape or mo.shape != (BH, Nc, 2 * D):
        raise ValueError("attn_train_bwd_prep_hd: bad shapes")
    dx = torch.empty_like(x)
    dmo = torch.empty_like(mo)
    dd = torch.empty(BH, Nc, device=x.device, dtype=torch.float32)
    _call("mhada_attn_train_bwd_prep_hd", x, dout.data_ptr(), x.data_ptr(), mo.data_ptr(), dx.data_ptr(),
          dmo.data_ptr(), dd.data_ptr(), BH * Nc, D)
    return dx, dmo, dd


def layernorm_fwd(x: torch.Tensor, gamma: torch.Tensor, beta: torch.Tensor, eps: float, planes: bool = False):
    _need_gpu(x, gamma, beta)
    for t in (x, gamma, beta):
        if t.dtype != torch.float32 or not t.is_contiguous():
            raise ValueError("layernorm_fwd needs contiguous float32 operands")
    M, C = x.shape
    y = torch.empty_like(x)
    st = torch.empty(M, 2, device=x.device, dtype=torch.float32)
    if planes:
        pl = torch.empty(3, M, C, device=x.device, dtype=torch.bfloat16)
        _call("mhada_layernorm_fwd_split3", x, x.data_ptr(), y.data_ptr(), pl.data_ptr(), st.data_ptr(),
              gamma.data_ptr(), beta.data_ptr(), M, C, float(eps))
        return y, st, pl
    _call("mhada_layernorm_fwd", x, x.data_ptr(), y.data_ptr(), st.data_ptr(), gamma.data_ptr(), beta.data_ptr(),
          M, C, float(eps))
    return y, st


def layernorm_bwd(x: torch.Tensor, dy: torch.Tensor, st: torch.Tensor, gamma: torch.Tensor):
    _need_gpu(x, dy, st, gamma)
    for t in (x, dy, st, gamma):
        if t.dtype != torch.float32 or not t.is_contiguous():
            raise ValueError("layernorm_bwd needs contiguous float32 operands")
    M, C = x.shape
    dx = torch.empty_like(x)
    dg = torch.empty(C, device=x.device, dtype=torch.float32)
    db = torch.empty(C, device=x.device, dtype=torch.float32)
    nw = ((M + 127) // 128 * 2 + 2) * C
    work = torch.empty(nw, device=x.device, dtype=torch.float32)
    _call("mhada_layernorm_bwd", x, x.data_ptr(), dy.data_ptr(), st.data_ptr(), gamma.data_ptr(), dx.data_ptr(),
          dg.data_ptr(), db.data_ptr(), work.data_ptr(), nw, M, C)
    return dx, dg, db


def instnorm_stats(x: torch.Tensor, eps: float = 1e-5):
    _need_gpu(x)
    if x.dtype != torch.float32 or not x.is_contiguous() or x.dim() != 3:
        raise ValueError(f"instnorm_stats needs contiguous float32 token rows [B][N][C], got {x.dtype} "
                         f"{tuple(x.shape)}")
    B, N, C = x.shape
    splits = max(1, min(N // 32, 2048 // max(1, B * ((C + 63) // 64))))
    mu = torch.empty(B, C, device=x.device, dtype=torch.float32)
    rstd = torch.empty(B, C, device=x.device, dtype=torch.float32)
    work = torch.empty(splits, B, C, 2, device=x.device, dtype=torch.float64)
    _call("mhada_instnorm_stats", x, x.data_ptr(), mu.data_ptr(), rstd.data_ptr(), work.data_ptr(), B, N, C,
                                          splits, eps)
    return mu, rstd


LOG2E = 1.4426950408889634


def fold_block(wf, wg, wh, bg, bh, rstd_c, mu_s, rstd_s, dtype: torch.dtype, kscale: float = LOG2E):
    B, C = rstd_c.shape
    H = wf.shape[0]
    dev = wf.device
    wq = torch.empty(B, H, 64, 64, device=dev, dtype=dtype)
    wkv = torch.empty(B, H, 128, 64, device=dev, dtype=dtype)
    bkv = torch.empty(H, 128, device=dev, dtype=torch.float32)
    v_mu = torch.empty(B, C, device=dev, dtype=torch.float32)
    _need_gpu(wf, wg, wh, bg, bh, rstd_c, mu_s, rstd_s)
    _call("mhada_fold_block", wf, wf.data_ptr(), wg.data_ptr(), wh.data_ptr(), bg.data_ptr(), bh.data_ptr(),
          rstd_c.data_ptr(), mu_s.data_ptr(), rstd_s.data_ptr(), wq.data_ptr(), wkv.data_ptr(), bkv.data_ptr(),
          v_mu.data_ptr(), kscale, dt_code(dtype), B, H)
    return wq, wkv, bkv, v_mu


def transpose_v(kv: torch.Tensor) -> torch.Tensor:
    _need_gpu(kv)
    B, H, Ns, _ = kv.shape
    ldt = (Ns + 63) // 64 * 64
    vt = torch.empty(B, H, 128, ldt, device=kv.device, dtype=kv.dtype)
    _call("mhada_transpose_v", kv, kv.data_ptr(), vt.data_ptr(), dt_code(kv.dtype), B, H, Ns)
    return vt


def cosine_prep(q: Optional[torch.Tensor], kv: Optional[torch.Tensor]) -> None:
    _need_gpu(q, kv)
    ref = q if q is not None else kv
    B, H = ref.shape[0], ref.shape[1]
    Nc = q.shape[2] if q is not None else 0
    Ns = kv.shape[2] if kv is not None else 0
    _call("mhada_cosine_prep", ref, _ptr(q), _ptr(kv), dt_code(ref.dtype), B, H, Nc, Ns)


def cosine_moments(kv: torch.Tensor, vt: torch.Tensor) -> torch.Tensor:
    _need_gpu(kv, vt)
    B, H, Ns, _ = kv.shape
    if vt.shape != (B, H, 128, (Ns + 63) // 64 * 64) or vt.dtype != kv.dtype:
# ... 736 lines not shown
```

Before: 356.9 frames/s.

## Chain fp16 hi/lo planes from MLP first GEMM into second GEMM

Adds a half2 output epilogue so the first MLP GEMM writes scaled fp16 hi/lo planes (two planes instead of three bf16 planes). The second MLP GEMM then runs on the half2 path, using weights prescaled by a per-column power-of-two bound derived from the LayerNorm and first-layer weights. The goal is to replace the three-plane bf16 split GEMM with the cheaper two-plane fp16 GEMM and to cut intermediate bandwidth. An equivalent path for attention output into the out-projection is added but disabled by default. The main risk is precision, since the bound-based scaling relies on analytic activation bounds to avoid fp16 overflow and underflow.

```diff
diff --git a/include/mhada_hip.h b/include/mhada_hip.h
--- a/include/mhada_hip.h
+++ b/include/mhada_hip.h
@@ -98,6 +98,10 @@
                           float eps, float scale, mhada_stream_t stream);
 int mhada_half2_weight(const float* w, void* out, float* t, int N, int K0, mhada_stream_t stream);
 int mhada_gemm_half2(const mhada_gemm_args* args, const float* col_scale, mhada_stream_t stream);
+int mhada_gemm_half2_planes(const mhada_gemm_args* args, const float* col_scale, const float* out_scale,
+                            mhada_stream_t stream);
+int mhada_vit_batch_attn_half2(const float* qkv, void* planes, long long pstride, const float* out_scale, int L,
+                               int ntok, int heads, int head_dim, mhada_stream_t stream);
 int mhada_kv_proj_split3(const float* fs, const float* mu_s, const float* wkv, const float* bkv, void* img,
                          int B, int H, int Ns, mhada_stream_t stream);
 int mhada_attn_split3(const float* q, const void* img, const float* fcs, const float* fcs_mu,
diff --git a/mhada-style-transfer_amd/csrc/common.h b/mhada-style-transfer_amd/csrc/common.h
--- a/mhada-style-transfer_amd/csrc/common.h
+++ b/mhada-style-transfer_amd/csrc/common.h
@@ -61,6 +61,11 @@
 template <> MHADA_DEV float from_f32<float>(float x) { return x; }
 template <> MHADA_DEV bf16 from_f32<bf16>(float x) { return (bf16)x; }
 
+MHADA_DEV _Float16 half2_plane(float v) {
+  const _Float16 q = (_Float16)v;
+  return fabsf((float)q) < 6.103515625e-05f ? (_Float16)0.0f : q;
+}
+
 template <typename T> struct Vec16;
 template <> struct Vec16<float> { typedef f32x4 type; static constexpr int N = 4; };
 template <> struct Vec16<bf16> { typedef bf16x8 type; static constexpr int N = 8; };
diff --git a/mhada-style-transfer_amd/csrc/gemm_half2.hip b/mhada-style-transfer_amd/csrc/gemm_half2.hip
--- a/mhada-style-transfer_amd/csrc/gemm_half2.hip
+++ b/mhada-style-transfer_amd/csrc/gemm_half2.hip
@@ -2,9 +2,7 @@
 
 using namespace mhada;
 
-extern "C" int mhada_gemm_half2(const mhada_gemm_args* a, const float* col_scale, mhada_stream_t stream_) {
-  if (!a) return fail("mhada_gemm_half2: null args");
-  hipStream_t stream = (hipStream_t)stream_;
+static int gemm_half2(const mhada_gemm_args* a, const float* col_scale, const float* out_scale, hipStream_t stream) {
   if (a->M < 0 || a->N <= 0 || a->K <= 0) return fail("mhada_gemm_half2: bad sizes");
   if (a->nb1 != 1 || a->nb2 != 1) return fail("mhada_gemm_half2: one problem only (nb1 = nb2 = 1)");
   if (a->K % 64) return fail("mhada_gemm_half2: K0 must be a multiple of 64");
@@ -12,7 +10,11 @@
   if (a->c_dtype != MHADA_F32 && a->c_dtype != MHADA_BF16) return fail("mhada_gemm_half2: bad c_dtype");
   if (a->r && a->r_dtype != a->c_dtype) return fail("mhada_gemm_half2: residual dtype must equal output dtype");
   if (a->relu < 0 || a->relu > 1) return fail("mhada_gemm_half2: relu must be 0 or 1");
-  if (!a->a || !a->w || !col_scale || (!a->c && !a->c2_planes)) return fail("mhada_gemm_half2: null operand");
+  if (!a->a || !a->w || !col_scale || (!a->c && !a->c2_planes && !out_scale)) return fail("mhada_gemm_half2: null operand");
+  if (out_scale && (!a->c2 || a->c_dtype != MHADA_F32 || a->N % 4 || !tuning().gemm_ldsepi || !aligned16(out_scale) ||
+                    a->ldc2 < a->N))
+    return fail("mhada_gemm_half2_planes: needs a c2 buffer with ldc2 >= N, c_dtype fp32, N % 4 == 0, a 16-byte "
+                "aligned out_scale and the LDS epilogue");
   if (a->M == 0) return MHADA_OK;
   if (!aligned16(a->a) || a->lda % 8 || a->lda < a->K)
     return fail("mhada_gemm_half2: A must be 16-byte aligned with lda a multiple of 8 and >= K0");
@@ -25,7 +27,7 @@
   if (a->bias && !aligned16(a->bias)) return fail("mhada_gemm_half2: bias must be 16-byte aligned");
   if (a->c2 && (a->c_dtype != MHADA_F32 || ((uintptr_t)a->c2 & 7) || a->ldc2 % 4))
     return fail("mhada_gemm_half2: c2 needs fp32 C, 8-byte alignment and ldc2 % 4 == 0");
-  if (a->c2_planes && (!a->c2 || a->N % 4 || !tuning().gemm_ldsepi))
+  if (!out_scale && a->c2_planes && (!a->c2 || a->N % 4 || !tuning().gemm_ldsepi))
     return fail("mhada_gemm_half2: c2_planes needs a c2 buffer, N % 4 == 0 and the LDS epilogue");
   if ((((long long)a->M + 255) / 256) * (((long long)a->N + 255) / 256) >= (1LL << 31))
     return fail("mhada_gemm_half2: more than 2^31 tiles");
@@ -41,7 +43,19 @@
   p.c = a->c; p.ldc = a->ldc;
   p.relu = a->relu;
   p.c2 = a->c2; p.ldc2 = a->ldc2;
-  p.c2planes = a->c2_planes ? 1 : 0;
+  p.c2planes = !out_scale && a->c2_planes ? 1 : 0;
+  if (out_scale) return launch_gemm_h2_f16(p, col_scale, out_scale, stream);
   if (a->c_dtype == MHADA_F32) return launch_gemm_h2<float>(p, col_scale, stream);
   return launch_gemm_h2<bf16>(p, col_scale, stream);
 }
+
+extern "C" int mhada_gemm_half2(const mhada_gemm_args* a, const float* col_scale, mhada_stream_t stream) {
+  if (!a) return fail("mhada_gemm_half2: null args");
+  return gemm_half2(a, col_scale, nullptr, (hipStream_t)stream);
+}
+
+extern "C" int mhada_gemm_half2_planes(const mhada_gemm_args* a, const float* col_scale, const float* out_scale,
+                                       mhada_stream_t stream) {
+  if (!a || !out_scale) return fail("mhada_gemm_half2_planes: null args");
+  return gemm_half2(a, col_scale, out_scale, (hipStream_t)stream);
+}
diff --git a/mhada-style-transfer_amd/csrc/gemm_impl.h b/mhada-style-transfer_amd/csrc/gemm_impl.h
--- a/mhada-style-transfer_amd/csrc/gemm_impl.h
+++ b/mhada-style-transfer_amd/csrc/gemm_impl.h
@@ -263,9 +263,11 @@
 }
 
 
-template <typename TO, int TM, int TN, bool PLANES = false>
+typedef _Float16 f16x4 __attribute__((ext_vector_type(4)));
+
+template <typename TO, int TM, int TN, bool PLANES = false, bool H2OUT = false>
 MHADA_DEV void store_tile_lds(const GemmP& p, const f32x16 (&acc)[TM][TN], int z1, int z2, int mrow0, int ncol0,
-                              int lane, float* scr) {
+                              int lane, float* scr, const float* os = nullptr) {
   TO* cbase = reinterpret_cast<TO*>(p.c) + z1 * p.sc1 + z2 * p.sc2;
   const TO* rbase = p.r ? reinterpret_cast<const TO*>(p.r) + z1 * p.sr1 + z2 * p.sr2 : nullptr;
   const float* bbase = p.bias ? p.bias + z1 * p.sb1 + z2 * p.sb2 : nullptr;
@@ -282,6 +284,10 @@
 #pragma unroll
         for (int e = 0; e < 4; ++e) bb[e] = n + e < p.N ? bbase[n + e] : 0.f;
       }
+    }
+    f32x4 ob = {0.f, 0.f, 0.f, 0.f};
+    if constexpr (H2OUT) {
+      if (n + 3 < p.N) ob = *reinterpret_cast<const f32x4*>(os + n);
     }
 #pragma unroll
     for (int mi = 0; mi < TM; ++mi) {
@@ -319,7 +325,18 @@
               for (int e = 0; e < 4; ++e) x[e] = p.relu == 2 ? (q[e] > 0.f ? x[e] : 0.f) : x[e] + q[e];
             }
             if (!PLANES || p.c) *reinterpret_cast<f32x4*>(crow + n) = f32x4{x[0], x[1], x[2], x[3]};
-            if (p.c2) {
+            if constexpr (H2OUT) {
+              _Float16* c2row = reinterpret_cast<_Float16*>(p.c2) + (long long)m * p.ldc2 + n;
+              f16x4 hi, lo;
+#pragma unroll
+              for (int e = 0; e < 4; ++e) {
+                const float v = ob[e] * x[e];
+                hi[e] = half2_plane(v);
+                lo[e] = half2_plane(v - (float)hi[e]);
+              }
+              *reinterpret_cast<f16x4*>(c2row) = hi;
+              *reinterpret_cast<f16x4*>(c2row + (long long)p.M * p.ldc2) = lo;
+            } else if (p.c2) {
               bf16* c2row = reinterpret_cast<bf16*>(p.c2) + z1 * p.sc21 + z2 * p.sc22 + (long long)m * p.ldc2 + n;
               const bf16x4 h0 = {(bf16)x[0], (bf16)x[1], (bf16)x[2], (bf16)x[3]};
               *reinterpret_cast<bf16x4*>(c2row) = h0;
@@ -1268,8 +1285,15 @@
 
 typedef _Float16 f16x8 __attribute__((ext_vector_type(8)));
 
-template <typename TO>
-__global__ void __launch_bounds__(512) gemm_h2_kernel(const GemmP p, int total, const float* __restrict__ cs) {
+template <typename... T>
+MHADA_DEV const float* h2_out_scale(T... t) {
+  const float* a[] = {nullptr, t...};
+  return a[sizeof...(T)];
+}
+
+template <typename TO, bool H2OUT = false, typename... OS>
+__global__ void __launch_bounds__(512) gemm_h2_kernel(const GemmP p, int total, const float* __restrict__ cs, OS... os_) {
+  const float* const os = h2_out_scale(os_...);
   constexpr int BK = 64, PE = 512, HALF = 128 * BK, SLOT = 2 * HALF;
   constexpr int SCR = 8 * 4096 / 2;
   __shared__ __attribute__((aligned(16))) _Float16 smem[4 * SLOT + SCR];
@@ -1435,7 +1459,10 @@
         wide = !p.r;
         if (wide) store_tile_lds_bf16<4>(p, acc, 0, 0, cur.m0 + grp * 128, cur.n0 + wc * 64, lane, scr);
       }
-      if (!wide) store_tile_lds<TO, 4, 2, true>(p, acc, 0, 0, cur.m0 + grp * 128, cur.n0 + wc * 64, lane, scr);
+      if constexpr (H2OUT)
+        store_tile_lds<TO, 4, 2, true, true>(p, acc, 0, 0, cur.m0 + grp * 128, cur.n0 + wc * 64, lane, scr, os);
+      else if (!wide)
+        store_tile_lds<TO, 4, 2, true>(p, acc, 0, 0, cur.m0 + grp * 128, cur.n0 + wc * 64, lane, scr);
     } else {
       store_tile<TO, 4, 2>(p, acc, 0, 0, cur.m0 + grp * 128 + r32, cur.n0 + wc * 64, h);
     }
@@ -1586,6 +1613,19 @@
   const int grid = (int)std::min<long long>(total, num_cus());
   hipLaunchKernelGGL((gemm_h2_kernel<TO>), dim3(grid), dim3(512), 0, stream, p, (int)total, cs);
   return check_launch("mhada_gemm_half2");
+}
+
+static int launch_gemm_h2_f16(const GemmP& p0, const float* cs, const float* os, hipStream_t stream) {
+  GemmP p = p0;
+  p.tiles_n = (int)(((long long)p.N + 255) / 256);
+  const long long total = (((long long)p.M + 255) / 256) * p.tiles_n;
+  if (total >= (1LL << 31)) return fail("mhada_gemm_half2_planes: more than 2^31 tiles");
+  p.ntiles = (int)total;
+  p.lds_epi = 1;
+  p.rinit = 0;
+  const int grid = (int)std::min<long long>(total, num_cus());
+  hipLaunchKernelGGL((gemm_h2_kernel<float, true, const float*>), dim3(grid), dim3(512), 0, stream, p, (int)total, cs, os);
+  return check_launch("mhada_gemm_half2_planes");
 }
 
 static bool pp_enabled() { return tuning().gemm_pp != 0; }
diff --git a/mhada-style-transfer_amd/csrc/small_ops.hip b/mhada-style-transfer_amd/csrc/small_ops.hip
--- a/mhada-style-transfer_amd/csrc/small_ops.hip
+++ b/mhada-style-transfer_amd/csrc/small_ops.hip
@@ -5,10 +5,6 @@
 namespace mhada {
 
 typedef _Float16 f16;
-MHADA_DEV f16 half2_plane(float v) {
-  const f16 q = (f16)v;
-  return fabsf((float)q) < 6.103515625e-05f ? (f16)0.0f : q;
-}
 
 template <typename TO, int VPL, int FORM = 0>
 __global__ void __launch_bounds__(256) layernorm_kernel(const float* __restrict__ x, TO* __restrict__ y,
@@ -203,9 +199,9 @@
   out[n * row16 + c] = qkv[n * 3 * row16 + 2 * row16 + c];
 }
 
-template <typename T, bool PLANES>
+template <typename T, int PLANES>
 MHADA_DEV void vit_batch_attn_small_body(const T* __restrict__ qkv, void* __restrict__ out_, long long pstride,
-                                         int L, int ntok, int heads) {
+                                         int L, int ntok, int heads, const float* __restrict__ os = nullptr) {
   constexpr int D = 64;
   __shared__ float sq[4][8][D + 1];
   __shared__ float sk[4][8][D + 1];
@@ -247,12 +243,20 @@
   sp[wv][i][j] = e / sum;
   __syncthreads();
   if (!valid) return;
+  float osc = 1.f;
+  if constexpr (PLANES == 2) osc = os[hh * D + lane];
   for (int r = 0; r < L; ++r) {
     float o = 0.f;
 #pragma unroll
     for (int c = 0; c < 8; ++c) o = fmaf(sp[wv][r][c], vr[c], o);
     const long long at = ((long long)r * ntok + n) * C + hh * D + lane;
-    if constexpr (PLANES) {
+    if constexpr (PLANES == 2) {
+      f16* pl = reinterpret_cast<f16*>(out_) + at;
+      const float v = osc * o;
+      const f16 hi = half2_plane(v);
+      pl[0] = hi;
+      pl[pstride] = half2_plane(v - (float)hi);
+    } else if constexpr (PLANES == 1) {
       bf16* pl = reinterpret_cast<bf16*>(out_) + at;
       const bf16 a = (bf16)o;
       const float r1 = o - (float)a;
@@ -269,13 +273,20 @@
 template <typename T>
 __global__ void __launch_bounds__(256) vit_batch_attn_small_kernel(const T* __restrict__ qkv, T* __restrict__ out,
                                                                    int L, int ntok, int heads) {
-  vit_batch_attn_small_body<T, false>(qkv, out, 0, L, ntok, heads);
+  vit_batch_attn_small_body<T, 0>(qkv, out, 0, L, ntok, heads);
 }
 
 __global__ void __launch_bounds__(256) vit_batch_attn_small_s3_kernel(const float* __restrict__ qkv,
                                                                       bf16* __restrict__ planes, long long pstride,
                                                                       int L, int ntok, int heads) {
-  vit_batch_attn_small_body<float, true>(qkv, planes, pstride, L, ntok, heads);
+  vit_batch_attn_small_body<float, 1>(qkv, planes, pstride, L, ntok, heads);
+}
+
+__global__ void __launch_bounds__(256) vit_batch_attn_small_h2_kernel(const float* __restrict__ qkv,
+                                                                      f16* __restrict__ planes, long long pstride,
+                                                                      const float* __restrict__ os, int L, int ntok,
+                                                                      int heads) {
+  vit_batch_attn_small_body<float, 2>(qkv, planes, pstride, L, ntok, heads, os);
 }
 
 __global__ void __launch_bounds__(256) vit_batch_copy_v_s3_kernel(const float* __restrict__ qkv,
@@ -966,6 +977,22 @@
   return check_launch("mhada_vit_batch_attn_split3");
 }
 
+extern "C" int mhada_vit_batch_attn_half2(const float* qkv, void* planes, long long pstride, const float* out_scale,
+                                          int L, int ntok, int heads, int head_dim, mhada_stream_t s_) {
+  hipStream_t s = (hipStream_t)s_;
+  if (!qkv || !planes || !out_scale || L <= 0 || ntok < 0 || heads <= 0)
+    return fail("mhada_vit_batch_attn_half2: bad args");
+  if (head_dim != 64) return fail("mhada_vit_batch_attn_half2: head_dim must be 64");
+  if (L > 8) return fail("mhada_vit_batch_attn_half2: L must be <= 8");
+  if (pstride < (long long)L * ntok * heads * 64)
+    return fail("mhada_vit_batch_attn_half2: plane stride smaller than this call's output");
+  if (ntok == 0) return MHADA_OK;
+  const long long pairs = (long long)ntok * heads;
+  hipLaunchKernelGGL(vit_batch_attn_small_h2_kernel, dim3((unsigned)((pairs + 3) / 4)), dim3(256), 0, s, qkv,
+                     reinterpret_cast<f16*>(planes), pstride, out_scale, L, ntok, heads);
+  return check_launch("mhada_vit_batch_attn_half2");
+}
+
 extern "C" int mhada_pos_embed(const float* pos, float* out, int C, int bh, int bw, int oh, int ow,
                                mhada_stream_t s_) {
   if (!pos || !out || C <= 0 || bh <= 0 || bw <= 0 || oh <= 0 || ow <= 0) return fail("mhada_pos_embed: bad args");
diff --git a/mhada-style-transfer_amd/mhada_hip/_lib.py b/mhada-style-transfer_amd/mhada_hip/_lib.py
--- a/mhada-style-transfer_amd/mhada_hip/_lib.py
+++ b/mhada-style-transfer_amd/mhada_hip/_lib.py
@@ -74,6 +74,8 @@
     "mhada_layernorm_half2": (_I, [_vp, _vp, _vp, _vp, _I, _I, _F, _F, _vp]),
     "mhada_half2_weight": (_I, [_vp, _vp, _vp, _I, _I, _vp]),
     "mhada_gemm_half2": (_I, [ctypes.POINTER(GemmArgs), _vp, _vp]),
+    "mhada_gemm_half2_planes": (_I, [ctypes.POINTER(GemmArgs), _vp, _vp, _vp]),
+    "mhada_vit_batch_attn_half2": (_I, [_vp, _vp, _c_ll, _vp, _I, _I, _I, _I, _vp]),
     "mhada_attn_split3": (_I, [_vp] * 7 + [_I, _I, _I, _I, _vp]),
     "mhada_attn_split3_planes": (_I, [_vp] * 7 + [_I, _I, _I, _I, _vp]),
     "mhada_attn_train_fwd": (_I, [_vp] * 7 + [_I, _I, _I, _vp]),
diff --git a/mhada-style-transfer_amd/mhada_hip/engine.py b/mhada-style-transfer_amd/mhada_hip/engine.py
--- a/mhada-style-transfer_amd/mhada_hip/engine.py
+++ b/mhada-style-transfer_amd/mhada_hip/engine.py
@@ -140,6 +140,22 @@
     if k2 not in L:
         with torch.no_grad():
             L[k2] = ops.half2_prepare(L[ln + "_g"], L[ln + "_b"], L[key])
+    return L[k2]
+
+
+def _h2_chain(L: dict, key: str) -> Optional[dict]:
+    if not (ops.F32_HALF2 and ops.F32_HALF2_CHAIN) or (key == "w_o" and not ops.F32_HALF2_CHAIN_OUTPROJ):
+        return None
+    k2 = key + "_half2"
+    if k2 not in L:
+        with torch.no_grad():
+            if key == "w2":
+                L[k2] = None if _h2(L, "ln2", "w1") is None else \
+                    ops.half2_chain_prepare(L["ln2_g"], L["ln2_b"], L["w1"], L["b1"], L["w2"])
+            else:
+                C = L["w_o"].shape[1]
+                L[k2] = ops.half2_chain_prepare(L["ln1_g"], L["ln1_b"], L["w_qkv"][2 * C:], L["b_qkv"][2 * C:],
+                                                L["w_o"])
     return L[k2]
 
 
@@ -179,19 +195,29 @@
             hb = ops.layernorm(xs, L["ln1_g"], L["ln1_b"], dt, L["eps"])
             qkv = ops.linear(hb, L["w_qkv"], L["b_qkv"], dt)
         if split_mlp and ops.F32_SPLIT_OUTPROJ and C == L["heads"] * HEAD_DIM and B <= ops.VIT_ATTN_SPLIT3_MAX_L:
-            att3 = ops.vit_batch_attn_split3(qkv.view(B, N, 3 * C), B, N, L["heads"])
-            xs = ops.linear_split3(att3, _w6(L, "w_o"), L["b_o"], torch.float32, residual=xs)
+            h2o = _h2_chain(L, "w_o")
+            if h2o is not None:
+                att2 = ops.vit_batch_attn_half2(qkv.view(B, N, 3 * C), B, N, L["heads"], h2o["u"])
+                xs = ops.linear_half2_planes(att2, h2o["w2"], h2o["cs"], L["b_o"], residual=xs)
+            else:
+                att3 = ops.vit_batch_attn_split3(qkv.view(B, N, 3 * C), B, N, L["heads"])
+                xs = ops.linear_split3(att3, _w6(L, "w_o"), L["b_o"], torch.float32, residual=xs)
         else:
             att = ops.vit_batch_attn(qkv.view(B, N, 3 * C), B, N, L["heads"])
             xs = ops.linear(att.view(B * N, C), L["w_o"], L["b_o"], torch.float32, residual=xs)
         if split_mlp:
+            h2c = _h2_chain(L, "w2")
             if h2m is not None:
                 m1 = ops.linear_half2(ops.layernorm_half2(xs, L["ln2_g"], L["ln2_b"], L["eps"], h2m["s_a"]),
-                                      h2m["w2"], h2m["cs"], L["b1"], dt, relu=True, out_planes=True)
+                                      h2m["w2"], h2m["cs"], L["b1"], dt, relu=True, out_planes=True,
+                                      out_scale=h2c["u"] if h2c is not None else None)
             else:
                 m1 = ops.linear_split3(ops.layernorm_split3(xs, L["ln2_g"], L["ln2_b"], L["eps"]), _w6(L, "w1"),
                                        L["b1"], dt, relu=True, out_planes=True)
-            xs = ops.linear_split3(m1, _w6(L, "w2"), L["b2"], torch.float32, residual=xs)
+            if h2c is not None:
+                xs = ops.linear_half2_planes(m1, h2c["w2"], h2c["cs"], L["b2"], residual=xs)
+            else:
+                xs = ops.linear_split3(m1, _w6(L, "w2"), L["b2"], torch.float32, residual=xs)
         else:
             h2 = ops.layernorm(xs, L["ln2_g"], L["ln2_b"], dt, L["eps"])
             m1 = ops.linear(h2, L["w1"], L["b1"], dt, relu=True)
diff --git a/mhada-style-transfer_amd/mhada_hip/ops.py b/mhada-style-transfer_amd/mhada_hip/ops.py
--- a/mhada-style-transfer_amd/mhada_hip/ops.py
+++ b/mhada-style-transfer_amd/mhada_hip/ops.py
@@ -54,14 +54,18 @@
          ldc: int = 0, sc=(0, 0), relu: bool = False, pad: int = 0,
          c2: Optional[torch.Tensor] = None, ldc2: int = 0, sc2=(0, 0),
          vt: Optional[torch.Tensor] = None, ldt: int = 0, svt=(0, 0), c2_planes: bool = False,
-         col_scale: Optional[torch.Tensor] = None) -> torch.Tensor:
-    _need_gpu(a, w, c, a_mu, bias, r, c2, vt, col_scale)
+         col_scale: Optional[torch.Tensor] = None, out_scale: Optional[torch.Tensor] = None) -> torch.Tensor:
+    _need_gpu(a, w, c, a_mu, bias, r, c2, vt, col_scale, out_scale)
     half2 = col_scale is not None
     if half2 and (a.dtype != torch.float16 or col_scale.dtype != torch.float32 or col_scale.numel() < N):
         raise ValueError("col_scale (fp32 [N]) goes with fp16 HALF2 operands")
-    if c is None and not c2_planes:
+    h2out = out_scale is not None
+    if h2out and (not half2 or c2 is None or c2.dtype != torch.float16 or c2_planes
+                  or out_scale.dtype != torch.float32 or out_scale.numel() < N):
+        raise ValueError("out_scale (fp32 [N]) goes with col_scale and an fp16 c2 [2][M][ldc2]")
+    if c is None and not c2_planes and not h2out:
         raise ValueError("gemm: C may be None only with c2_planes")
-    if c2 is not None and (c2.dtype != torch.bfloat16 or (c is not None and c.dtype != torch.float32)):
+    if c2 is not None and ((c2.dtype != torch.bfloat16 and not h2out) or (c is not None and c.dtype != torch.float32)):
         raise ValueError("c2 is the bf16 copy of an fp32 C")
     if c2_planes and (c2 is None or c2.shape[0] != 3 or not c2.is_contiguous()):
         raise ValueError("c2_planes needs c2 = contiguous bf16 [3][M][ldc2]")
@@ -101,7 +105,9 @@
     args.vt, args.ldt = _ptr(vt), ldt
     args.svt1, args.svt2 = svt
     args.c2_planes = int(c2_planes)
-    if half2:
+    if h2out:
+        _call("mhada_gemm_half2_planes", a, ctypes.byref(args), col_scale.data_ptr(), out_scale.data_ptr())
+    elif half2:
         _call("mhada_gemm_half2", a, ctypes.byref(args), col_scale.data_ptr())
     else:
         _call("mhada_gemm", a, ctypes.byref(args))
@@ -459,7 +465,7 @@
 
 def linear_half2(planes: torch.Tensor, w2: torch.Tensor, cs: torch.Tensor, bias: Optional[torch.Tensor],
                  out_dtype: torch.dtype, residual: Optional[torch.Tensor] = None, relu: bool = False,
-                 out_planes: bool = False):
+                 out_planes: bool = False, out_scale: Optional[torch.Tensor] = None):
     if planes.dim() != 3 or planes.shape[0] != 2 or planes.dtype != torch.float16 or not planes.is_contiguous():
         raise ValueError("linear_half2: planes must be contiguous fp16 [2][M][K0]")
     _, M, K0 = planes.shape
@@ -471,9 +477,71 @@
     if out_planes:
         if out_dtype != torch.float32:
             raise ValueError("linear_half2: out_planes splits an fp32 result")
+        if out_scale is not None:
+            c2 = torch.empty(2, M, N, device=planes.device, dtype=torch.float16)
+            return gemm(c=None, c2=c2, ldc2=N, out_scale=out_scale, **kw)
         c2 = torch.empty(3, M, N, device=planes.device, dtype=torch.bfloat16)
         return gemm(c=None, c2=c2, ldc2=N, c2_planes=True, **kw)
+    if out_scale is not None:
+        raise ValueError("linear_half2: out_scale goes with out_planes")
     return gemm(c=torch.empty(M, N, device=planes.device, dtype=out_dtype), **kw)
+
+
+F32_HALF2_CHAIN = True
+F32_HALF2_CHAIN_OUTPROJ = False
+
+
+def half2_chain_bound(gamma: torch.Tensor, beta: torch.Tensor, w: torch.Tensor, b: Optional[torch.Tensor]):
+    g, be, W = gamma.detach().double(), beta.detach().double(), w.detach().double()
+    off = W @ be
+    if b is not None:
+        off = off + b.detach().double()
+    return math.sqrt(g.numel()) * (W * g[None, :]).norm(dim=1) + off.abs()
+
+
+def half2_out_scale(Z: torch.Tensor) -> Optional[torch.Tensor]:
+    Z = Z.detach().double()
+    if not bool((torch.isfinite(Z) & (Z > 0)).all()):
+        return None
+    q = 32768.0 / Z
+    if not bool((torch.isfinite(q) & (q > 0)).all()):
+        return None
+    e = torch.frexp(q)[1] - 1
+    if int(e.min()) < -40 or int(e.max()) > 40:
+        return None
+    return ((127 + e).to(torch.int32) << 23).view(torch.float32)
+
+
+def half2_chain_prepare(gamma: torch.Tensor, beta: torch.Tensor, w_p: torch.Tensor, b_p: Optional[torch.Tensor],
+                        w_c: torch.Tensor) -> Optional[dict]:
+    ts = [t for t in (gamma, beta, w_p, b_p, w_c) if t is not None]
+    if w_c.shape[1] % 64 or w_c.shape[1] != w_p.shape[0] or not all(bool(torch.isfinite(t).all()) for t in ts):
+        return None
+    u = half2_out_scale(half2_chain_bound(gamma, beta, w_p, b_p))
+    if u is None:
+        return None
+    lo, hi = _H2_SCALE_WINDOW
+    wu = (w_c.detach().float() / u.to(w_c.device)[None, :]).contiguous()
+    m = wu.abs().amax(dim=1)
+    if not bool(torch.isfinite(m).all()) or float(m.min()) < lo or float(m.max()) > hi:
+        return None
+    w2, t = half2_weight_dev(wu) if wu.is_cuda else half2_weight(wu)
+    if float(t.min()) < lo or float(t.max()) > hi:
+        return None
+    return dict(u=u.to(w_c.device).contiguous(), w2=w2, cs=(1.0 / t.double()).float().contiguous())
+
+
+def linear_half2_planes(planes: torch.Tensor, w2: torch.Tensor, cs: torch.Tensor, bias: Optional[torch.Tensor],
+                        residual: Optional[torch.Tensor] = None) -> torch.Tensor:
+    if planes.dim() != 3 or planes.shape[0] != 2 or planes.dtype != torch.float16 or not planes.is_contiguous():
+        raise ValueError("linear_half2_planes: planes must be contiguous fp16 [2][M][K0]")
+    _, M, K0 = planes.shape
+    N = w2.shape[0]
+    if w2.dtype != torch.float16 or w2.shape[1] != 2 * K0 or not w2.is_contiguous():
+        raise ValueError("linear_half2_planes: w2 must be half2_weight(w / u), fp16 [N][2*K0]")
+    return gemm(a=planes, w=w2, c=torch.empty(M, N, device=planes.device, dtype=torch.float32), M=M, N=N, K=K0,
+                compute=torch.float16, lda=K0, ldw=2 * K0, bias=bias, r=residual,
+                ldr=N if residual is not None else 0, ldc=N, col_scale=cs)
 
 
 def vit_batch_attn(qkv: torch.Tensor, L: int, ntok: int, heads: int, groups: int = 1) -> torch.Tensor:
@@ -500,6 +568,19 @@
     planes = torch.empty(3, L * ntok, C, device=qkv.device, dtype=torch.bfloat16)
     _call("mhada_vit_batch_attn_split3", qkv, qkv.data_ptr(), planes.data_ptr(), L * ntok * C, L, ntok, heads,
           C // heads)
+    return planes
+
+
+def vit_batch_attn_half2(qkv: torch.Tensor, L: int, ntok: int, heads: int, out_scale: torch.Tensor) -> torch.Tensor:
+    _need_gpu(qkv, out_scale)
+    C = qkv.shape[-1] // 3
+    if qkv.dtype != torch.float32 or not qkv.is_contiguous():
+        raise ValueError("vit_batch_attn_half2 needs contiguous float32 qkv")
+    if out_scale.dtype != torch.float32 or out_scale.numel() != C or not out_scale.is_contiguous():
+        raise ValueError("vit_batch_attn_half2: out_scale must be contiguous float32 [C]")
+    planes = torch.empty(2, L * ntok, C, device=qkv.device, dtype=torch.float16)
+    _call("mhada_vit_batch_attn_half2", qkv, qkv.data_ptr(), planes.data_ptr(), L * ntok * C, out_scale.data_ptr(),
+          L, ntok, heads, C // heads)
     return planes
 
 
```

New measurement: 371.6 frames/s, median of 6. 1.04x the previous value.
